# SumitTarafder/Figbird

Measured on AMD Instinct MI355X. Metric: gaps/sec (+ filled-bases/sec), synthetic 1e5-gap set recipe, jump-library fill pass, higher is better.
Workload: dtype f64

## Files before the change

figbird_amd/csrc/fig_abi.hip:

```cpp
#include <hip/hip_runtime.h>

#include <algorithm>
#include <cstdio>
#include <cstdlib>
#include <cstring>
#include <new>
#include <vector>
#include <chrono>
#include <thread>
#include <mutex>

#include "../../include/figbird_hip.h"
#include "fig_engine.h"
#include "fig_pack.h"
#include "fig_abi_host.h"
#include "fig_quality.h"
#include "fig_quality_host.h"
#include "fig_placement.h"
#include "fig_softqual.h"
#include "fig_indel.h"

#ifdef FIG_PROF
#define FIG_PROF_BEGIN() const unsigned long long _k0 = __builtin_readcyclecounter()
#define FIG_PROF_FLUSH() do { if (E.lane == 0) { atomicAdd(&B.counters[FIG_CNT_WAIT], E.wait_cycles); atomicAdd(&B.counters[FIG_CNT_WAVE], (unsigned long long)__builtin_readcyclecounter() - _k0); \
    for (int i = 0; i < FIG_PROF_SLOTS; i++) if (E.prof[i]) atomicAdd(&B.counters[i < FIG_PROF_SPLIT ? FIG_CNT_PROF_LO + i : FIG_CNT_PROF_HI + (i - FIG_PROF_SPLIT)], E.prof[i]); } } while (0)
#else
#define FIG_PROF_BEGIN() ((void)0)
#define FIG_PROF_FLUSH() ((void)0)
#endif

FIG_D void fig_eng_init(FigEng &E, const FigDevModel &M, const FigDevBatch &B, const FigKernArgs &A, bool lds_tab, FigScr &work) {
    fig_eng_ident(E, threadIdx.x, blockDim.x, 64);
    E.M = &M; E.B = &B;
    E.flops = 0; E.mle_alg = 0; E.mle_exec = 0; E.wait_cycles = 0;
    for (int i = 0; i < FIG_PROF_SLOTS; i++) E.prof[i] = 0;
    unsigned char *slab = B.scratch + (long long)blockIdx.x * B.scratch_stride;
    fig_scratch_layout(slab, B.capG, B.capR, B.capP, B.capC, B.capW, B.capE, &work);
    E.scr = work;
    fig_eng_carve(E, M, A, lds_tab);
}

FIG_D void fig_kernel_begin(FigEng &E, const FigDevModel &M, const FigDevBatch &B, const FigKernArgs &A, bool lds_tab, FigScr &work) {
    fig_eng_init(E, M, B, A, lds_tab, work);
    if (blockIdx.x == 0 && threadIdx.x == 0) B.queue_head[A.qsel ^ 1] = 0;
}

FIG_D int fig_queue_pop(FigEng &E, const FigDevBatch &B, const FigKernArgs &A) {
    if (E.tid == 0) E.S->bc_i = atomicAdd(B.queue_head + A.qsel, 1);
    __syncthreads();
    const int qi = E.S->bc_i;
    __syncthreads();
    return qi;
}

template <typename T> struct FigItemSrc { const T *v; int first, end; };
FIG_D FigItemSrc<int32_t> fig_src_order(const FigDevBatch &B, const FigKernArgs &A) { return {B.order, A.q_begin, A.q_end}; }

template <typename Src, typename Body>
FIG_D void fig_pop_loop(FigEng &E, const FigDevBatch &B, const FigKernArgs &A, Src src, Body body) {
    while (true) {
        const int qi = fig_queue_pop(E, B, A);
        const auto s = src();
        if (s.first + qi >= s.end) break;
        body(s.v[s.first + qi]);
    }
}

FIG_D void fig_kernel_flush(const FigEng &E, const FigDevBatch &B) {
    if (E.flops) atomicAdd(&B.counters[FIG_CNT_FLOPS], E.flops);
    if (E.mle_alg) atomicAdd(&B.counters[FIG_CNT_MLE_ALG], E.mle_alg);
    if (E.lane == 0 && E.mle_exec) atomicAdd(&B.counters[FIG_CNT_MLE_EXEC], E.mle_exec);
}

template <bool LDS_TAB, int NT>
__global__ void __launch_bounds__(NT, (NT <= 256 ? 2 : 1)) fig_fill_kernel(FigDevModel M, FigDevBatch B, FigKernArgs A) {
    FigEng E; FigScr work;
    fig_kernel_begin(E, M, B, A, LDS_TAB, work);
    FIG_PROF_BEGIN();
    fig_pop_loop(E, B, A, [&] { return fig_src_order(B, A); }, [&](int gi) { fig_item_fill<LDS_TAB>(E, work, gi); });
    FIG_PROF_FLUSH();
    fig_kernel_flush(E, B);
}

template <bool LDS_TAB, int NT>
__global__ void __launch_bounds__(NT, (NT <= 256 ? 2 : 1)) fig_begin_kernel(FigDevModel M, FigDevBatch B, FigKernArgs A) {
    FigEng E; FigScr work;
    fig_kernel_begin(E, M, B, A, LDS_TAB, work);
    fig_pop_loop(E, B, A, [&] { return fig_src_order(B, A); }, [&](int gi) { fig_item_begin<LDS_TAB>(E, work, gi); });
    fig_kernel_flush(E, B);
}

template <bool LDS_TAB, int NT>
__global__ void __launch_bounds__(NT, (NT <= 256 ? 2 : 1)) fig_probe_kernel(FigDevModel M, FigDevBatch B, FigKernArgs A) {
    FigEng E; FigScr work;
    fig_kernel_begin(E, M, B, A, LDS_TAB, work);
    fig_pop_loop(E, B, A, [&] { return fig_src_order(B, A); }, [&](int gi) { fig_item_probe<LDS_TAB>(E, work, gi); });
}

FIG_D int fig_ld_acquire(const int32_t *p) { return __hip_atomic_load(p, __ATOMIC_ACQUIRE, __HIP_MEMORY_SCOPE_AGENT); }
FIG_D int fig_ld_relaxed(const int32_t *p) { return __hip_atomic_load(p, __ATOMIC_RELAXED, __HIP_MEMORY_SCOPE_AGENT); }

FIG_D bool fig_chunk_finished(FigEng &E, const FigDevBatch &B, int gi, int n) {
    __threadfence();
    __syncthreads();
    if (E.tid == 0) {
        const int done = __hip_atomic_fetch_add(B.gap_pending + gi, 1, __ATOMIC_ACQ_REL, __HIP_MEMORY_SCOPE_AGENT) + 1;
        if (done == n) __hip_atomic_store(B.gap_pending + gi, 0, __ATOMIC_RELAXED, __HIP_MEMORY_SCOPE_AGENT);
        E.S->bc_i = done == n;
    }
    __syncthreads();
    const bool last = E.S->bc_i != 0;
    __syncthreads();
    if (last) __threadfence();
    return last;
}

FIG_D void fig_cont_publish(FigEng &E, const FigDevBatch &B, const FigKernArgs &A, const FigCont &c) {
    __threadfence();
    __syncthreads();
    if (E.tid == 0) {
        bool ok = true;
        if (c.kind == FIG_CONT_EVAL) {
            const long long live = (long long)gridDim.x - fig_ld_relaxed(&B.cont_hdr->exited);
            ok = live * 100 >= (long long)c.n * A.cont_live;
        }
        if (ok) {
            const int idx = atomicAdd(&B.cont_hdr->tail, 1);
            if (idx < B.cont_cap) {
                FigCont *e = B.cont + idx;
                e->gap = c.gap; e->j0 = c.j0; e->n = c.n; e->kind = c.kind; e->next = 0; e->rank = c.rank; e->pad = 0;
                __hip_atomic_store(&e->ready, 1, __ATOMIC_RELEASE, __HIP_MEMORY_SCOPE_AGENT);
                if (c.kind == FIG_CONT_EVAL) atomicAdd(&B.counters[FIG_CNT_CONT], 1ull);
            }
        }
    }
    __syncthreads();
}

FIG_D bool fig_cont_pop(FigEng &E, const FigDevBatch &B, const FigKernArgs &A, FigCont &out, int &k) {
    FigState &S = *E.S;
    if (E.tid == 0) { const int t = fig_ld_relaxed(&B.cont_hdr->tail); S.bc_j = t < B.cont_cap ? t : B.cont_cap; }
    __syncthreads();
    const int tail = S.bc_j;
    __syncthreads();
    for (int pass = 0; pass <= tail; pass++) {
        if (E.tid == 0) S.bc_i = -1;
        __syncthreads();
        int best = -1;
        for (int i = E.tid; i < tail; i += E.nt) {
            const FigCont *e = B.cont + i;
            if (!fig_ld_acquire(&e->ready)) continue;
            if (fig_ld_relaxed(&e->next) >= e->n) continue;
            const int rank = A.cont_prio ? (e->rank < 32767 ? e->rank : 32767) : 0;
            const int key = rank * 65536 + (FIG_CONT_CAP_MAX - i);
            best = key > best ? key : best;
        }
        if (best >= 0) atomicMax(&S.bc_i, best);
        __syncthreads();
        const int key = S.bc_i;
        if (key < 0) { __syncthreads(); return false; }
        const int idx = FIG_CONT_CAP_MAX - (key & 65535);
        if (E.tid == 0) S.bc_j = atomicAdd(&B.cont[idx].next, 1);
        __syncthreads();
        k = S.bc_j;
        __syncthreads();
        if (k < B.cont[idx].n) { __threadfence(); out = B.cont[idx]; return true; }
    }
    return false;
}

static_assert(sizeof(FigItem) == sizeof(int4) && sizeof(FigEntry) == sizeof(int4), "item records travel as int4");
template <bool LDS_TAB, int NT>
__global__ void __launch_bounds__(NT, (NT <= 256 ? 2 : 1)) fig_eval_kernel(FigDevModel M, FigDevBatch B, FigKernArgs A, const int4 *items, int n_items) {
    FigEng E; FigScr work;
    fig_kernel_begin(E, M, B, A, LDS_TAB, work);
    FIG_PROF_BEGIN();
    auto eval = [&](FigItem it) {
        fig_item_eval<LDS_TAB>(E, work, it);
        if (A.cont && it.chunk > 0 && fig_chunk_finished(E, B, it.gap, it.chunk)) {
            FigCont nx;
            fig_item_continue(E, work, it.gap, it.chunk, A.minc, nx);
            fig_cont_publish(E, B, A, nx);
        }
    };
    fig_pop_loop(E, B, A, [&] { return FigItemSrc<FigItem>{(const FigItem *)items, 0, n_items}; }, eval);
    if (A.cont) {
        FigCont c; int k;
        while (fig_cont_pop(E, B, A, c, k)) {
            if (c.kind == FIG_CONT_END) fig_item_end<LDS_TAB>(E, work, c.gap);
            else eval(FigItem{c.gap, c.j0 + k, k, c.n});
        }
        if (E.tid == 0) atomicAdd(&B.cont_hdr->exited, 1);
    }
    FIG_PROF_FLUSH();
    fig_kernel_flush(E, B);
}

__global__ void __launch_bounds__(64) fig_replay_kernel(FigDevModel M, FigDevBatch B, const int4 *entries, int n) {
    if ((int)blockIdx.x >= n) return;
    FigEng E{}; FigScr work{};
    fig_eng_ident(E, threadIdx.x, blockDim.x, 64);
    E.M = &M; E.B = &B; E.nteams = 1; E.S = (FigState *)fig_lds;
    const FigEntry en = ((const FigEntry *)entries)[blockIdx.x];
    if (en.stamped) {
        const FigGapCtl c = B.gapctl[en.gap];
        if (c.status != FIG_GAP_MORE || c.j != en.j_planned || en.n != 0) return;
    }
    fig_item_replay(E, work, en);
}

template <bool LDS_TAB, int NT>
__global__ void __launch_bounds__(NT, (NT <= 256 ? 2 : 1)) fig_end_kernel(FigDevModel M, FigDevBatch B, FigKernArgs A, const int *list, int n) {
    FigEng E; FigScr work;
    fig_kernel_begin(E, M, B, A, LDS_TAB, work);
    fig_pop_loop(E, B, A, [&] { return FigItemSrc<int>{list, 0, n}; }, [&](int gi) { fig_item_end<LDS_TAB>(E, work, gi); });
    fig_kernel_flush(E, B);
}

__global__ void __launch_bounds__(256) fig_stream_kernel(FigDevModel M, FigDevBatch B, uint32_t *out) {
    for (long long gi = blockIdx.x; gi < B.n_gaps; gi += gridDim.x) {
        const FigDevGap &g = B.gaps[gi];
        const int L = M.L;
        const long long n = (long long)((g.nU + FIG_SH_C - 1) / FIG_SH_C) * L * (FIG_SH_C / 2);
        for (long long i = threadIdx.x; i < n; i += blockDim.x) {
            const int sp = (int)(i % (FIG_SH_C / 2));
            const long long cj = i / (FIG_SH_C / 2);
            const int j = (int)(cj % L);
            uint32_t v = 0;
            for (int h = 0; h < 2; h++) {
                const long long r = (cj / L) * FIG_SH_C + 2 * sp + h;
                unsigned e = 0x1000u | FIG_SH_ONE;
                if (r < g.nU) {
                    const long long idx = g.uBase + r;
                    const int len = B.u.len[idx], aux = B.u.aux[idx];
                    if (len == L && !(aux & 2)) {
                        const uint32_t w = B.packed[B.u.woff[idx] + (j >> 4)];
                        e = 0x1000u | (2u * (4u * (unsigned)(aux & 1) + ((w >> ((j & 15) * 2)) & 3u)));
                    }
                }
                v |= e << (16 * h);
            }
            out[g.streamOff + i] = v;
        }
    }
}

#define FIG_HIP(call) do { hipError_t _e = (call); if (_e != hipSuccess) { ctx->last_hip = (int)_e; return FIG_EHIP; } } while (0)

struct DevBuf { void *p = nullptr; };

struct FigTmpBufs {
    std::vector<void *> bufs;
    ~FigTmpBufs() { for (void *p : bufs) hipFree(p); }
    void *alloc(size_t n) { void *p = nullptr; if (hipMalloc(&p, n ? n : 8) != hipSuccess) return nullptr; bufs.push_back(p); return p; }
};

struct FigLane { hipStream_t stream = nullptr; hipEvent_t done = nullptr; int32_t *queue_head = nullptr; uint8_t *scratch = nullptr; FigItem *d_items = nullptr; FigEntry *d_entries = nullptr; size_t cap = 0;
                 FigGapCtl *h_ctl = nullptr; FigItem *h_items = nullptr; FigEntry *h_entries = nullptr; int qsel = 0;
                 uint8_t *d_cont = nullptr; int cont_cap = 0; };

struct fig_ctx {
    int device = 0;
    hipStream_t stream = nullptr;
    hipEvent_t ev0 = nullptr, ev1 = nullptr;
    int n_cu = 0;
    int last_hip = 0;
    bool have_model = false;
    FigDevModel dm;
    DevBuf d_model_tabs;
    fig_model hm;
    std::vector<double> h_ins, h_del;
    bool have_batch = false;
    FigDevBatch db;
    std::vector<int32_t> h_order;
    struct Cls { FigLaunchClass c; int blocks; int capacity; };
    std::vector<Cls> classes;
    std::vector<DevBuf> bufs;
    int64_t n_gaps = 0, n_ureads = 0, n_preads = 0, str_total = 0;
    std::vector<int64_t> h_str_off;
    int nslots = 32;
    std::vector<FigLane> lanes;
    fig_stats stats;
    int sh_on = FIG_SH_SC;
    FigKnobs fill_knobs;
    std::vector<uint8_t> h_ot;
    uint8_t *d_ot = nullptr;
};

static int dev_alloc(fig_ctx *ctx, size_t bytes, void **out) {
    DevBuf b;
    if (bytes == 0) bytes = 8;
    hipError_t e = hipMalloc(&b.p, bytes);
    if (e != hipSuccess) { ctx->last_hip = (int)e; return FIG_ENOMEM; }
    ctx->bufs.push_back(b);
    *out = b.p;
    return FIG_OK;
}

template <typename T>
static int dev_upload(fig_ctx *ctx, const std::vector<T> &v, const T **out) {
    void *p = nullptr;
    int rc = dev_alloc(ctx, v.size() * sizeof(T), &p);
    if (rc) return rc;
    if (!v.empty()) {
        hipError_t e = hipMemcpyAsync(p, v.data(), v.size() * sizeof(T), hipMemcpyHostToDevice, ctx->stream);
        if (e != hipSuccess) { ctx->last_hip = (int)e; return FIG_EHIP; }
    }
    *out = (const T *)p;
    return FIG_OK;
}

extern "C" int fig_version(void) { return FIG_ABI_VERSION; }

extern "C" const char *fig_strerror(int code) { return fig_strerror_text(code); }

extern "C" int fig_ctx_create(int device_ordinal, fig_ctx **out) {
    if (!out) return FIG_EINVAL;
    *out = nullptr;
    static std::once_flag env_once;
    std::call_once(env_once, [] { setenv("GPU_MAX_HW_QUEUES", "8", 0); });
    int n = 0;
    if (hipGetDeviceCount(&n) != hipSuccess || n <= 0) return FIG_ENODEV;
    if (device_ordinal < 0 || device_ordinal >= n) return FIG_ENODEV;
    if (hipSetDevice(device_ordinal) != hipSuccess) return FIG_ENODEV;
    hipDeviceProp_t prop;
    if (hipGetDeviceProperties(&prop, device_ordinal) != hipSuccess) return FIG_ENODEV;
    fig_ctx *ctx = new (std::nothrow) fig_ctx();
    if (!ctx) return FIG_ENOMEM;
    ctx->device = device_ordinal;
    ctx->n_cu = prop.multiProcessorCount > 0 ? prop.multiProcessorCount : 256;
    if (hipStreamCreate(&ctx->stream) != hipSuccess || hipEventCreate(&ctx->ev0) != hipSuccess || hipEventCreate(&ctx->ev1) != hipSuccess) {
        delete ctx;
        return FIG_EHIP;
    }
    memset(&ctx->stats, 0, sizeof(ctx->stats));
    ctx->sh_on = fig_knobs_from_env(0).sh_on;
    *out = ctx;
    return FIG_OK;
}

static void free_batch(fig_ctx *ctx) {
    for (auto &b : ctx->bufs) if (b.p) hipFree(b.p);
    ctx->bufs.clear();
    ctx->d_ot = nullptr;
    ctx->have_batch = false;
    ctx->classes.clear();
    for (auto &l : ctx->lanes) { if (l.stream) hipStreamDestroy(l.stream); if (l.done) hipEventDestroy(l.done); if (l.h_ctl) hipHostFree(l.h_ctl); if (l.h_items) hipHostFree(l.h_items); if (l.h_entries) hipHostFree(l.h_entries); }
    ctx->lanes.clear();
}

extern "C" void fig_batch_free(fig_ctx *ctx) {
    if (!ctx) return;
    hipSetDevice(ctx->device);
    free_batch(ctx);
}

extern "C" void fig_ctx_destroy(fig_ctx *ctx) {
    if (!ctx) return;
    hipSetDevice(ctx->device);
    free_batch(ctx);
    if (ctx->d_model_tabs.p) hipFree(ctx->d_model_tabs.p);
    if (ctx->ev0) hipEventDestroy(ctx->ev0);
    if (ctx->ev1) hipEventDestroy(ctx->ev1);
    if (ctx->stream) hipStreamDestroy(ctx->stream);
    delete ctx;
}

extern "C" int fig_ctx_set_model(fig_ctx *ctx, const fig_model *m) {
    if (!ctx) return FIG_EINVAL;
    if (int rc = fig_model_check(m)) return rc;
    hipSetDevice(ctx->device);
    free_batch(ctx);
    ctx->hm = *m;
    ctx->h_ins.assign(m->in_pos_dist, m->in_pos_dist + m->max_read_length);
    ctx->h_del.assign(m->del_pos_dist, m->del_pos_dist + m->max_read_length);
    std::vector<double> all;
    FigModelOffsets o;
    fig_model_tables(m, all, o, ctx->dm);
    if (ctx->d_model_tabs.p) { hipFree(ctx->d_model_tabs.p); ctx->d_model_tabs.p = nullptr; }
    if (hipMalloc(&ctx->d_model_tabs.p, all.size() * sizeof(double)) != hipSuccess) return FIG_ENOMEM;
    if (hipMemcpy(ctx->d_model_tabs.p, all.data(), all.size() * sizeof(double), hipMemcpyHostToDevice) != hipSuccess) return FIG_EHIP;
    fig_model_point(ctx->dm, o, (const double *)ctx->d_model_tabs.p);
    ctx->have_model = true;
    return FIG_OK;
}

extern "C" int64_t fig_results_capacity(const fig_model *m, const fig_gap_batch *b) {
    if (!m || !b) return FIG_EINVAL;
    return fig_pack_results_capacity(m, b);
}

enum FigKind { FIG_K_FILL, FIG_K_BEGIN, FIG_K_EVAL, FIG_K_END, FIG_K_PROBE };

template <typename... P, typename... Args>
static hipError_t launch_one(void (*k)(P...), size_t lds, int nt, int blocks, hipStream_t stream, Args... args) {
    hipError_t e = hipFuncSetAttribute((const void *)k, hipFuncAttributeMaxDynamicSharedMemorySize, (int)lds);
    if (e != hipSuccess) return e;
    hipLaunchKernelGGL(k, dim3(blocks), dim3(nt), lds, stream, args...);
    return hipGetLastError();
}

template <bool LDS_TAB, int NT>
static hipError_t launch_kind(fig_ctx *ctx, const fig_ctx::Cls &c, const FigDevBatch &db, hipStream_t stream, FigKind kind, int blocks, const void *list, int n, int qsel) {
    FigKernArgs A = fig_kargs_of(c.c, qsel, ctx->sh_on);
    if (kind == FIG_K_EVAL) { const FigKnobs &kn = ctx->fill_knobs; A.cont = kn.cont && db.cont_cap > 0; A.minc = kn.minc; A.cont_live = kn.cont_live; A.cont_prio = kn.cont_prio; }
    switch (kind) {
        case FIG_K_FILL: return launch_one(fig_fill_kernel<LDS_TAB, NT>, c.c.lds, NT, blocks, stream, ctx->dm, db, A);
        case FIG_K_BEGIN: return launch_one(fig_begin_kernel<LDS_TAB, NT>, c.c.lds, NT, blocks, stream, ctx->dm, db, A);
        case FIG_K_PROBE: return launch_one(fig_probe_kernel<LDS_TAB, NT>, c.c.lds, NT, blocks, stream, ctx->dm, db, A);
        case FIG_K_EVAL: return launch_one(fig_eval_kernel<LDS_TAB, NT>, c.c.lds, NT, blocks, stream, ctx->dm, db, A, (const int4 *)list, n);
        case FIG_K_END: return launch_one(fig_end_kernel<LDS_TAB, NT>, c.c.lds, NT, blocks, stream, ctx->dm, db, A, (const int *)list, n);
    }
    return hipErrorInvalidValue;
}

static hipError_t launch_any(fig_ctx *ctx, const fig_ctx::Cls &c, const FigDevBatch &db, hipStream_t stream, FigKind kind, int blocks, const void *list, int n, int qsel = 0) {
    if (c.c.tiles > 0) return launch_kind<true, 512>(ctx, c, db, stream, kind, blocks, list, n, qsel);
    if (c.c.lds_tab) return c.c.nt == 256 ? launch_kind<true, 256>(ctx, c, db, stream, kind, blocks, list, n, qsel) : launch_kind<true, 512>(ctx, c, db, stream, kind, blocks, list, n, qsel);
    return launch_kind<false, 512>(ctx, c, db, stream, kind, blocks, list, n, qsel);
}

extern "C" int fig_batch_upload(fig_ctx *ctx, const fig_gap_batch *b) {
    if (!ctx || !b) return FIG_EINVAL;
    if (!ctx->have_model) return FIG_EINVAL;
    hipSetDevice(ctx->device);
    free_batch(ctx);
    const fig_model *m = &ctx->hm;
    hipEventRecord(ctx->ev0, ctx->stream);
    FigPacked K;
    int prc = fig_pack(m, b, sizeof(FigState), K);
    if (prc) return prc;
    int64_t ng = K.n_gaps;
    ctx->h_order = K.order; ctx->h_str_off = K.str_off;
    ctx->str_total = K.str_total; ctx->n_gaps = ng;
    ctx->n_ureads = (int64_t)K.u_pos.size(); ctx->n_preads = (int64_t)K.p_pos.size();
    ctx->classes.clear();
    const bool log = fig_knobs_from_env(0).log;
    for (const FigLaunchClass &lc : K.classes) {
        fig_ctx::Cls c;
        c.c = lc;
        int per_cu = (int)std::max<size_t>(1, std::min<size_t>((160 * 1024) / std::max<size_t>(lc.lds, 1), (size_t)(2048 / lc.nt)));
        per_cu = std::min(per_cu, 8);
        c.capacity = ctx->n_cu * per_cu;
        c.blocks = std::min<int>(lc.q_end - lc.q_begin, c.capacity);
        if (log) fprintf(stderr, "[figsched] class: capG=%d capGl=%d ncolE=%d Wcap=%d nt=%d nteams=%d lds_tab=%d tiles=%d tile_cols=%d lds=%zu gaps=%d per_cu=%d blocks=%d (FigState %zu B)\n",
                                             lc.capG, lc.capGl, lc.ncolE, lc.Wcap, lc.nt, lc.nteams, (int)lc.lds_tab, lc.tiles, lc.tile_cols, lc.lds, lc.q_end - lc.q_begin, per_cu, c.blocks, sizeof(FigState));
        ctx->classes.push_back(c);
    }
    int64_t stride = fig_scratch_layout(nullptr, K.capG, K.capR, K.capP, K.capC, K.capW, K.capE, nullptr);
    stride = (stride + 255) & ~255LL;

    FigDevBatch &db = ctx->db;
    memset(&db, 0, sizeof(db));
    db.n_gaps = ng;
    int rc;
#define UP(vec, field) do { rc = dev_upload(ctx, K.vec, &db.field); if (rc) return rc; } while (0)
    UP(gaps, gaps); UP(order, order); UP(packed, packed); UP(qual, qual); UP(flank, flank);
    UP(u_pos, u.pos); UP(u_aux, u.aux); UP(u_len, u.len); UP(u_woff, u.woff);
    UP(p_pos, p.pos); UP(p_aux, p.aux); UP(p_clip, p.clip); UP(p_ref, p.refpos); UP(p_len, p.len); UP(p_woff, p.woff); UP(p_qoff, p.qoff);
#undef UP
    db.u.clip = nullptr; db.u.refpos = nullptr; db.u.qoff = nullptr;
    void *p;
    if (m->unmapped_flag) {
        if ((rc = dev_alloc(ctx, (size_t)K.stream_total * 4, &p))) return rc;
        db.ustream = (const uint32_t *)p;
        FIG_HIP(hipMemsetD32Async((hipDeviceptr_t)p, (int)(((0x1000u | FIG_SH_ONE) << 16) | (0x1000u | FIG_SH_ONE)), (size_t)K.stream_total, ctx->stream));
        if (ng > 0) {
            hipLaunchKernelGGL(fig_stream_kernel, dim3((unsigned)std::min<int64_t>(ng, 4096)), dim3(256), 0, ctx->stream, ctx->dm, db, (uint32_t *)p);
            FIG_HIP(hipGetLastError());
        }
    }
    if ((rc = dev_alloc(ctx, (size_t)ng * 4, &p))) return rc; db.filled_len = (int32_t *)p;
    if ((rc = dev_alloc(ctx, (size_t)ng * 4, &p))) return rc; db.gaptofill = (int32_t *)p;
    if ((rc = dev_alloc(ctx, (size_t)K.str_total, &p))) return rc; db.str = (char *)p;
    if ((rc = dev_alloc(ctx, 64 * (ctx->classes.size() + 1), &p))) return rc; db.queue_head = (int32_t *)p;
    if ((rc = dev_alloc(ctx, FIG_CNT_N * sizeof(unsigned long long), &p))) return rc; db.counters = (unsigned long long *)p;
    size_t total_blocks = 0;
    for (const fig_ctx::Cls &c : ctx->classes) total_blocks += (size_t)c.capacity;
    if ((rc = dev_alloc(ctx, (size_t)stride * std::max<size_t>(total_blocks, 1), &p))) return rc; db.scratch = (uint8_t *)p;
    if ((rc = dev_alloc(ctx, (size_t)K.persist_total + 256, &p))) return rc; db.persist = (uint8_t *)p;
    if ((rc = dev_alloc(ctx, (size_t)std::max<int64_t>(ng, 1) * sizeof(FigGapCtl), &p))) return rc; db.gapctl = (FigGapCtl *)p;
    if ((rc = dev_alloc(ctx, (size_t)std::max<int64_t>(ng, 1) * 4, &p))) return rc; db.gap_pending = (int32_t *)p;
    if ((rc = dev_alloc(ctx, (size_t)std::max<int64_t>(ng, 1), &p))) return rc; ctx->d_ot = (uint8_t *)p; db.ot_preset = ctx->d_ot;
    ctx->h_ot = K.ot_preset;
    FIG_HIP(hipMemcpyAsync(ctx->d_ot, ctx->h_ot.data(), (size_t)std::max<int64_t>(ng, 1), hipMemcpyHostToDevice, ctx->stream));
    ctx->nslots = K.nslots;
    {   size_t blk = 0;
        for (size_t ci = 0; ci < ctx->classes.size(); ci++) {
            const fig_ctx::Cls &c = ctx->classes[ci];
            ctx->lanes.push_back(FigLane());
            FigLane &l = ctx->lanes.back();
            if (hipStreamCreate(&l.stream) != hipSuccess || hipEventCreateWithFlags(&l.done, hipEventDisableTiming) != hipSuccess) return FIG_EHIP;
            l.queue_head = db.queue_head + 16 * (ci + 1);
            l.scratch = db.scratch + (size_t)stride * blk; blk += (size_t)c.capacity;
            l.cap = (size_t)std::max(c.c.q_end - c.c.q_begin, 1) * (size_t)(K.nslots + 1);
            if ((rc = dev_alloc(ctx, l.cap * sizeof(FigItem), &p))) return rc; l.d_items = (FigItem *)p;
            if ((rc = dev_alloc(ctx, l.cap * sizeof(FigEntry), &p))) return rc; l.d_entries = (FigEntry *)p;
            l.cont_cap = fig_cont_capacity(std::vector<int>(K.order.begin() + c.c.q_begin, K.order.begin() + c.c.q_end), K.gaps, fig_knobs_from_env(0).minc);
            if ((rc = dev_alloc(ctx, sizeof(FigContHdr) + (size_t)l.cont_cap * sizeof(FigCont), &p))) return rc; l.d_cont = (uint8_t *)p;
            if (hipHostMalloc((void **)&l.h_ctl, (size_t)std::max<int64_t>(ng, 1) * sizeof(FigGapCtl), hipHostMallocDefault) != hipSuccess) return FIG_ENOMEM;
            if (hipHostMalloc((void **)&l.h_items, l.cap * sizeof(FigItem), hipHostMallocDefault) != hipSuccess) return FIG_ENOMEM;
            if (hipHostMalloc((void **)&l.h_entries, l.cap * sizeof(FigEntry), hipHostMallocDefault) != hipSuccess) return FIG_ENOMEM;
        }
    }
    db.scratch_stride = stride;
    db.capG = K.capG; db.capR = K.capR; db.capP = K.capP; db.capC = K.capC; db.capW = K.capW; db.capE = K.capE;
    db.n_ureads = ctx->n_ureads;
    FIG_HIP(hipMemsetAsync(db.counters, 0, FIG_CNT_N * sizeof(unsigned long long), ctx->stream));
    FIG_HIP(hipMemsetAsync(db.queue_head, 0, 64 * (ctx->classes.size() + 1), ctx->stream));
    hipEventRecord(ctx->ev1, ctx->stream);
    FIG_HIP(hipStreamSynchronize(ctx->stream));
    float ms = 0; hipEventElapsedTime(&ms, ctx->ev0, ctx->ev1);
    ctx->stats.h2d_ms = ms;
    ctx->stats.packed_bytes = K.packed_bytes();
    ctx->have_batch = true;
    if (!K.ot_given && m->partial_flag && ng > 0 && (rc = fig_ot_carry_measured(ctx, ng))) { free_batch(ctx); return rc; }
    return FIG_OK;
}

extern "C" int fig_batch_probe_reach(fig_ctx *ctx, uint8_t *reach) {
    if (!ctx || !reach || !ctx->have_batch) return FIG_EINVAL;
    hipSetDevice(ctx->device);
    const int64_t ng = ctx->n_gaps;
    memset(reach, 0, (size_t)ng);
    if (!ctx->hm.partial_flag || ng == 0) return FIG_OK;
    FigDevBatch db = ctx->db;
    fig_batch_clear_planes(db);
    FIG_HIP(hipMemsetAsync(db.gapctl, 0, (size_t)ng * sizeof(FigGapCtl), ctx->stream));
    for (const fig_ctx::Cls &c : ctx->classes) {
        FIG_HIP(hipMemsetAsync(db.queue_head, 0, 8, ctx->stream));
        FIG_HIP(launch_any(ctx, c, db, ctx->stream, FIG_K_PROBE, c.blocks, nullptr, 0));
    }
    std::vector<FigGapCtl> ctl((size_t)ng);
    FIG_HIP(hipMemcpyAsync(ctl.data(), db.gapctl, (size_t)ng * sizeof(FigGapCtl), hipMemcpyDeviceToHost, ctx->stream));
    FIG_HIP(hipStreamSynchronize(ctx->stream));
    for (int64_t g = 0; g < ng; g++) reach[g] = ctl[g].reach ? 1 : 0;
    return FIG_OK;
}

extern "C" int fig_batch_set_ot_preset(fig_ctx *ctx, const uint8_t *preset) {
    if (!ctx || !preset || !ctx->have_batch) return FIG_EINVAL;
    hipSetDevice(ctx->device);
    const int64_t ng = ctx->n_gaps;
    for (int64_t g = 0; g < ng; g++) ctx->h_ot[(size_t)g] = preset[g] ? 1 : 0;
    if (ng > 0) { FIG_HIP(hipMemcpy(ctx->d_ot, ctx->h_ot.data(), (size_t)ng, hipMemcpyHostToDevice)); }
    return FIG_OK;
}

static int run_class_parallel(fig_ctx *ctx, const fig_ctx::Cls &c, FigLane &ln, const FigKnobs &knobs) {
    FigDevBatch db = ctx->db;
    db.queue_head = ln.queue_head; db.scratch = ln.scratch;
    db.cont_hdr = (FigContHdr *)ln.d_cont; db.cont = (FigCont *)(ln.d_cont + sizeof(FigContHdr));
    db.cont_cap = knobs.cont ? std::min(ln.cont_cap, knobs.cont_cap) : 0;
    const size_t cont_bytes = sizeof(FigContHdr) + (size_t)db.cont_cap * sizeof(FigCont);
    hipStream_t stream = ln.stream;
    hipSetDevice(ctx->device);
    int nl = 0;
    hipError_t e;
    auto fail = [&](hipError_t er) { ctx->last_hip = (int)er; return -1; };
    const int capacity = std::max(1, c.capacity);
    auto launch = [&](FigKind kind, int n_work, const void *list) {
        hipError_t er = launch_any(ctx, c, db, stream, kind, std::min(capacity, n_work), list, n_work, ln.qsel);
        ln.qsel ^= 1; nl++;
        return er;
    };
    if ((e = launch(FIG_K_BEGIN, c.c.q_end - c.c.q_begin, nullptr)) != hipSuccess) return fail(e);
    FigGapCtl *ctl = ln.h_ctl;
    const size_t ctl_bytes = (size_t)ctx->n_gaps * sizeof(FigGapCtl);
    const std::vector<int> ids(ctx->h_order.begin() + c.c.q_begin, ctx->h_order.begin() + c.c.q_end);
    FigRound R;
    auto now = [] { return std::chrono::duration<double, std::milli>(std::chrono::steady_clock::now().time_since_epoch()).count(); };
    const double t_start = now();
    double t_prev = now(); int round = 0, last_items = 0, last_active = 0, last_chunk = 0, n_active_max = 0;
    while (true) {
        if ((e = hipMemcpyAsync(ctl, db.gapctl, ctl_bytes, hipMemcpyDeviceToHost, stream)) != hipSuccess) return fail(e);
        if ((e = hipStreamSynchronize(stream)) != hipSuccess) return fail(e);
        fig_plan_round(ids, ctl, capacity, c.c.nsplit, ctx->nslots, knobs.minc, knobs.ipw, n_active_max, R);
        if (knobs.log) { double t = now(); fprintf(stderr, "[figsched] capG=%d round %d: active=%d chunk=%d items=%d blocks=%d  %.1f ms\n", c.c.capG, round, last_active, last_chunk, last_items, capacity, t - t_prev); t_prev = t; }
        round++;
        if (R.n_active == 0) break;
        if (ln.cap < R.items.size() || ln.cap < R.entries.size()) return fail(hipErrorOutOfMemory);
        const int n_empty = knobs.cont ? fig_round_stamp(R, ctl) : 0;
        const int n_items = (int)R.items.size(), n_ent = (int)R.entries.size();
        const size_t items_bytes = R.items.size() * sizeof(FigItem), ent_bytes = R.entries.size() * sizeof(FigEntry);
        last_items = n_items; last_active = R.n_active; last_chunk = R.chunk;
        if (n_items > 0) {
            memcpy(ln.h_items, R.items.data(), items_bytes);
            if ((e = hipMemcpyAsync(ln.d_items, ln.h_items, items_bytes, hipMemcpyHostToDevice, stream)) != hipSuccess) return fail(e);
            if (knobs.cont && (e = hipMemsetAsync(ln.d_cont, 0, cont_bytes, stream)) != hipSuccess) return fail(e);
            if ((e = launch(FIG_K_EVAL, n_items, ln.d_items)) != hipSuccess) return fail(e);
        }
        if (knobs.cont && n_empty == 0) continue;
        memcpy(ln.h_entries, R.entries.data(), ent_bytes);
        if ((e = hipMemcpyAsync(ln.d_entries, ln.h_entries, ent_bytes, hipMemcpyHostToDevice, stream)) != hipSuccess) return fail(e);
        hipLaunchKernelGGL(fig_replay_kernel, dim3(n_ent), dim3(64), sizeof(FigState) + 64, stream, ctx->dm, db, (const int4 *)ln.d_entries, n_ent);
        if ((e = hipGetLastError()) != hipSuccess) return fail(e);
        nl++;
    }
    std::vector<int> endlist;
    for (int g : ids) if (ctl[g].status == FIG_GAP_LOOP_DONE) endlist.push_back(g);
    if (!endlist.empty()) {
        if ((e = hipStreamSynchronize(stream)) != hipSuccess) return fail(e);
        memcpy(ln.h_items, endlist.data(), endlist.size() * sizeof(int));
        if ((e = hipMemcpyAsync(ln.d_items, ln.h_items, endlist.size() * sizeof(int), hipMemcpyHostToDevice, stream)) != hipSuccess) return fail(e);
        if ((e = launch(FIG_K_END, (int)endlist.size(), ln.d_items)) != hipSuccess) return fail(e);
        if (knobs.log) { const double t0 = now(); hipStreamSynchronize(stream); fprintf(stderr, "[figsched] capG=%d end kernel: %d gaps, %.1f ms (lane done at %.1f ms since its first round)\n", c.c.capG, (int)endlist.size(), now() - t0, now() - t_start); }
    }
    return nl;
}

extern "C" int fig_fill_resident(fig_ctx *ctx, fig_gap_results *out) { return fig_fill_resident_ex(ctx, out, nullptr); }

extern "C" int fig_fill_resident_ex(fig_ctx *ctx, fig_gap_results *out, const fig_gap_support *sup) {
    if (!ctx || !out || !ctx->have_batch) return FIG_EINVAL;
    if (!out->filled_len || !out->gaptofill || !out->str_off || (!out->str && ctx->str_total > 0)) return FIG_EINVAL;
    if (sup && (!sup->counts || !sup->origin)) return FIG_EINVAL;
    hipSetDevice(ctx->device);
    int64_t ng = ctx->n_gaps;
    FigDevBatch &db = ctx->db;
    FigTmpBufs tmp;
    std::vector<int32_t> hsup(sup ? (size_t)ctx->str_total * 5 : 0);
    const std::vector<FigPlane> planes = fig_fill_planes(db, ctx->n_ureads + ctx->n_preads, ctx->str_total, out, sup, hsup.data());
    auto clear = [&](void *p, int v, size_t n) { return n ? hipMemsetAsync(p, v, n, ctx->stream) : hipSuccess; };
    auto fetch = [&](void *dst, const void *src, size_t n) { return n ? hipMemcpyAsync(dst, src, n, hipMemcpyDeviceToHost, ctx->stream) : hipSuccess; };
    for (const FigPlane &pl : planes) {
        if (!(*pl.dev = tmp.alloc(pl.bytes))) return FIG_ENOMEM;
        if (pl.fill >= 0) FIG_HIP(clear(*pl.dev, pl.fill, pl.bytes));
    }
    FIG_HIP(clear(db.counters, 0, FIG_CNT_N * sizeof(unsigned long long)));
    FIG_HIP(clear(db.queue_head, 0, 64 * (ctx->classes.size() + 1)));
    for (auto &l : ctx->lanes) l.qsel = 0;
    FIG_HIP(clear(db.filled_len, 0, (size_t)std::max<int64_t>(ng, 1) * 4));
    FIG_HIP(clear(db.gaptofill, 0, (size_t)std::max<int64_t>(ng, 1) * 4));
    FIG_HIP(clear(db.str, 'N', (size_t)ctx->str_total));
    FIG_HIP(clear(db.gapctl, 0, (size_t)std::max<int64_t>(ng, 1) * sizeof(FigGapCtl)));
    FIG_HIP(clear(db.gap_pending, 0, (size_t)std::max<int64_t>(ng, 1) * 4));
    FIG_HIP(hipEventRecord(ctx->ev0, ctx->stream));
    int nl = 0;
    const FigKnobs knobs = fig_knobs_from_env(ctx->dm.unmapped);
    ctx->fill_knobs = knobs;
    if (knobs.seq) {
        for (const fig_ctx::Cls &c : ctx->classes) {
            FIG_HIP(clear(db.queue_head, 0, 4));
            FIG_HIP(launch_any(ctx, c, db, ctx->stream, FIG_K_FILL, c.blocks, nullptr, 0));
            nl++;
        }
    } else {
        const size_t nc = ctx->classes.size();
        std::vector<int> rcs(nc, 0);
        for (size_t ci = 0; ci < nc; ci++) FIG_HIP(hipStreamWaitEvent(ctx->lanes[ci].stream, ctx->ev0, 0));
        if (nc <= 1 || knobs.lanes_serial) {
            for (size_t ci = 0; ci < nc; ci++) rcs[ci] = run_class_parallel(ctx, ctx->classes[ci], ctx->lanes[ci], knobs);
        } else {
            std::vector<std::thread> th;
            for (size_t ci = 0; ci < nc; ci++) th.emplace_back([&, ci] { rcs[ci] = run_class_parallel(ctx, ctx->classes[ci], ctx->lanes[ci], knobs); });
            for (auto &t : th) t.join();
        }
        for (size_t ci = 0; ci < nc; ci++) {
            if (rcs[ci] < 0) { hipDeviceSynchronize(); return FIG_EHIP; }
            nl += rcs[ci];
            FIG_HIP(hipEventRecord(ctx->lanes[ci].done, ctx->lanes[ci].stream));
            FIG_HIP(hipStreamWaitEvent(ctx->stream, ctx->lanes[ci].done, 0));
        }
    }
    FIG_HIP(hipEventRecord(ctx->ev1, ctx->stream)); FIG_HIP(hipStreamSynchronize(ctx->stream));
    float ms = 0; FIG_HIP(hipEventElapsedTime(&ms, ctx->ev0, ctx->ev1));
    ctx->stats.kernel_ms = ms; ctx->stats.n_launches = nl;
    FIG_HIP(hipEventRecord(ctx->ev0, ctx->stream));
    std::vector<char> hstr((size_t)ctx->str_total);
    unsigned long long cnt[FIG_CNT_N] = {0};
    FIG_HIP(fetch(out->filled_len, db.filled_len, (size_t)ng * 4)); FIG_HIP(fetch(out->gaptofill, db.gaptofill, (size_t)ng * 4));
    FIG_HIP(fetch(hstr.data(), db.str, (size_t)ctx->str_total));
    FIG_HIP(fetch(cnt, db.counters, sizeof(cnt)));
    for (const FigPlane &pl : planes) FIG_HIP(fetch(pl.host, *pl.dev, pl.bytes));
    FIG_HIP(hipEventRecord(ctx->ev1, ctx->stream)); FIG_HIP(hipStreamSynchronize(ctx->stream));
    FIG_HIP(hipEventElapsedTime(&ms, ctx->ev0, ctx->ev1));
    ctx->stats.d2h_ms = ms;
#ifdef FIG_PROF
    { auto prof = [&](int i) { return cnt[i < FIG_PROF_SPLIT ? FIG_CNT_PROF_LO + i : FIG_CNT_PROF_HI + (i - FIG_PROF_SPLIT)]; };
      const unsigned long long wave = cnt[FIG_CNT_WAVE];
      const char *nm[14] = {"A.wait", "B.wait", "-", "M.finish", "PR.pre", "PR.estep", "PR.mid", "PR.mle", "PR.post", "A.chain", "A.logexp", "A.work", "B.work", "M.chains"};
      for (int i = 0; i < 14; i++) fprintf(stderr, "[figprof] %-9s %8.1f Gcycles = %5.1f %% of wave-cycles\n", nm[i], prof(i) / 1e9, wave ? 100.0 * prof(i) / wave : 0.0);
      const char *mn[4] = {"M.setup", "M.hint", "M.rounds", "M.surv"};
      for (int i = 0; i < 4; i++) fprintf(stderr, "[figprof] %-9s %8.1f Gcycles = %5.1f %% of wave-cycles\n", mn[i], prof(14 + i) / 1e9, wave ? 100.0 * prof(14 + i) / wave : 0.0);
      fprintf(stderr, "[figprof] raw slots:"); for (int i = 0; i < FIG_PROF_SLOTS; i++) fprintf(stderr, " %d:%.1f", i, prof(i) / 1e9); fprintf(stderr, "\n");
      fprintf(stderr, "[figprof] barrier wait %.3f of %.3f wave-Gcycles = %.1f %%\n", cnt[FIG_CNT_WAIT] / 1e9, wave / 1e9, wave ? 100.0 * cnt[FIG_CNT_WAIT] / wave : 0.0); }
#endif
    if (knobs.log) fprintf(stderr, "[figsched] useful flops %.4g, speculative evaluations executed %.4g (%.1f %% discarded)\n", (double)cnt[FIG_CNT_FLOPS], (double)cnt[FIG_CNT_SPEC], cnt[FIG_CNT_SPEC] ? 100.0 * (1.0 - ((double)cnt[FIG_CNT_FLOPS] / (double)cnt[FIG_CNT_SPEC])) : 0.0);
    fig_stats_from_counters(cnt, ctx->stats);
    int rc = fig_compact_results(ng, hstr.data(), ctx->h_str_off.data(), out);
    if (!rc && sup) fig_compact_support(ng, hsup.data(), ctx->h_str_off.data(), out, sup->counts);
    return rc;
}

struct FigPostFill {
    fig_ctx *ctx = nullptr;
    const fig_gap_results *f = nullptr;
    int64_t total = 0;
    std::vector<FigDevGap> hg;
    std::vector<double> tabs;
    FigTmpBufs tmp;
    bool oom = false;
    float ms = 0;

    int open(fig_ctx *c, const fig_gap_results *filled, std::vector<double> *insd = nullptr) {
        ctx = c; f = filled;
        if (!ctx || !f || !ctx->have_batch || !ctx->have_model) return FIG_EINVAL;
        if (!f->filled_len || !f->str_off || !f->draw_pos || !f->draw_len) return FIG_EINVAL;
        hipSetDevice(ctx->device);
        const int64_t ng = ctx->n_gaps;
        if (f->str_off[0] < 0) return FIG_EINVAL;
        for (int64_t g = 0; g < ng; g++) if (f->str_off[g + 1] < f->str_off[g]) return FIG_EINVAL;
        total = f->str_off[ng];
        if (total > 0 && !f->str) return FIG_EINVAL;
        const int L = ctx->dm.L;
        hg.resize((size_t)ng);
        std::vector<double> he((size_t)L), home((size_t)L);
        tabs.resize((size_t)fig_quality_tab_doubles(L));
        if (ng > 0) FIG_HIP(fetch(hg.data(), ctx->db.gaps, (size_t)ng * sizeof(FigDevGap)));
        FIG_HIP(fetch(he.data(), ctx->dm.e, (size_t)L * sizeof(double)));
        FIG_HIP(fetch(home.data(), ctx->dm.ome1, (size_t)L * sizeof(double)));
        if (insd) { insd->resize((size_t)ctx->dm.max_insert); FIG_HIP(fetch(insd->data(), ctx->dm.insd, insd->size() * sizeof(double))); }
        FIG_HIP(hipStreamSynchronize(ctx->stream));
        fig_quality_tables(L, he.data(), home.data(), ctx->dm.T, tabs.data(), tabs.data() + L, tabs.data() + 2 * L);
        return FIG_OK;
    }
    int64_t drawn_reads(int64_t g, int32_t n, int64_t base, int64_t cnt, int64_t limit) const {
        if (n > (1 << 30) || f->str_off[g] + n > f->str_off[g + 1] || base < 0 || cnt < 0 || base + cnt > limit) return -1;
        return fig_quality_check_placements(f->draw_pos + base, cnt);
    }
    hipError_t fetch(void *dst, const void *src, size_t bytes) { return hipMemcpyAsync(dst, src, bytes, hipMemcpyDeviceToHost, ctx->stream); }
    void *alloc(size_t bytes) { void *p = tmp.alloc(bytes); oom = oom || !p; return p; }
    template <typename T> const T *up(const T *src, size_t count) {
        void *p = alloc(count * sizeof(T));
        if (p && count && hipMemcpyAsync(p, src, count * sizeof(T), hipMemcpyHostToDevice, ctx->stream) != hipSuccess) { oom = true; return nullptr; }
        return (const T *)p;
    }
    template <typename Launch, typename Back> int run(Launch launch, Back back) {
        if (oom) { hipStreamSynchronize(ctx->stream); return FIG_ENOMEM; }
        FIG_HIP(hipEventRecord(ctx->ev0, ctx->stream));
        launch();
        FIG_HIP(hipGetLastError());
        FIG_HIP(hipEventRecord(ctx->ev1, ctx->stream));
        FIG_HIP(back());
        FIG_HIP(hipStreamSynchronize(ctx->stream));
        FIG_HIP(hipEventElapsedTime(&ms, ctx->ev0, ctx->ev1));
        return FIG_OK;
    }
};
#define FIG_TRY(call) do { const int _rc = (call); if (_rc != FIG_OK) return _rc; } while (0)

extern "C" int fig_batch_quality(fig_ctx *ctx, const fig_gap_results *f, const int32_t *origin, fig_gap_quality *q) {
    if (!q || !q->loglik || !q->phred || !q->state || (f && !f->draw_isz)) return FIG_EINVAL;
    FigPostFill P;
    FIG_TRY(P.open(ctx, f));
    const int64_t ng = ctx->n_gaps, total = P.total, nr = ctx->n_ureads + ctx->n_preads;
    const FigDevBatch &db = ctx->db;
    std::vector<int32_t> list, ncol((size_t)std::max<int64_t>(ng, 1), 0);
    std::vector<uint8_t> part((size_t)std::max<int64_t>(ng, 1), 0);
    int64_t cols = 0, reads = 0;
    for (int64_t g = 0; g < ng; g++) {
        const int32_t n = f->filled_len[g], lu = f->draw_len[2 * g], lp = f->draw_len[2 * g + 1];
        q->state[g] = fig_quality_gap_on(n, lu, lp, origin != nullptr, origin ? origin[g] : 0);
        if (q->state[g] != FIG_QUAL_ON) continue;
        const bool p = lp >= 0;
        const int64_t base = p ? ctx->n_ureads + P.hg[(size_t)g].pBase : P.hg[(size_t)g].uBase, cnt = p ? P.hg[(size_t)g].nP : P.hg[(size_t)g].nU;
        const int64_t drawn = P.drawn_reads(g, n, base, cnt, nr);
        if (drawn < 0) return FIG_EINVAL;
        list.push_back((int32_t)g); ncol[(size_t)g] = n; part[(size_t)g] = p ? 1 : 0;
        cols += n; reads += drawn;
    }
    if (total > 0) memset(q->loglik, 0, (size_t)total * 4 * sizeof(double));
    if (total > 0) memset(q->phred, 0, (size_t)total);
    if (!list.empty()) {
        FigQualArgs A;
        A.gaps = db.gaps; A.u_len = db.u.len; A.u_aux = db.u.aux; A.p_len = db.p.len; A.u_woff = db.u.woff; A.p_woff = db.p.woff;
        A.packed = db.packed; A.n_ureads = ctx->n_ureads; A.L = ctx->dm.L;
        A.draw_pos = P.up(f->draw_pos, (size_t)nr);
        A.list = P.up(list.data(), list.size());
        A.ncol = P.up(ncol.data(), (size_t)ng);
        A.partial = P.up(part.data(), (size_t)ng);
        A.str_off = P.up(f->str_off, (size_t)(ng + 1));
        A.tabs = P.up(P.tabs.data(), P.tabs.size());
        A.loglik = (double *)P.alloc((size_t)total * 4 * sizeof(double));
        if (A.loglik) FIG_HIP(hipMemsetAsync(A.loglik, 0, (size_t)total * 4 * sizeof(double), ctx->stream));
        FIG_TRY(P.run([&] { hipLaunchKernelGGL(fig_quality_kernel, dim3((unsigned)list.size()), dim3(FIG_Q_NT), 0, ctx->stream, A); },
                      [&] { return P.fetch(q->loglik, A.loglik, (size_t)total * 4 * sizeof(double)); }));
    }
    for (int32_t g : list)
        for (int64_t i = f->str_off[g], e = f->str_off[g] + ncol[(size_t)g]; i < e; i++) q->phred[i] = fig_quality_phred(q->loglik + i * 4, f->str[i]);
    if (fig_knobs_from_env(ctx->dm.unmapped).log)
        fprintf(stderr, "[figqual] gaps on %zu of %lld, columns %lld, reads %lld, kernel %.3f ms\n", list.size(), (long long)ng, (long long)cols, (long long)reads, P.ms);
    return FIG_OK;
}

struct FigPlacePass {
    std::vector<int32_t> items, ncol;
    std::vector<uint8_t> scored, state;
    std::vector<double> li, hd;
    std::vector<int32_t> hi;
    int64_t gaps_on = 0, reads = 0, placements = 0, cols = 0, nu = 0;
    FigPlaceArgs A;
    double *dd = nullptr;
    int32_t *di = nullptr;

    int prepare(FigPostFill &P, const int32_t *origin, const std::vector<double> &insd) {
        fig_ctx *ctx = P.ctx;
        const fig_gap_results *f = P.f;
        const int64_t ng = ctx->n_gaps;
        const FigDevBatch &db = ctx->db;
        const int MI = ctx->dm.max_insert;
        nu = ctx->n_ureads;
        li.resize((size_t)MI);
        fig_placement_li(MI, insd.data(), li.data());
        ncol.assign((size_t)std::max<int64_t>(ng, 1), 0);
        state.assign((size_t)std::max<int64_t>(ng, 1), FIG_PLACE_OFF);
        scored.assign((size_t)std::max<int64_t>(nu, 1), 0);
        for (int64_t g = 0; g < ng; g++) {
            const int32_t n = f->filled_len[g];
            state[(size_t)g] = fig_placement_gap_on(ctx->dm.unmapped != 0, n, f->draw_len[2 * g], f->draw_len[2 * g + 1], origin != nullptr, origin ? origin[g] : 0);
            if (state[(size_t)g] != FIG_PLACE_ON) continue;
            const int64_t base = P.hg[(size_t)g].uBase, cnt = P.hg[(size_t)g].nU;
            const int64_t drawn = P.drawn_reads(g, n, base, cnt, nu);
            if (drawn < 0) return FIG_EINVAL;
            gaps_on++; ncol[(size_t)g] = n; reads += drawn; cols += n;
            for (int64_t r = 0; r < cnt; r++) scored[(size_t)(base + r)] = f->draw_pos[base + r] != INT32_MIN;
            for (int64_t c0 = 0; c0 < cnt; c0 += FIG_RS_CHUNK) {
                bool any = false;
                for (int64_t r = c0; r < std::min<int64_t>(c0 + FIG_RS_CHUNK, cnt); r++) any = any || scored[(size_t)(base + r)];
                if (any) { items.push_back((int32_t)g); items.push_back((int32_t)c0); }
            }
        }
        if (items.empty()) return FIG_OK;
        A.gaps = db.gaps; A.u_len = db.u.len; A.u_aux = db.u.aux; A.u_pos = db.u.pos; A.u_woff = db.u.woff; A.packed = db.packed; A.flank = db.flank;
        A.L = ctx->dm.L; A.Tmin = ctx->dm.Tmin; A.Tmax = ctx->dm.Tmax; A.max_insert = MI;
        A.draw_pos = P.up(f->draw_pos, (size_t)nu);
        A.items = P.up(items.data(), items.size());
        A.ncol = P.up(ncol.data(), (size_t)ng);
        A.str_off = P.up(f->str_off, (size_t)(ng + 1));
        A.str = P.up(f->str, (size_t)P.total);
        A.tabs = P.up(P.tabs.data(), P.tabs.size());
        A.li = P.up(li.data(), li.size());
        dd = (double *)P.alloc((size_t)nu * 3 * sizeof(double));
        di = (int32_t *)P.alloc((size_t)nu * 2 * sizeof(int32_t));
        A.ll_drawn = dd; A.ll_other = dd + nu; A.sum_other = dd + 2 * nu; A.off_other = di; A.n_valid = di + nu;
        hd.resize((size_t)nu * 3); hi.resize((size_t)nu * 2);
        return FIG_OK;
    }
    void launch(hipStream_t stream) { hipLaunchKernelGGL(fig_placement_kernel, dim3((unsigned)(items.size() / 2)), dim3(FIG_P_NT), 0, stream, A); }
    hipError_t fetch(FigPostFill &P) { const hipError_t e = P.fetch(hd.data(), dd, hd.size() * sizeof(double)); return e != hipSuccess ? e : P.fetch(hi.data(), di, hi.size() * sizeof(int32_t)); }
    void finish(fig_read_placement *p, int64_t ng, bool launched) {
        for (int64_t g = 0; g < ng; g++) p->state[g] = state[(size_t)g];
        for (int64_t r = 0; r < nu; r++) {
            p->ll_drawn[r] = 0.0; p->ll_other[r] = 0.0; p->sum_other[r] = 0.0; p->off_other[r] = INT32_MIN; p->n_valid[r] = 0; p->pq[r] = FIG_PLACE_NONE;
        }
        placements = 0;
        if (!launched) return;
        for (int64_t r = 0; r < nu; r++) {
            if (!scored[(size_t)r]) continue;
            p->ll_drawn[r] = hd[(size_t)r]; p->ll_other[r] = hd[(size_t)(nu + r)]; p->sum_other[r] = hd[(size_t)(2 * nu + r)];
            p->off_other[r] = hi[(size_t)r]; p->n_valid[r] = hi[(size_t)(nu + r)];
            p->pq[r] = fig_placement_phred(p->ll_drawn[r], p->ll_other[r], p->sum_other[r]);
            placements += p->n_valid[r];
        }
    }
};
static bool fig_placement_members(const fig_read_placement *p) { return p->ll_drawn && p->ll_other && p->sum_other && p->off_other && p->n_valid && p->pq && p->state; }

extern "C" int fig_batch_placement(fig_ctx *ctx, const fig_gap_results *f, const int32_t *origin, fig_read_placement *p) {
    if (!p || !fig_placement_members(p)) return FIG_EINVAL;
    FigPostFill P;
    std::vector<double> insd;
    FIG_TRY(P.open(ctx, f, &insd));
    FigPlacePass PP;
    FIG_TRY(PP.prepare(P, origin, insd));
    const bool work = !PP.items.empty();
    if (work) FIG_TRY(P.run([&] { PP.launch(ctx->stream); }, [&] { return PP.fetch(P); }));
    PP.finish(p, ctx->n_gaps, work);
    if (fig_knobs_from_env(ctx->dm.unmapped).log)
        fprintf(stderr, "[figplace] gaps on %lld of %lld, reads scored %lld, placements scored %lld, kernel %.3f ms\n", (long long)PP.gaps_on, (long long)ctx->n_gaps, (long long)PP.reads, (long long)PP.placements, P.ms);
    return FIG_OK;
}

extern "C" int fig_batch_softqual(fig_ctx *ctx, const fig_gap_results *f, const int32_t *origin, fig_read_placement *pl, fig_gap_softqual *out) {
    if (!out || !out->wcount || !out->eloglik || !out->phred || !out->state) return FIG_EINVAL;
    if (pl && !fig_placement_members(pl)) return FIG_EINVAL;
    FigPostFill P;
    std::vector<double> insd;
    FIG_TRY(P.open(ctx, f, &insd));
    FigPlacePass PP;
    FIG_TRY(PP.prepare(P, origin, insd));
    const int64_t ng = ctx->n_gaps, total = P.total;
    for (int64_t g = 0; g < ng; g++) out->state[g] = PP.state[(size_t)g] == FIG_PLACE_ON ? FIG_SOFTQ_ON : FIG_SOFTQ_OFF;
    if (total > 0) { memset(out->wcount, 0, (size_t)total * 4 * sizeof(double)); memset(out->eloglik, 0, (size_t)total * 4 * sizeof(double)); memset(out->phred, 0, (size_t)total); }
    const bool work = !PP.items.empty();
    float ms_place = 0, ms_soft = 0;
    int64_t active = 0;
    if (work) {
        std::vector<int32_t> blocks;
        for (int64_t g = 0; g < ng; g++)
            if (PP.state[(size_t)g] == FIG_PLACE_ON) for (int32_t xb = 0; xb < PP.ncol[(size_t)g]; xb += FIG_SQ_NT) { blocks.push_back((int32_t)g); blocks.push_back(xb); }
        const size_t nb = blocks.size() / 2, plane = (size_t)total * 4;
        FigSoftqArgs A;
        const FigPlaceArgs &Q = PP.A;
        A.gaps = Q.gaps; A.u_len = Q.u_len; A.u_aux = Q.u_aux; A.u_pos = Q.u_pos; A.u_woff = Q.u_woff; A.packed = Q.packed; A.flank = Q.flank;
        A.draw_pos = Q.draw_pos; A.ncol = Q.ncol; A.str_off = Q.str_off; A.str = Q.str; A.tabs = Q.tabs; A.li = Q.li;
        A.L = Q.L; A.Tmin = Q.Tmin; A.Tmax = Q.Tmax; A.max_insert = Q.max_insert;
        A.placed = PP.dd; A.n_ureads = PP.nu;
        A.items = P.up(blocks.data(), blocks.size());
        double *dp = (double *)P.alloc(plane * 2 * sizeof(double) + nb * sizeof(int32_t));
        A.out = dp; A.plane = (int64_t)plane;
        std::vector<int32_t> hact(nb, 0);
        struct Ev { hipEvent_t e = nullptr; ~Ev() { if (e) hipEventDestroy(e); } } mid;
        if (P.oom) { hipStreamSynchronize(ctx->stream); return FIG_ENOMEM; }
        FIG_HIP(hipEventCreate(&mid.e));
        FIG_HIP(hipMemsetAsync(dp, 0, plane * 2 * sizeof(double), ctx->stream));
        FIG_HIP(hipEventRecord(ctx->ev0, ctx->stream));
        PP.launch(ctx->stream);
        FIG_HIP(hipGetLastError());
        FIG_HIP(hipEventRecord(mid.e, ctx->stream));
        hipLaunchKernelGGL(fig_softqual_kernel, dim3((unsigned)nb), dim3(FIG_SQ_NT), 0, ctx->stream, A);
        FIG_HIP(hipGetLastError());
        FIG_HIP(hipEventRecord(ctx->ev1, ctx->stream));
        FIG_HIP(P.fetch(out->wcount, dp, plane * sizeof(double)));
        FIG_HIP(P.fetch(out->eloglik, dp + plane, plane * sizeof(double)));
        FIG_HIP(P.fetch(hact.data(), dp + 2 * plane, nb * sizeof(int32_t)));
        if (pl) FIG_HIP(PP.fetch(P));
        FIG_HIP(hipStreamSynchronize(ctx->stream));
        FIG_HIP(hipEventElapsedTime(&ms_place, ctx->ev0, mid.e));
        FIG_HIP(hipEventElapsedTime(&ms_soft, mid.e, ctx->ev1));
        for (int32_t a : hact) active += a;
    }
    if (pl) PP.finish(pl, ng, work);
    for (int64_t g = 0; g < ng; g++)
        if (out->state[g] == FIG_SOFTQ_ON)
            for (int64_t i = f->str_off[g], e = f->str_off[g] + PP.ncol[(size_t)g]; i < e; i++) out->phred[i] = fig_quality_phred(out->eloglik + i * 4, f->str[i]);
    if (fig_knobs_from_env(ctx->dm.unmapped).log)
        fprintf(stderr, "[figsoftq] gaps on %lld of %lld, columns %lld, reads %lld, active placements %lld, placement kernel %.3f ms, softqual kernel %.3f ms\n",
                (long long)PP.gaps_on, (long long)ng, (long long)PP.cols, (long long)PP.reads, (long long)active, ms_place, ms_soft);
    return FIG_OK;
}

extern "C" int fig_batch_indel(fig_ctx *ctx, const fig_gap_results *f, const int32_t *origin, fig_gap_indel *out) {
    if (!out || !out->ll_flat || !out->ll_gapped || !out->n_ins || !out->n_del || !out->d_end || !out->d_start || !out->del_reads || !out->ins_reads ||
        !out->cover || !out->ins_end || !out->call || !out->call_end || !out->state) return FIG_EINVAL;
    FigPostFill P;
    FIG_TRY(P.open(ctx, f));
    const int64_t ng = ctx->n_gaps, total = P.total, nu = ctx->n_ureads;
    const FigDevBatch &db = ctx->db;
    const int L = ctx->dm.L;
    std::vector<int32_t> hlen((size_t)std::max<int64_t>(nu, 1), 0);
    if (nu > 0) { FIG_HIP(P.fetch(hlen.data(), db.u.len, (size_t)nu * sizeof(int32_t))); FIG_HIP(hipStreamSynchronize(ctx->stream)); }
    std::vector<int32_t> items, ncol((size_t)std::max<int64_t>(ng, 1), 0);
    std::vector<uint8_t> aligned((size_t)std::max<int64_t>(nu, 1), 0);
    int64_t gaps_on = 0, reads = 0, events = 0, called = 0;
    for (int64_t g = 0; g < ng; g++) {
        const int32_t n = f->filled_len[g];
        out->state[g] = fig_indel_gap_on(ctx->dm.unmapped != 0, n, f->draw_len[2 * g], f->draw_len[2 * g + 1], origin != nullptr, origin ? origin[g] : 0);
        if (out->state[g] != FIG_INDEL_ON) continue;
        const int64_t base = P.hg[(size_t)g].uBase, cnt = P.hg[(size_t)g].nU;
        if (P.drawn_reads(g, n, base, cnt, nu) < 0) return FIG_EINVAL;
        gaps_on++; ncol[(size_t)g] = n;
        for (int64_t c0 = 0; c0 < cnt; c0 += FIG_RS_CHUNK) {
            bool any = false;
            for (int64_t r = c0; r < std::min<int64_t>(c0 + FIG_RS_CHUNK, cnt); r++) {
                const bool a = fig_indel_aligned(f->draw_pos[base + r], std::min(std::max(hlen[(size_t)(base + r)], 0), L), n);
                aligned[(size_t)(base + r)] = a; any = any || a; reads += a;
            }
            if (any) { items.push_back((int32_t)g); items.push_back((int32_t)c0); }
        }
    }
    for (int64_t r = 0; r < nu; r++) { out->ll_flat[r] = 0.0; out->ll_gapped[r] = 0.0; out->n_ins[r] = 0; out->n_del[r] = 0; out->d_end[r] = 0; out->d_start[r] = INT32_MIN; }
    for (int64_t i = 0; i < total; i++) { out->del_reads[i] = 0; out->ins_reads[i] = 0; out->cover[i] = 0; out->call[i] = '.'; }
    for (int64_t g = 0; g < ng; g++) { out->ins_end[g] = 0; out->call_end[g] = '.'; }
    if (!items.empty()) {
        std::vector<double> tid((size_t)(2 * L));
        fig_indel_tables(L, ctx->h_ins.data(), ctx->h_del.data(), tid.data(), tid.data() + L);
        FigIndelArgs A;
        A.gaps = db.gaps; A.u_len = db.u.len; A.u_aux = db.u.aux; A.u_woff = db.u.woff; A.packed = db.packed; A.flank = db.flank; A.L = L;
        A.draw_pos = P.up(f->draw_pos, (size_t)nu);
        A.items = P.up(items.data(), items.size());
        A.ncol = P.up(ncol.data(), (size_t)ng);
        A.str_off = P.up(f->str_off, (size_t)(ng + 1));
        A.str = P.up(f->str, (size_t)total);
        A.tabs = P.up(P.tabs.data(), P.tabs.size());
        A.tabs_id = P.up(tid.data(), tid.size());
        double *dd = (double *)P.alloc((size_t)nu * 2 * sizeof(double));
        int32_t *di = (int32_t *)P.alloc((size_t)nu * 4 * sizeof(int32_t));
        const size_t ncnt = (size_t)total * 3 + (size_t)ng;
        int32_t *dc = (int32_t *)P.alloc(ncnt * sizeof(int32_t));
        A.ll_flat = dd; A.ll_gapped = dd + nu; A.n_ins = di; A.n_del = di + nu; A.d_end = di + 2 * nu; A.d_start = di + 3 * nu;
        A.del_reads = dc; A.ins_reads = dc + total; A.cover = dc + 2 * total; A.ins_end = dc + 3 * total;
        if (dc) FIG_HIP(hipMemsetAsync(dc, 0, ncnt * sizeof(int32_t), ctx->stream));
        std::vector<double> hd((size_t)nu * 2);
        std::vector<int32_t> hi((size_t)nu * 4);
        FIG_TRY(P.run([&] { fig_indel_launch(A, (unsigned)(items.size() / 2), ctx->stream); },
                      [&] {
                          hipError_t e = P.fetch(hd.data(), dd, hd.size() * sizeof(double));
                          if (e == hipSuccess) e = P.fetch(hi.data(), di, hi.size() * sizeof(int32_t));
                          if (e == hipSuccess && total > 0) e = P.fetch(out->del_reads, A.del_reads, (size_t)total * sizeof(int32_t));
                          if (e == hipSuccess && total > 0) e = P.fetch(out->ins_reads, A.ins_reads, (size_t)total * sizeof(int32_t));
                          if (e == hipSuccess && total > 0) e = P.fetch(out->cover, A.cover, (size_t)total * sizeof(int32_t));
                          return e != hipSuccess ? e : P.fetch(out->ins_end, A.ins_end, (size_t)ng * sizeof(int32_t));
                      }));
        for (int64_t r = 0; r < nu; r++) {
            if (!aligned[(size_t)r]) continue;
            out->ll_flat[r] = hd[(size_t)r]; out->ll_gapped[r] = hd[(size_t)(nu + r)];
            out->n_ins[r] = hi[(size_t)r]; out->n_del[r] = hi[(size_t)(nu + r)]; out->d_end[r] = hi[(size_t)(2 * nu + r)]; out->d_start[r] = hi[(size_t)(3 * nu + r)];
            events += out->n_ins[r] + out->n_del[r] > 0;
        }
        for (int64_t g = 0; g < ng; g++) {
            if (out->state[g] != FIG_INDEL_ON) continue;
            const int64_t s0 = f->str_off[g], n = ncol[(size_t)g];
            for (int64_t i = s0; i < s0 + n; i++) { out->call[i] = fig_indel_call(out->del_reads[i], out->ins_reads[i], out->cover[i]); called += out->call[i] != '.'; }
            out->call_end[g] = fig_indel_majority(out->ins_end[g], out->cover[s0 + n - 1]) ? 'I' : '.';
            called += out->call_end[g] != '.';
        }
    }
    if (fig_knobs_from_env(ctx->dm.unmapped).log)
        fprintf(stderr, "[figindel] gaps on %lld of %lld, reads aligned %lld, reads with an event %lld, columns called %lld, kernel %.3f ms\n",
                (long long)gaps_on, (long long)ng, (long long)reads, (long long)events, (long long)called, P.ms);
    return FIG_OK;
}

extern "C" int fig_fill_gaps(fig_ctx *ctx, const fig_gap_batch *batch, fig_gap_results *out) { return fig_fill_gaps_once(ctx, batch, out); }

extern "C" int fig_get_stats(const fig_ctx *ctx, fig_stats *out) {
    if (!ctx || !out) return FIG_EINVAL;
    *out = ctx->stats;
    return FIG_OK;
}
```

figbird_amd/csrc/fig_abi_host.h:

```cpp
#ifndef FIG_ABI_HOST_H
#define FIG_ABI_HOST_H
#include <algorithm>
#include <cmath>
#include <cstdlib>
#include <cstring>
#include <vector>
#include "../../include/figbird_hip.h"
#include "fig_types.h"
#include "fig_gaprules.h"

static_assert(FIG_ORG_NONE == FIG_SUP_NONE && FIG_ORG_FINAL == FIG_SUP_FINAL && FIG_ORG_ORIGINAL == FIG_SUP_ORIGINAL && FIG_ORG_TIEBREAK == FIG_SUP_TIEBREAK,
              "the engine's path mask (fig_types.h) is fig_gap_support::origin");

static inline const char *fig_strerror_text(int code) {
    switch (code) {
        case FIG_OK: return "ok";
        case FIG_EINVAL: return "invalid argument";
        case FIG_ENODEV: return "no usable HIP device (libfighip has no CPU path)";
        case FIG_ENOMEM: return "out of memory";
        case FIG_EHIP: return "HIP runtime error";
        case FIG_ENOSPC: return "result string buffer too small";
        case FIG_EUNSUP: return "input outside the supported envelope";
        default: return "unknown error";
    }
}

static inline int fig_model_check(const fig_model *m) {
    if (!m || !m->error_pos_dist || !m->in_pos_dist || !m->del_pos_dist || !m->insert_len_dist_smoothed) return FIG_EINVAL;
    if (m->max_read_length <= 0 || m->max_read_length > FIG_MAX_READLEN) return FIG_EUNSUP;
    if (m->max_insert_size <= 0) return FIG_EINVAL;
    if (m->partial_flag && m->unmapped_flag) return FIG_EUNSUP;
    if (m->insert_threshold_min < 0 || m->insert_threshold_max >= m->max_insert_size + 1) return FIG_EINVAL;
    return FIG_OK;
}

struct FigModelOffsets { size_t e, pairs, m3, insd, qtab, ome; };

static void fig_model_tables(const fig_model *m, std::vector<double> &all, FigModelOffsets &o, FigDevModel &dm) {
    const int L = m->max_read_length;
    std::vector<double> h_e(m->error_pos_dist, m->error_pos_dist + L), h_ome(L), h_m3(L);
    for (int k = 0; k < L; k++) {
        volatile double a = 1 - m->error_pos_dist[k];
        h_ome[k] = a;
        volatile double b = 1 - m->error_pos_dist[k] - m->in_pos_dist[k] - m->del_pos_dist[k];
        h_m3[k] = b;
    }
    std::vector<double> h_insd(m->insert_len_dist_smoothed, m->insert_len_dist_smoothed + m->max_insert_size);
    h_insd.push_back(0.0);
    std::vector<double> h_qtab(256);
    for (int c = 0; c < 256; c++) { int Q = c - 33; h_qtab[c] = pow(10, -Q / 10.0); }
    std::vector<double> pairs((size_t)8 * L);
    for (int k = 0; k < L; k++) {
        pairs[2 * k] = h_ome[k]; pairs[2 * k + 1] = h_e[k];
        pairs[2 * L + 2 * k] = h_ome[L - 1 - k]; pairs[2 * L + 2 * k + 1] = h_e[L - 1 - k];
        pairs[4 * L + 2 * k] = h_m3[k]; pairs[4 * L + 2 * k + 1] = h_e[k];
        pairs[6 * L + 2 * k] = h_m3[L - 1 - k]; pairs[6 * L + 2 * k + 1] = h_e[L - 1 - k];
    }
    all.clear();
    o.e = 0; all.insert(all.end(), h_e.begin(), h_e.end()); while (all.size() % 8) all.push_back(0);
    o.pairs = all.size(); all.insert(all.end(), pairs.begin(), pairs.end()); while (all.size() % 8) all.push_back(0);
    o.m3 = all.size(); all.insert(all.end(), h_m3.begin(), h_m3.end()); while (all.size() % 8) all.push_back(0);
    o.insd = all.size(); all.insert(all.end(), h_insd.begin(), h_insd.end()); while (all.size() % 8) all.push_back(0);
    o.qtab = all.size(); all.insert(all.end(), h_qtab.begin(), h_qtab.end());
    o.ome = all.size(); all.insert(all.end(), h_ome.begin(), h_ome.end());
    dm.L = L; dm.Tmin = m->insert_threshold_min; dm.Tmax = m->insert_threshold_max; dm.cutoff = m->gap_prob_cutoff;
    dm.partial_flag = m->partial_flag; dm.unmapped = m->unmapped_flag; dm.script_itr = m->script_itr; dm.D = m->max_distance;
    dm.read_length = m->read_length; dm.neg_overlap = m->neg_overlap; dm.partial_len = m->partial_len; dm.unm_limit = m->unm_limit;
    dm.max_insert = m->max_insert_size;
    for (int i = 0; i < 25; i++) dm.T[i] = m->error_type_probs[i];
    dm.fmm_up = fig_model_fmm(m);
}

static inline void fig_model_point(FigDevModel &dm, const FigModelOffsets &o, const double *d) {
    dm.e = d + o.e; dm.ome = d + o.pairs; dm.m3 = d + o.m3; dm.insd = d + o.insd; dm.qtab = d + o.qtab;
    dm.ome1 = d + o.ome;
}

static inline void fig_batch_clear_planes(FigDevBatch &db) {
    db.dbg_n_cand = nullptr; db.dbg_cand_i = nullptr; db.dbg_cand_lik = nullptr; db.dbg_max_cand = 0; db.dbg_n_place = nullptr;
    db.draw_pos = db.draw_isz = db.draw_len = nullptr;
    db.dbg_counts = db.dbg_read_maxlv = nullptr; db.dbg_plane_cols = db.dbg_plane_reads = 0;
    db.sup_counts = db.sup_origin = nullptr;
}

struct FigPlane { void **dev; void *host; size_t bytes; int fill; };

static std::vector<FigPlane> fig_fill_planes(FigDevBatch &db, int64_t n_reads, int64_t str_total, const fig_gap_results *out, const fig_gap_support *sup, int32_t *sup_host) {
    std::vector<FigPlane> pl;
    auto add = [&](auto *&dev, void *host, size_t bytes, int fill) { pl.push_back(FigPlane{(void **)&dev, host, bytes, fill}); };
    const size_t ng = (size_t)db.n_gaps, nr = (size_t)n_reads;
    fig_batch_clear_planes(db);
    if (out->dbg_n_cand && out->dbg_cand_i && out->dbg_cand_lik && out->dbg_max_cand > 0) {
        const size_t nc = ng * out->dbg_max_cand;
        db.dbg_max_cand = out->dbg_max_cand;
        add(db.dbg_n_cand, out->dbg_n_cand, ng * 4, 0);
        add(db.dbg_cand_i, out->dbg_cand_i, nc * 12, -1);
        add(db.dbg_cand_lik, out->dbg_cand_lik, nc * 8, -1);
        if (out->dbg_n_place) add(db.dbg_n_place, out->dbg_n_place, ng * 4, 0);
        if (out->dbg_counts && out->dbg_plane_cols > 0) { db.dbg_plane_cols = out->dbg_plane_cols; add(db.dbg_counts, out->dbg_counts, nc * out->dbg_plane_cols * 5 * 8, 0); }
        if (out->dbg_read_maxlv && out->dbg_plane_reads > 0) { db.dbg_plane_reads = out->dbg_plane_reads; add(db.dbg_read_maxlv, out->dbg_read_maxlv, nc * out->dbg_plane_reads * 8, 0); }
    }
    if (out->draw_pos && out->draw_isz && out->draw_len) {
        add(db.draw_pos, out->draw_pos, nr * 4, -1);
        add(db.draw_isz, out->draw_isz, nr * 4, 0);
        add(db.draw_len, out->draw_len, ng * 8, -1);
    }
    if (sup) {
        add(db.sup_counts, sup_host, (size_t)str_total * 5 * 4, 0);
        add(db.sup_origin, sup->origin, ng * 4, 0);
    }
    return pl;
}

static inline void fig_stats_from_counters(const unsigned long long *cnt, fig_stats &st) {
    st.place_calls = (int64_t)cnt[FIG_CNT_PLACE];
    st.alg_flops = (double)cnt[FIG_CNT_FLOPS]; st.spec_flops = (double)cnt[FIG_CNT_SPEC];
    st.mle_alg_flops = (double)cnt[FIG_CNT_MLE_ALG]; st.mle_exec_flops = (double)cnt[FIG_CNT_MLE_EXEC];
    st.cont_chunks = (int32_t)cnt[FIG_CNT_CONT];
}

static FigKernArgs fig_kargs_of(const FigLaunchClass &c, int qsel, int sh_on) {
    FigKernArgs A;
    A.capG = c.capG; A.capGl = c.capGl; A.ncolE = c.ncolE; A.Wcap = c.Wcap; A.nteams = c.nteams;
    A.q_begin = c.q_begin; A.q_end = c.q_end; A.qsel = qsel;
    A.tiles = c.tiles; A.tile_step = c.tile_step; A.tile_cols = c.tile_cols; A.tiled_max = c.tiled_max;
    A.sh_on = sh_on;
    return A;
}

static int fig_ot_carry_measured(fig_ctx *ctx, int64_t ng) {
    std::vector<uint8_t> reach((size_t)ng, 0), preset((size_t)ng, 0);
    int rc;
    if ((rc = fig_batch_probe_reach(ctx, reach.data()))) return rc;
    std::vector<int64_t> ids((size_t)ng);
    for (int64_t g = 0; g < ng; g++) ids[(size_t)g] = g;
    fig_ot_carry(ids, reach.data(), preset.data());
    return fig_batch_set_ot_preset(ctx, preset.data());
}

static int fig_compact_results(int64_t ng, const char *src, const int64_t *src_off, fig_gap_results *out) {
    int64_t need = 0;
    for (int64_t g = 0; g < ng; g++) need += out->filled_len[g] > 0 ? out->filled_len[g] : 0;
    if (need > out->str_capacity) return FIG_ENOSPC;
    int64_t o = 0;
    for (int64_t g = 0; g < ng; g++) {
        out->str_off[g] = o;
        int n = out->filled_len[g];
        if (n > 0) { memcpy(out->str + o, src + src_off[g], (size_t)n); o += n; }
    }
    out->str_off[ng] = o;
    return FIG_OK;
}

static void fig_compact_support(int64_t ng, const int32_t *src, const int64_t *src_off, const fig_gap_results *out, int32_t *dst) {
    for (int64_t g = 0; g < ng; g++) {
        int n = out->filled_len[g];
        if (n > 0) memcpy(dst + out->str_off[g] * 5, src + src_off[g] * 5, (size_t)n * 5 * sizeof(int32_t));
    }
}

static int fig_fill_gaps_once(fig_ctx *ctx, const fig_gap_batch *batch, fig_gap_results *out) {
    int rc = fig_batch_upload(ctx, batch);
    if (rc) return rc;
    rc = fig_fill_resident(ctx, out);
    fig_batch_free(ctx);
    return rc;
}

struct FigKnobs {
    bool seq;
    bool cont; int cont_cap, cont_live, cont_prio;
    bool lanes_serial;
    bool log;
    int minc;
    double ipw;
    int sh_on;
};

static FigKnobs fig_knobs_from_env(int unmapped) {
    FigKnobs k;
    const char *sched = getenv("FIG_SCHED"), *ser = getenv("FIG_LANES"), *mc = getenv("FIG_MIN_CHUNK"), *ipw = getenv("FIG_ITEMS_PER_WG");
    const char *ev = getenv("FIG_ESTEP"), *sc = getenv("FIG_SH_CHUNKS");
    k.seq = sched && strcmp(sched, "seq") == 0;
    const char *cc = getenv("FIG_CONT_CAP"), *cl = getenv("FIG_CONT_LIVE"), *cp = getenv("FIG_CONT_PRIO");
    k.cont = sched ? strcmp(sched, "continuous") == 0 : unmapped != 0;
    k.cont_cap = cc ? std::max(1, atoi(cc)) : FIG_CONT_CAP_MAX;
    k.cont_live = cl ? std::max(0, atoi(cl)) : 100;
    k.cont_prio = cp ? (atoi(cp) != 0) : 1;
    k.lanes_serial = ser && strcmp(ser, "serial") == 0;
    k.log = getenv("FIG_SCHED_LOG") != nullptr;
    k.minc = mc ? std::max(1, atoi(mc)) : 16;
    k.ipw = ipw ? std::max(1.0, atof(ipw)) : (unmapped ? 12.0 : 6.0);
    k.sh_on = (ev && !strcmp(ev, "pair")) ? 0 : (sc ? std::max(1, std::min(FIG_SH_SC, atoi(sc))) : FIG_SH_SC);
    return k;
}

struct FigRound { std::vector<FigItem> items; std::vector<FigEntry> entries; int chunk = 0, n_active = 0; };

static void fig_plan_round(const std::vector<int> &ids, const FigGapCtl *ctl, int capacity, int nsplit, int slots_cap, int minc, double ipw_base,
                           int &n_active_max, FigRound &R) {
    R.items.clear(); R.entries.clear();
    R.chunk = 0; R.n_active = 0;
    for (int g : ids) if (ctl[g].status == FIG_GAP_MORE) R.n_active++;
    if (R.n_active == 0) return;
    long long rem_total = 0;
    for (int g : ids) if (ctl[g].status == FIG_GAP_MORE) rem_total += std::max(0, ctl[g].range - ctl[g].j);
    n_active_max = std::max(n_active_max, R.n_active);
    const double ipw = ipw_base * std::min(8.0, std::max(1.0, n_active_max / 96.0));
    const double share = rem_total > 0 ? (ipw * capacity / (double)std::max(1, nsplit)) / (double)rem_total : 1.0;
    const double target = ipw * capacity / (double)std::max(1, nsplit);
    long long total = 0;
    for (int g : ids) {
        if (ctl[g].status != FIG_GAP_MORE) continue;
        if ((double)total >= 1.25 * target) break;
        int j = ctl[g].j, range = ctl[g].range;
        int want = (int)std::ceil((range - j) * share);
        want = std::min(std::max(want, minc), slots_cap);
        int n = std::max(0, std::min(want, range - j));
        R.chunk = std::max(R.chunk, n);
        total += n;
        R.entries.push_back(FigEntry{g, n, 0, 0});
    }
    for (const FigEntry &en : R.entries)
        for (int k = en.n - 1; k >= 0; k--) R.items.push_back(FigItem{en.gap, ctl[en.gap].j + k, k, 0});
}

static int fig_round_stamp(FigRound &R, const FigGapCtl *ctl) {
    size_t pos = 0; int n_empty = 0;
    for (FigEntry &en : R.entries) {
        en.j_planned = ctl[en.gap].j; en.stamped = 1;
        if (en.n == 0) n_empty++;
        for (int k = 0; k < en.n; k++) R.items[pos++].chunk = en.n;
    }
    return n_empty;
}

static int fig_cont_capacity(const std::vector<int> &ids, const std::vector<FigDevGap> &gaps, int minc) {
    long long n = 0;
    for (int g : ids) n += gaps[(size_t)g].rangeCap / std::max(1, minc) + 3;
    return (int)std::min<long long>(std::max<long long>(n, 1), FIG_CONT_CAP_MAX);
}

#endif
```

figbird_amd/csrc/fig_engine.h:

```cpp
#ifndef FIG_ENGINE_H
#define FIG_ENGINE_H

#include "fig_types.h"

#ifdef FIG_EMU
#include <cmath>
#include <cstring>
#define FIG_D static inline
#define FIG_NOINLINE
#define FIG_HD static inline
#define FIG_SYNC() ((void)0)
FIG_D double fig_log10(double x) { return log10(x); }
FIG_D double fig_log(double x) { return log(x); }
FIG_D double fig_exp(double x) { return exp(x); }
FIG_D double fig_pow10(double x) { return pow(10, x); }
FIG_D int fig_atomic_add_i32(int *p, int v) { int o = *p; *p += v; return o; }
FIG_D void fig_atomic_max_i32(int *p, int v) { if (v > *p) *p = v; }
FIG_D int fig_atomic_fetch_add_i32(int *p, int v) { int o = *p; *p += v; return o; }
FIG_D void fig_atomic_min_i32(int *p, int v) { if (v < *p) *p = v; }
FIG_D void fig_atomic_or_i32(int *p, int v) { *p |= v; }
FIG_D void fig_atomic_add_u64(unsigned long long *p, unsigned long long v) { *p += v; }
FIG_D unsigned long long fig_shfl_down_u64(unsigned long long v, int off) { (void)v; (void)off; return 0; }
#else
#include <hip/hip_runtime.h>
#define FIG_D __device__ static
#define FIG_NOINLINE __attribute__((noinline))
#define FIG_HD __host__ __device__ static
#ifdef FIG_PROF
#define FIG_SYNC() do { unsigned long long _bt = __builtin_readcyclecounter(); __syncthreads(); E.wait_cycles += __builtin_readcyclecounter() - _bt; } while (0)
#else
#define FIG_SYNC() __syncthreads()
#endif
FIG_D double fig_log10(double x) { return log10(x); }
FIG_D double fig_log(double x) { return log(x); }
FIG_D double fig_exp(double x) { return exp(x); }
FIG_D double fig_pow10(double x) { return pow(10.0, x); }
FIG_D int fig_atomic_add_i32(int *p, int v) { return atomicAdd(p, v); }
FIG_D void fig_atomic_max_i32(int *p, int v) { atomicMax(p, v); }
FIG_D int fig_atomic_fetch_add_i32(int *p, int v) { return atomicAdd(p, v); }
FIG_D void fig_atomic_min_i32(int *p, int v) { atomicMin(p, v); }
FIG_D void fig_atomic_or_i32(int *p, int v) { atomicOr(p, v); }
FIG_D void fig_atomic_add_u64(unsigned long long *p, unsigned long long v) { atomicAdd(p, v); }
FIG_D unsigned long long fig_shfl_down_u64(unsigned long long v, int off) { return __shfl_down(v, off, 64); }
#endif

#define FIG_NOPOS 0x7fffffff
#define FIG_PLB_TEAMS 8
#define FIG_PLB_BYTES (FIG_PLB_TEAMS * 64 * 4)

#if defined(FIG_PROF) && !defined(FIG_EMU)
#define FIG_T0(E) unsigned long long _fig_t = __builtin_readcyclecounter()
#define FIG_TICK(E, slot) do { unsigned long long _n = __builtin_readcyclecounter(); (E).prof[slot] += _n - _fig_t; _fig_t = _n; } while (0)
#define FIG_COUNT(E, slot, n) do { (E).prof[slot] += (n); } while (0)
#else
#define FIG_COUNT(E, slot, n) do { } while (0)
#define FIG_T0(E) do { } while (0)
#define FIG_TICK(E, slot) do { } while (0)
#endif

#ifdef FIG_EMU
static double *fig_lds = nullptr;
#define FIG_RFL(x) (x)
typedef const uint32_t *fig_cu32p;
typedef const double *fig_cdp;
typedef double *fig_gdp;
typedef const double *fig_gcdp;
typedef const uint32_t *fig_gcu32p;
typedef const unsigned char *fig_gcu8p;
typedef const unsigned char *fig_lcu8p;
#else
extern __shared__ __attribute__((aligned(16))) double fig_lds[];
#define FIG_RFL(x) __builtin_amdgcn_readfirstlane(x)
typedef const uint32_t __attribute__((address_space(4))) *fig_cu32p;
typedef const double __attribute__((address_space(4))) *fig_cdp;
typedef double __attribute__((address_space(1))) *fig_gdp;
typedef const double __attribute__((address_space(1))) *fig_gcdp;
typedef const uint32_t __attribute__((address_space(1))) *fig_gcu32p;
typedef const unsigned char __attribute__((address_space(1))) *fig_gcu8p;
typedef const unsigned char __attribute__((address_space(3))) *fig_lcu8p;
#endif

struct alignas(16) FigPQ { double p, q; };

struct FigLoop {
    int inr, range, gapMin, j, gapEstimate, maxGapEstimate, finalize_flag;
    int fill_or_not, same_count, same_thresh, stuckCount, side_flag, less_read_flag;
    int prev_best, curr_best, prev_u, curr_u, sec_same, sec_same2;
    int done, need_orig;
    int ev_iters, ev_side_break, ev_fill;
    double maxLikelihood, secondMaxLikelihood, prevlikelihood, likelihood;
};

struct FigState {
    int G, ncols;
    int left, right;
    int side_limit; long long end_pos_max;
    int valid_count, invalid_count, partial_read_count;
    double region_perct, region_perct_max;
    int partial_read_len, rep_flag, one_side_repeat_flag, large_gap_flag, comp_count;
    int left_max, right_min, discont_or_not;
    int psr_temp[2], psr_final[2];
    int umaxleftf, umaxrightf, ucoverf;
    int num_itr, overlap_threshold, gaptofill;
    int gl_len, gr_len, pl_len, pr_len;
    int cons_len, best_len, cur_len, prev_len, orig_len;
    unsigned char gap_left[32], gap_right[32];
    unsigned char partial_left[100], partial_right[100];
    double FP[6][5], FQ[6][5];
    double red_v[16]; int red_i[16];
    double bc_d; int bc_i, bc_j;
    int ibuf[8];
    double lik;
    int ctl[8];
    int tm_lo[16], tm_hi[16], tm_len[16], tm_tis0[16], tm_dir[16];
    int tm_aux[16]; long long tm_woff[16];
    double wv_v[32]; int wv_o[32];
    short sh_lo[FIG_SH_SC * FIG_SH_C], sh_hi[FIG_SH_SC * FIG_SH_C];
    int sh_tis0[FIG_SH_SC * FIG_SH_C];
    unsigned sh_woff[FIG_SH_SC * FIG_SH_C];
    unsigned char sh_len[FIG_SH_SC * FIG_SH_C], sh_aux[FIG_SH_SC * FIG_SH_C];
    unsigned sh_irr[16], sh_pad;
    int mle_next, pad_mn;
    int fin_i[8];
    FigLoop L;
    unsigned long long flops_useful; int n_place, sup_any;
    int dbg_j, sup_origin;
};

struct FigTrip { int v[3]; };



struct FigScr {
    double *cnt;
    double *ncnt;
    double *tmp;
    int *pc;
    int *nci;
    unsigned char *accf;
    unsigned char *mdone;
    int *cov;
    int *region;
    unsigned char *cons, *best, *cur, *prev, *orig;
    unsigned char *colchar;
    unsigned char *mark, *saved;
    double *maxlv;
    int *frp;
    int *org;
    int *fin;
    FigTrip *sortbuf;
    int *hint;
    int *hint_e;
    double *hval;
    int *repeatflag;
    int *ppos_org;
    int *pflag;
    int *prf;
    int *lcross, *rcross; unsigned char *smflag;
    int *used_read_arr; int *lrmd;
    FigPQ *pqg; double *q4g;
    double *wg;
};

FIG_HD long long fig_align8(long long x) { return (x + 15) & ~15LL; }

FIG_HD long long fig_scratch_layout(unsigned char *base, int capG, int capR, int capP, int capC, int capW, int capE, FigScr *s) {
    long long o = 0;
#define FIG_CARVE(field, type, count) do { if (s) s->field = (type *)(base + o); o = fig_align8(o + (long long)sizeof(type) * (count)); } while (0)
    FIG_CARVE(cnt, double, 5LL * capG);
    FIG_CARVE(ncnt, double, 5LL * capG);
    FIG_CARVE(tmp, double, 5LL * capG);
    FIG_CARVE(pqg, FigPQ, 4LL * capE);
    FIG_CARVE(q4g, double, capE);
    FIG_CARVE(wg, double, capW);
    FIG_CARVE(maxlv, double, capR > capP ? capR : capP);
    FIG_CARVE(hval, double, capR);
    FIG_CARVE(pc, int, 4LL * capG);
    FIG_CARVE(nci, int, 5LL * capG);
    FIG_CARVE(cov, int, capG);
    FIG_CARVE(region, int, 2LL * capG + 16);
    FIG_CARVE(frp, int, 2LL * capR);
    FIG_CARVE(org, int, 2LL * capR);
    FIG_CARVE(fin, int, 2LL * capR);
    FIG_CARVE(sortbuf, FigTrip, capR);
    FIG_CARVE(hint, int, capR);
    FIG_CARVE(hint_e, int, capR);
    FIG_CARVE(repeatflag, int, 3LL * capP);
    FIG_CARVE(ppos_org, int, 3LL * capP);
    FIG_CARVE(pflag, int, 2LL * capP);
    FIG_CARVE(prf, int, 3LL * capP);
    FIG_CARVE(lcross, int, capP);
    FIG_CARVE(rcross, int, capP);
    FIG_CARVE(used_read_arr, int, capC);
    FIG_CARVE(lrmd, int, 2LL * capC);
    FIG_CARVE(cons, unsigned char, capG + 8);
    FIG_CARVE(best, unsigned char, capG + 8);
    FIG_CARVE(cur, unsigned char, capG + 8);
    FIG_CARVE(prev, unsigned char, capG + 8);
    FIG_CARVE(orig, unsigned char, capG + 8);
    FIG_CARVE(colchar, unsigned char, capG + 8);
    FIG_CARVE(mark, unsigned char, capR + 8);
    FIG_CARVE(saved, unsigned char, capR + 8);
    FIG_CARVE(accf, unsigned char, capR + 8);
    FIG_CARVE(mdone, unsigned char, capR + 8);
    FIG_CARVE(smflag, unsigned char, capP + 8);
#undef FIG_CARVE
    return o;
}

struct FigEng {
    int tid, nt;
    const FigDevModel *M;
    const FigDevBatch *B;
    const FigDevGap *g;
    FigState *S;
    FigScr scr;
    FigPQ *pq; double *q4;
    int ncolE, xoff;
    int off_pq, off_q4, off_w;
    int off_plb;
    int pq_lds, w_lds;
    int lds_tw;
    int tiles, tile_step, tile_cols;
    double *wbuf;
    int Wcap, nteams;
    int sh_on;
    int lane, wave, nw, wsz;
    const double *kt_fwd, *kt_rev;
    const double *mt_fwd, *mt_rev;
    unsigned char *rb;
    uint32_t *plb;
    unsigned char *gs;
    int capG;
    unsigned long long flops;
    unsigned long long mle_alg;
    unsigned long long mle_exec;
    unsigned long long wait_cycles;
    unsigned long long prof[FIG_PROF_SLOTS];
};

FIG_D void fig_eng_ident(FigEng &E, unsigned tid, unsigned nt, unsigned wsz) {
    E.tid = (int)tid; E.nt = (int)nt;
    E.lane = (int)(tid % wsz); E.wave = (int)(tid / wsz); E.nw = (int)((nt + wsz - 1) / wsz); E.wsz = (int)wsz;
}

struct FigKernArgs { int capG, capGl, ncolE, Wcap, nteams, q_begin, q_end, qsel, tiles, tile_step, tile_cols, tiled_max, sh_on;
                     int cont = 0, minc = 16, cont_live = 100, cont_prio = 1; };

FIG_D long long fig_eng_carve(FigEng &E, const FigDevModel &M, const FigKernArgs &A, bool lds_tab) {
    E.capG = A.capG;
    E.ncolE = A.ncolE; E.xoff = M.L - 1; E.Wcap = A.Wcap; E.nteams = A.nteams; E.sh_on = A.sh_on;
    long long off = 0;
    E.pq_lds = lds_tab; E.w_lds = lds_tab;
    E.tiles = A.tiles; E.tile_step = A.tile_step; E.tile_cols = A.tile_cols;
    if (lds_tab && A.tiles > 0) {
        E.pq_lds = 0;
        E.off_pq = 0; E.off_q4 = 8 * A.tile_cols; E.off_w = 9 * A.tile_cols;
        off = 9LL * A.tile_cols + (long long)A.nteams * A.Wcap;
        { const long long mle = FIG_TILED_MLE_DOUBLES(A.ncolE, (int)E.nw); if (mle > off && mle <= A.tiled_max) off = mle; }
        E.pq = E.scr.pqg; E.q4 = E.scr.q4g; E.wbuf = E.scr.wg;
    } else if (lds_tab) {
        E.off_pq = 0; E.off_q4 = 8 * A.ncolE; E.off_w = 9 * A.ncolE;
        off = 9LL * A.ncolE + (long long)A.nteams * A.Wcap;
        E.pq = (FigPQ *)(fig_lds + E.off_pq); E.q4 = fig_lds + E.off_q4; E.wbuf = fig_lds + E.off_w;
    } else {
        E.off_pq = E.off_q4 = E.off_w = 0;
        E.pq = E.scr.pqg; E.q4 = E.scr.q4g; E.wbuf = E.scr.wg;
    }
    E.S = (FigState *)(fig_lds + off); E.lds_tw = (int)off;
    unsigned char *bp = (unsigned char *)(E.S + 1);
    E.gs = bp; bp += ((A.capGl + 7) & ~7);
    E.rb = bp; bp += ((FIG_MAX_READLEN + 8 + 15) & ~15);
    E.plb = (uint32_t *)bp; E.off_plb = (int)((double *)bp - fig_lds);
    E.kt_fwd = M.ome; E.kt_rev = M.ome + 2 * M.L; E.mt_fwd = M.ome + 4 * M.L; E.mt_rev = M.ome + 6 * M.L;
    return off * 8 + (long long)sizeof(FigState) + ((A.capGl + 7) & ~7) + ((FIG_MAX_READLEN + 8 + 15) & ~15) + FIG_PLB_BYTES;
}

FIG_D int fig_read_code(const uint32_t *packed, long long woff, int len, int j) {
    int nw2 = (len + 15) >> 4;
    uint32_t w = packed[woff + (j >> 4)];
    uint32_t m = packed[woff + nw2 + (j >> 5)];
    int c = (w >> ((j & 15) * 2)) & 3;
    return ((m >> (j & 31)) & 1) ? 4 : c;
}

FIG_D int fig_flank_l(const FigEng &E, int k) {
    if (k > FIG_FLANK) return 4;
    return ((fig_gcu8p)E.B->flank)[E.g->flankOff + (k - 1)];
}
FIG_D int fig_flank_r(const FigEng &E, int k) {
    if (k >= FIG_FLANK) return 4;
    return ((fig_gcu8p)E.B->flank)[E.g->flankOff + FIG_FLANK + k];
}

FIG_D void fig_stage_read(FigEng &E, const FigDevReads &R, long long idx) {
    int len = R.len[idx];
    long long woff = R.woff[idx];
    for (int j = E.tid; j < len; j += E.nt) E.rb[j] = (unsigned char)fig_read_code(E.B->packed, woff, len, j);
}

FIG_D int fig_load_read(const FigEng &E, const FigDevReads &R, long long idx, unsigned char *dst) {
    int len = R.len[idx];
    long long woff = R.woff[idx];
    for (int j = 0; j < len; j++) dst[j] = (unsigned char)fig_read_code(E.B->packed, woff, len, j);
    return len;
}

struct FigBest { double v; int o; };

FIG_D int fig_ovl(int o, int len, int G) { int a = o > 0 ? o : 0, b = o + len < G ? o + len : G; return b > a ? b - a : 0; }

FIG_D FigBest fig_best_merge(FigBest a, FigBest b) {
    if (b.o == FIG_NOPOS) return a;
    if (a.o == FIG_NOPOS) return b;
    if (b.v > a.v || (b.v == a.v && b.o < a.o)) return b;
    return a;
}

FIG_D FigBest fig_block_best(FigEng &E, FigBest x) {
#ifdef FIG_EMU
    return x;
#else
    for (int off = 32; off > 0; off >>= 1) {
        FigBest y;
        y.v = __shfl_down(x.v, off, 64);
        y.o = __shfl_down(x.o, off, 64);
        x = fig_best_merge(x, y);
    }
    int wave = E.tid >> 6, nw = (E.nt + 63) >> 6;
    if (nw == 1) {
        x.v = __shfl(x.v, 0, 64);
        x.o = __shfl(x.o, 0, 64);
        return x;
    }
    FIG_SYNC();
    if ((E.tid & 63) == 0) { E.S->red_v[wave] = x.v; E.S->red_i[wave] = x.o; }
    FIG_SYNC();
    FigBest r; r.v = E.S->red_v[0]; r.o = E.S->red_i[0];
    for (int w = 1; w < nw; w++) { FigBest y; y.v = E.S->red_v[w]; y.o = E.S->red_i[w]; r = fig_best_merge(r, y); }
    return r;
#endif
}

FIG_D void fig_ise(FigEng &E) {
    FigState &S = *E.S;
    long long gs = E.g->gapStart, cl = E.g->contigLen;
    if (gs - S.left < 0) { S.left = (int)gs; if (S.side_limit > S.left) S.side_limit = S.left; }
    if (gs + S.G + S.right > cl) { S.right = (int)(cl - (gs + S.G)); if (S.side_limit > S.right) S.side_limit = S.right; }
    long long endPos = gs + S.G + S.right;
    if (endPos > S.end_pos_max) S.end_pos_max = endPos;
    S.ncols = S.G;
}

FIG_D void fig_flank_tables(FigEng &E) {
    FigState &S = *E.S;
    for (int c = 0; c < 6; c++) {
        double cnt[5] = {0, 0, 0, 0, 0};
        if (c < 5) cnt[c] = 1;
        double total = 0;
        for (int j = 0; j < 5; j++) total = total + cnt[j];
        double Ncount = cnt[4];
        double pr[5];
        for (int j = 0; j < 4; j++) pr[j] = (c < 5) ? ((cnt[j] + (Ncount / 4)) / total) : 0.0;
        pr[4] = 0;
        for (int j = 0; j < 5; j++) {
            double sum = 0;
            for (int k = 0; k < 4; k++) { if (j == k) continue; sum += pr[k] * E.M->T[k * 5 + j]; }
            S.FQ[c][j] = (c < 5) ? sum : 0.0;
            S.FP[c][j] = pr[j];
        }
    }
}

FIG_D int fig_col_kind(const FigEng &E, int x, int G, int left, int right) {
    if (x < 0) { if (x < -left) return -1; return fig_flank_l(E, -x); }
    if (x < G) return 6;
    if (x < G + right) return fig_flank_r(E, x - G);
    return 5;
}
FIG_D int fig_from_code(const FigEng &E, int x, int G, int left, int right) {
    if (x < 0) { if (x < -left) return 4; return fig_flank_l(E, -x); }
    if (x < G) return ((fig_lcu8p)E.gs)[x];
    if (x < G + right) return fig_flank_r(E, x - G);
    return 4;
}

FIG_D int fig_from_code_u(fig_gcu8p fl, fig_lcu8p gs, int x, int G, int left, int right) {
    if (x < 0) { if (x < -left) return 4; const int k = -x; return k > FIG_FLANK ? 4 : fl[k - 1]; }
    if (x < G) return gs[x];
    if (x < G + right) { const int k = x - G; return k >= FIG_FLANK ? 4 : fl[FIG_FLANK + k]; }
    return 4;
}

#define FIG_PQ(E, b, x) ((E).pq[(long long)(b) * (E).ncolE + (x) + (E).xoff])
#define FIG_Q4(E, x) ((E).q4[(x) + (E).xoff])
#ifdef FIG_EMU
FIG_D void fig_pq_set(const FigEng &E, int b, int x, FigPQ v) { FIG_PQ(E, b, x) = v; }
FIG_D FigPQ fig_pq_get(const FigEng &E, int b, int x) { return FIG_PQ(E, b, x); }
FIG_D void fig_pq_set_p(const FigEng &E, int b, int x, double v) { FIG_PQ(E, b, x).p = v; }
FIG_D void fig_pq_set_q(const FigEng &E, int b, int x, double v) { FIG_PQ(E, b, x).q = v; }
FIG_D double fig_pq_get_p(const FigEng &E, int b, int x) { return FIG_PQ(E, b, x).p; }
FIG_D void fig_q4_set(const FigEng &E, int x, double v) { FIG_Q4(E, x) = v; }
FIG_D double fig_q4_get(const FigEng &E, int x) { return FIG_Q4(E, x); }
#else
typedef double fig_d2v __attribute__((ext_vector_type(2)));
typedef fig_d2v __attribute__((address_space(3))) *fig_ld2p;
typedef fig_d2v __attribute__((address_space(1))) *fig_gd2p;
typedef double __attribute__((address_space(3))) *fig_ldp;
FIG_D void fig_pq_set(const FigEng &E, int b, int x, FigPQ v) {
    const long long i = (long long)b * E.ncolE + x + E.xoff;
    fig_d2v t; t.x = v.p; t.y = v.q;
    if (E.pq_lds) ((fig_ld2p)(fig_lds + E.off_pq))[i] = t; else ((fig_gd2p)E.pq)[i] = t;
}
FIG_D FigPQ fig_pq_get(const FigEng &E, int b, int x) {
    const long long i = (long long)b * E.ncolE + x + E.xoff;
    fig_d2v t;
    if (E.pq_lds) t = ((fig_ld2p)(fig_lds + E.off_pq))[i]; else t = ((fig_gd2p)E.pq)[i];
    FigPQ v; v.p = t.x; v.q = t.y;
    return v;
}
FIG_D void fig_pq_set_p(const FigEng &E, int b, int x, double v) {
    const long long i = (long long)b * E.ncolE + x + E.xoff;
    if (E.pq_lds) ((fig_ldp)(fig_lds + E.off_pq))[2 * i] = v; else ((fig_gdp)(double *)E.pq)[2 * i] = v;
}
FIG_D void fig_pq_set_q(const FigEng &E, int b, int x, double v) {
    const long long i = (long long)b * E.ncolE + x + E.xoff;
    if (E.pq_lds) ((fig_ldp)(fig_lds + E.off_pq))[2 * i + 1] = v; else ((fig_gdp)(double *)E.pq)[2 * i + 1] = v;
}
FIG_D double fig_pq_get_p(const FigEng &E, int b, int x) {
    const long long i = (long long)b * E.ncolE + x + E.xoff;
    if (E.pq_lds) return ((fig_ldp)(fig_lds + E.off_pq))[2 * i];
    return ((fig_gdp)(double *)E.pq)[2 * i];
}
FIG_D void fig_q4_set(const FigEng &E, int x, double v) {
    if (E.pq_lds) ((fig_ldp)(fig_lds + E.off_q4))[x + E.xoff] = v; else ((fig_gdp)E.q4)[x + E.xoff] = v;
}
FIG_D double fig_q4_get(const FigEng &E, int x) {
    if (E.pq_lds) return ((fig_ldp)(fig_lds + E.off_q4))[x + E.xoff];
    return ((fig_gdp)E.q4)[x + E.xoff];
}
#endif

FIG_D void fig_build_flank_pq(FigEng &E) {
    const FigState &S = *E.S;
    int G = S.G, left = S.left, right = S.right, L1 = E.xoff;
    int n = 2 * L1;
    for (int i = E.tid; i < n; i += E.nt) {
        int x = i < L1 ? i - L1 : G + (i - L1);
        if (x + E.xoff >= E.ncolE) continue;
        int c;
        if (x < 0) c = (-x <= left) ? fig_flank_l(E, -x) : 5;
        else c = (x - G < right) ? fig_flank_r(E, x - G) : 5;
        for (int b = 0; b < 4; b++) { FigPQ v; v.p = S.FP[c][b]; v.q = S.FQ[c][b]; fig_pq_set(E, b, x, v); }
        fig_q4_set(E, x, S.FQ[c][4]);
    }
}

FIG_D void fig_compute_probs(FigEng &E) {
    int n = E.S->ncols, cg = E.capG;
    const double *T = E.M->T;
    for (int x = E.tid; x < n; x += E.nt) {
        double c0 = E.scr.cnt[x], c1 = E.scr.cnt[cg + x], c2 = E.scr.cnt[2 * cg + x], c3 = E.scr.cnt[3 * cg + x], c4 = E.scr.cnt[4 * cg + x];
        double total = 0;
        total = total + c0; total = total + c1; total = total + c2; total = total + c3; total = total + c4;
        double pr[4];
        if (total) {
            double nq = c4 / 4;
            pr[0] = (c0 + nq) / total; pr[1] = (c1 + nq) / total; pr[2] = (c2 + nq) / total; pr[3] = (c3 + nq) / total;
        } else { pr[0] = pr[1] = pr[2] = pr[3] = .25; }
        for (int j = 0; j < 5; j++) {
            double sum = 0;
            for (int k = 0; k < 4; k++) { if (j == k) continue; sum += pr[k] * T[k * 5 + j]; }
            if (j < 4) { FigPQ v; v.p = pr[j]; v.q = sum; fig_pq_set(E, j, x, v); }
            else fig_q4_set(E, x, sum);
        }
    }
    fig_build_flank_pq(E);
}
FIG_D void fig_compute_errprobs_only(FigEng &E) {
    int n = E.S->ncols;
    const double *T = E.M->T;
    for (int x = E.tid; x < n; x += E.nt) {
        double pr[4];
        for (int j = 0; j < 4; j++) pr[j] = fig_pq_get_p(E, j, x);
        for (int j = 0; j < 5; j++) {
            double sum = 0;
            for (int k = 0; k < 4; k++) { if (j == k) continue; sum += pr[k] * T[k * 5 + j]; }
            if (j < 4) fig_pq_set_q(E, j, x, sum); else fig_q4_set(E, x, sum);
        }
    }
    fig_build_flank_pq(E);
}

FIG_D void fig_compute_sequence(FigEng &E, int check, int choice) {
    int n = E.S->ncols, cg = E.capG;
    const double *A = choice == 0 ? E.scr.cnt : E.scr.ncnt;
    for (int x = E.tid; x < n; x += E.nt) {
        double mx = 0; int mi = -1;
        for (int j = 0; j <= 4; j++) { double v = A[j * cg + x]; if (v > mx) { mx = v; mi = j; } }
        int coverage_flag = 1;
        if (check == 1) { int cv = (int)mx; E.scr.cov[x] = cv; if (cv <= 0) coverage_flag = 0; }
        unsigned char c = 4;
        if (((mi != -1) || (!check)) && coverage_flag) c = (mi >= 0 && mi <= 3) ? (unsigned char)mi : 4;
        E.scr.cons[x] = c;
    }
    if (E.tid == 0) E.S->cons_len = n < 0 ? 0 : n;
    FIG_SYNC();
}

FIG_D void fig_copy_str(FigEng &E, unsigned char *dst, int *dlen, const unsigned char *src, int slen) {
    for (int x = E.tid; x < slen; x += E.nt) dst[x] = src[x];
    if (E.tid == 0) *dlen = slen;
    FIG_SYNC();
}

FIG_D bool fig_tlt(const FigTrip &a, const FigTrip &b) { return a.v[0] < b.v[0]; }
FIG_D void fig_tswap(FigTrip &a, FigTrip &b) { FigTrip t = a; a = b; b = t; }

FIG_D void fig_adjust_heap(FigTrip *first, int holeIndex, int len, FigTrip value) {
    int topIndex = holeIndex, secondChild = holeIndex;
    while (secondChild < (len - 1) / 2) {
        secondChild = 2 * (secondChild + 1);
        if (fig_tlt(first[secondChild], first[secondChild - 1])) secondChild--;
        first[holeIndex] = first[secondChild];
        holeIndex = secondChild;
    }
    if ((len & 1) == 0 && secondChild == (len - 2) / 2) {
        secondChild = 2 * (secondChild + 1);
        first[holeIndex] = first[secondChild - 1];
        holeIndex = secondChild - 1;
    }
    int parent = (holeIndex - 1) / 2;
    while (holeIndex > topIndex && fig_tlt(first[parent], value)) {
        first[holeIndex] = first[parent];
        holeIndex = parent;
        parent = (holeIndex - 1) / 2;
    }
    first[holeIndex] = value;
}
FIG_D void fig_heapsort(FigTrip *first, int n) {
    if (n < 2) return;
    for (int parent = (n - 2) / 2;; parent--) { FigTrip v = first[parent]; fig_adjust_heap(first, parent, n, v); if (parent == 0) break; }
    for (int last = n; last > 1; last--) { FigTrip v = first[last - 1]; first[last - 1] = first[0]; fig_adjust_heap(first, 0, last - 1, v); }
}
FIG_D void fig_unguarded_linear_insert(FigTrip *a, int last) {
    FigTrip val = a[last];
    int next = last - 1;
    while (fig_tlt(val, a[next])) { a[last] = a[next]; last = next; next--; }
    a[last] = val;
}
FIG_D void fig_insertion_sort(FigTrip *a, int first, int last) {
    if (first == last) return;
    for (int i = first + 1; i != last; ++i) {
        if (fig_tlt(a[i], a[first])) { FigTrip val = a[i]; for (int k = i; k > first; k--) a[k] = a[k - 1]; a[first] = val; }
        else fig_unguarded_linear_insert(a, i);
    }
}
FIG_D void fig_std_sort(FigTrip *a, int n) {
    if (n <= 0) return;
    int lg = 0; { int t = n; while (t > 1) { t >>= 1; lg++; } }
    int stack_f[64], stack_l[64], stack_d[64], sp = 0;
    stack_f[0] = 0; stack_l[0] = n; stack_d[0] = lg * 2; sp = 1;
    while (sp > 0) {
        sp--;
        int first = stack_f[sp], last = stack_l[sp], depth = stack_d[sp];
        while (last - first > 16) {
            if (depth == 0) { fig_heapsort(a + first, last - first); break; }
            --depth;
            int mid = first + (last - first) / 2;
            {
                int A = first + 1, Bm = mid, C = last - 1;
                if (fig_tlt(a[A], a[Bm])) {
                    if (fig_tlt(a[Bm], a[C])) fig_tswap(a[first], a[Bm]);
                    else if (fig_tlt(a[A], a[C])) fig_tswap(a[first], a[C]);
                    else fig_tswap(a[first], a[A]);
                } else if (fig_tlt(a[A], a[C])) fig_tswap(a[first], a[A]);
                else if (fig_tlt(a[Bm], a[C])) fig_tswap(a[first], a[C]);
                else fig_tswap(a[first], a[Bm]);
            }
            int lo = first + 1, hi = last;
            while (true) {
                while (fig_tlt(a[lo], a[first])) ++lo;
                --hi;
                while (fig_tlt(a[first], a[hi])) --hi;
                if (!(lo < hi)) break;
                fig_tswap(a[lo], a[hi]);
                ++lo;
            }
            int cut = lo;
            if (sp < 63) { stack_f[sp] = first; stack_l[sp] = cut; stack_d[sp] = depth; sp++; }
            first = cut;
        }
    }
    if (n > 16) { fig_insertion_sort(a, 0, 16); for (int i = 16; i != n; ++i) fig_unguarded_linear_insert(a, i); }
    else fig_insertion_sort(a, 0, n);
}

#include "fig_engine_core.h"

#endif
```

figbird_amd/csrc/fig_engine_sched.h:

```cpp
#ifndef FIG_ENGINE_SCHED_H
#define FIG_ENGINE_SCHED_H

template <bool LDS>
FIG_D void fig_gap_begin(FigEng &E) {
    FigState &S = *E.S;
    const FigDevModel &M = *E.M;
    const FigDevGap &g = *E.g;
    int G0 = g.G0, nU = g.nU;
    if (E.tid == 0) {
        S.left = M.D; S.right = M.D; S.side_limit = 30; S.end_pos_max = 0;
        S.valid_count = S.invalid_count = 0;
        S.partial_read_count = M.partial_flag == 1 ? g.nP : 0;
        S.region_perct = 0; S.region_perct_max = 0;
        S.partial_read_len = M.partial_len;
        S.rep_flag = 0; S.one_side_repeat_flag = 0; S.large_gap_flag = g.lgf; S.comp_count = 0;
        S.left_max = 0; S.right_min = 0; S.discont_or_not = 0;
        S.psr_temp[0] = S.psr_temp[1] = S.psr_final[0] = S.psr_final[1] = -1;
        S.umaxleftf = S.umaxrightf = S.ucoverf = 0;
        S.num_itr = 0; S.overlap_threshold = (E.B->ot_preset && E.B->ot_preset[g.gapNo]) ? 5 : 0; S.gaptofill = 0;
        S.gl_len = S.gr_len = S.pl_len = S.pr_len = 0;
        S.cons_len = 1; E.scr.cons[0] = 4;
        E.scr.used_read_arr[0] = 0;
        S.best_len = S.cur_len = S.prev_len = S.orig_len = 0;
        S.flops_useful = 0; S.n_place = 0; S.dbg_j = -1; S.sup_origin = FIG_ORG_NONE;
        fig_flank_tables(E);
        if (E.B->dbg_n_cand) E.B->dbg_n_cand[g.gapNo] = 0;
        if (E.B->draw_len) { E.B->draw_len[(long long)g.gapNo * 2] = -1; E.B->draw_len[(long long)g.gapNo * 2 + 1] = -1; }
    }
    for (int r = E.tid; r < nU; r += E.nt) {
        E.scr.saved[r] = 0; E.scr.mark[r] = 0; E.scr.org[r * 2] = -200; E.scr.org[r * 2 + 1] = 0;
        E.scr.frp[r * 2] = -200; E.scr.frp[r * 2 + 1] = 0;
        if (E.B->draw_pos) E.B->draw_pos[g.uBase + r] = (int)0x80000000;
    }
    for (int p = E.tid; p < g.nP; p += E.nt) {
        E.scr.ppos_org[p * 3] = 0; E.scr.ppos_org[p * 3 + 1] = -200; E.scr.ppos_org[p * 3 + 2] = 0;
        if (E.B->draw_pos) E.B->draw_pos[E.B->n_ureads + g.pBase + p] = (int)0x80000000;
    }
    FIG_SYNC();
    if (E.tid == 0) {
        S.G = G0; fig_ise(E);
        int n = 0;
        for (int k = S.side_limit; k >= 1; k--) S.gap_left[n++] = (unsigned char)fig_flank_l(E, k);
        S.gl_len = n;
        n = 0;
        for (int k = 0; k < S.right && n < S.side_limit; k++) {
            long long abs = g.gapStart + G0 + k;
            S.gap_right[n++] = (unsigned char)(abs < g.contigLen ? fig_flank_r(E, k) : 255);
        }
        S.gr_len = n;
    }
    FIG_SYNC();
    fig_find_repeat(E);
    if (E.tid == 0) {
        FigLoop &L = S.L;
        float gp_frac1 = g.gpf1, gp_frac2 = g.gpf2;
        int skip = 0;
        if (S.rep_flag == 1 && M.partial_flag) skip = 1;
        else if (S.one_side_repeat_flag == 1 && M.partial_flag && G0 > 3 * (2 * M.partial_len)) skip = 1;
        else if (g.fillflag == -1) skip = 1;
        else if (S.partial_read_count == 0 && nU == 0) skip = 1;
        int inr = !skip;
        if (inr && g.gapNo > (M.script_itr == 1 ? 765466 : 965757)) inr = 0;
        S.num_itr = inr ? 200 : 0;
        if (!inr) { gp_frac1 = 1; gp_frac2 = 1; }
        int gapMin = (int)(G0 * gp_frac1), gapMax = (int)(G0 * gp_frac2);
        L.inr = inr; L.gapMin = gapMin; L.gapEstimate = gapMin; L.maxGapEstimate = gapMin; L.j = 0;
        L.maxLikelihood = -FIG_DBL_MAX; L.secondMaxLikelihood = -FIG_DBL_MAX; L.likelihood = 0; L.prevlikelihood = 0;
        L.fill_or_not = 0; L.same_count = 0; L.same_thresh = M.unmapped ? 50 : 4; L.stuckCount = 0;
        int range = gapMax - gapMin + 1;
        if (range > E.B->capC) range = E.B->capC;
        L.range = range; L.side_flag = 0; L.less_read_flag = 0;
        L.prev_best = -1; L.curr_best = 0; L.prev_u = -1; L.curr_u = 0; L.sec_same = 0; L.sec_same2 = 0;
        L.done = 0; L.need_orig = 0; L.ev_iters = 0; L.ev_side_break = 0; L.ev_fill = 0;
        L.finalize_flag = 1;
        if (M.unmapped && S.large_gap_flag == 0) L.finalize_flag = 0;
    }
    FIG_SYNC();
    if (M.unmapped && G0 <= M.unm_limit && S.L.inr) {
        int lrf = fig_check_gap_reads<LDS>(E, G0);
        if (E.tid == 0) {
            S.L.less_read_flag = lrf;
            if (lrf == 1) S.L.range = 0;
            if (lrf == -2) { S.L.side_flag = 1; S.L.range = 0; }
        }
    }
    if (E.tid == 0 && S.L.range <= 0) S.L.done = 1;
    FIG_SYNC();
}

template <bool LDS>
FIG_D int fig_gap_probe(FigEng &E) {
    fig_gap_begin<LDS>(E);
    FigState &S = *E.S;
    if (S.L.range <= 0) return 0;
    int fill = fig_initialize(E, S.L.gapEstimate, 0);
    if (S.side_limit < 10) return 0;
    if (S.one_side_repeat_flag == 1) fill = 0;
    return !(fill != 0 && S.L.inr);
}

template <bool LDS>
FIG_D void fig_eval_candidate(FigEng &E) {
    FigState &S = *E.S;
    const FigDevModel &M = *E.M;
    const int G0 = E.g->G0;
    const int gapEstimate = S.L.gapEstimate, j = S.L.j, inr = S.L.inr, finalize_flag = S.L.finalize_flag;
    FIG_SYNC();
    FIG_T0(E);
    if (E.tid == 0) { S.umaxleftf = S.umaxrightf = S.ucoverf = 0; S.L.ev_side_break = 0; S.L.ev_iters = 0; S.dbg_j = j; }
    int fill = fig_initialize(E, gapEstimate, j);
    FIG_TICK(E, 35);
    if (S.side_limit < 10) { if (E.tid == 0) { S.L.ev_side_break = 1; S.L.ev_fill = fill; S.dbg_j = -1; } FIG_SYNC(); return; }
    if (S.one_side_repeat_flag == 1) fill = 0;
    if (E.tid == 0) S.L.ev_fill = fill;
    if (fill != 0 && inr) { if (E.tid == 0) S.dbg_j = -1; FIG_SYNC(); return; }
    int i = 0;
    if (E.tid == 0) { S.discont_or_not = 0; S.comp_count = 0; S.overlap_threshold = 5; S.lik = S.L.likelihood; }
    FIG_SYNC();
    int preset_unfilled_len = 2 * M.read_length;
    for (i = 0; i < S.num_itr; i++) {
        if (E.tid == 0) { S.valid_count = 0; S.invalid_count = 0; }
        FIG_SYNC();
        fig_place_reads<LDS>(E, i, finalize_flag, gapEstimate - G0, S.large_gap_flag);
        FIG_TICK(E, 38);
        fig_compute_probs(E);
        FIG_SYNC();
        FIG_TICK(E, 36);
        if (M.unmapped) {
            if (S.comp_count >= 5) break;
            if (S.large_gap_flag == 1 && S.region_perct * gapEstimate < preset_unfilled_len) break;
        } else { if (i == 2) break; }
    }
    if (M.unmapped && !finalize_flag && inr) {
        if (E.tid == 0) S.valid_count = 0;
        FIG_SYNC();
        fig_place_reads<LDS>(E, i, 1, gapEstimate - G0, 0);
    }
    fig_compute_sequence(E, 0, 0);
    if (E.tid == 0) { S.L.likelihood = S.lik; S.L.ev_iters = i; S.dbg_j = -1; }
    FIG_SYNC();
    FIG_TICK(E, 37);
}

FIG_D void fig_loop_step(FigEng &E) {
    FigState &S = *E.S;
    const FigDevModel &M = *E.M;
    const int G0 = E.g->G0, nU = E.g->nU;
    FIG_SYNC();
    if (S.L.ev_side_break) { if (E.tid == 0) { S.L.side_flag = 1; S.L.fill_or_not = S.L.ev_fill; S.L.done = 1; } FIG_SYNC(); return; }
    if (S.L.ev_fill != 0 && S.L.inr) { if (E.tid == 0) { S.L.fill_or_not = S.L.ev_fill; S.L.done = 1; } FIG_SYNC(); return; }
    const int j = S.L.j, gapEstimate = S.L.gapEstimate;
    const double likelihood = S.L.likelihood;
    const int valid_count = S.valid_count;
    const bool newbest = likelihood > S.L.maxLikelihood;
    if (E.tid == 0) fig_dbg_cand(E, gapEstimate, S.L.ev_iters, valid_count, likelihood);
    if (newbest) {
        fig_copy_str(E, E.scr.best, &S.best_len, E.scr.cons, S.cons_len);
        for (int k = E.tid; k < nU; k += E.nt) E.scr.saved[k] = E.scr.mark[k];
    }
    if (gapEstimate == G0) fig_copy_str(E, E.scr.orig, &S.orig_len, E.scr.cons, S.cons_len);
    FIG_SYNC();
    if (E.tid == 0) {
        FigLoop &L = S.L;
        L.fill_or_not = L.ev_fill;
        if (newbest) {
            L.secondMaxLikelihood = L.maxLikelihood;
            L.maxLikelihood = likelihood;
            L.maxGapEstimate = gapEstimate;
            S.region_perct_max = S.region_perct; S.psr_final[0] = S.psr_temp[0]; S.psr_final[1] = S.psr_temp[1];
            L.curr_best = j;
            L.prev_u = valid_count;
        } else if (likelihood > L.secondMaxLikelihood) L.secondMaxLikelihood = likelihood;
        if (j < E.B->capC) { E.scr.used_read_arr[j] = valid_count; E.scr.lrmd[j * 2] = S.left; E.scr.lrmd[j * 2 + 1] = S.right; }
        int brk = 0, need = 0;
        if (M.partial_flag || M.unmapped) {
            double diff1 = L.prevlikelihood - likelihood; if (diff1 < 0) diff1 = -diff1;
            if (diff1 <= 0.9) L.same_count++; else L.same_count = 0;
            L.prevlikelihood = likelihood;
            const int st = L.same_thresh;
            if (L.same_count == st) { brk = 1; need = S.G < G0; }
            if (!brk && M.unmapped) {
                L.curr_u = valid_count;
                int du = L.curr_u - L.prev_u; if (du < 0) du = -du;
                if (L.curr_best == L.prev_best && du <= 2) L.sec_same++;
                else { L.prev_best = L.curr_best; L.sec_same = 0; }
                if (L.sec_same >= 2 * st) { brk = 1; need = S.G < G0; }
                if (!brk && G0 <= 30) {
                    if (!(S.umaxleftf == 1 || S.umaxrightf == 1 || S.ucoverf == 1)) L.sec_same2++; else L.sec_same2 = 0;
                    if (L.sec_same2 >= 1.5 * st) { brk = 1; need = S.G < G0; }
                }
                if (!brk) {
                    if (S.discont_or_not == 1 && valid_count < 5) L.stuckCount++; else L.stuckCount = 0;
                    if (L.stuckCount > 3 * st) { brk = 1; need = S.G < G0; }
                }
            }
        }
        if (brk) { L.done = 1; L.need_orig = need; }
        else { L.gapEstimate++; L.j++; if (L.j >= L.range) L.done = 1; }
    }
    FIG_SYNC();
}

template <bool LDS>
FIG_D void fig_gap_end(FigEng &E) {
    FigState &S = *E.S;
    const FigDevModel &M = *E.M;
    const FigDevGap &g = *E.g;
    const int G0 = g.G0;
    FIG_SYNC();
    if (S.L.need_orig) fig_run_original<LDS>(E, E.scr.orig, &S.orig_len);
    const FigLoop L = S.L;
    FIG_SYNC();
    if (L.fill_or_not != 0 && L.inr) {
        if (E.tid == 0) { S.G = 0; S.gaptofill = L.fill_or_not; }
    } else if (L.inr) {
        if (M.unmapped) {
            if (L.less_read_flag == 1) {
                fig_run_original<LDS>(E, E.scr.orig, &S.orig_len);
                fig_finalize<LDS>(E, G0);
            } else if (L.side_flag) {
                fig_run_original<LDS>(E, E.scr.best, &S.best_len);
                fig_finalize<LDS>(E, G0);
            } else {
                int changed = 0;
                if (L.j != 1) for (int i = 1; i < L.j && i < E.B->capC; i++) if (E.scr.used_read_arr[0] != E.scr.used_read_arr[i]) { changed = 1; break; }
                if (changed) fig_finalize<LDS>(E, L.maxGapEstimate);
                else { fig_copy_str(E, E.scr.best, &S.best_len, E.scr.orig, S.orig_len); fig_finalize<LDS>(E, G0); }
            }
        } else {
            if (L.maxGapEstimate == 0) {
                if (E.scr.used_read_arr[0] != 0) fig_finalize<LDS>(E, L.maxGapEstimate);
                else {
                    if (L.maxGapEstimate < G0) fig_run_original<LDS>(E, E.scr.orig, &S.orig_len);
                    fig_finalize<LDS>(E, G0);
                }
            } else {
                if (L.side_flag) {
                    int idx = L.maxGapEstimate - L.gapMin;
                    if (E.tid == 0 && idx >= 0 && idx < E.B->capC) { S.left = E.scr.lrmd[idx * 2]; S.right = E.scr.lrmd[idx * 2 + 1]; }
                    FIG_SYNC();
                }
                fig_finalize<LDS>(E, L.maxGapEstimate);
            }
        }
    }
    FIG_SYNC();
    int len = S.G;
    const char A[5] = {'A', 'C', 'G', 'T', 'N'};
    char *dst = E.B->str + g.strOff;
    for (int x = E.tid; x < len && x < g.alloc_arg; x += E.nt) {
        int c = x < S.cons_len ? E.scr.cons[x] : 4;
        dst[x] = A[c > 4 ? 4 : c];
    }
    if (E.B->sup_counts) {
        const int org = S.sup_origin, cg = E.capG;
        int32_t *sup = E.B->sup_counts + g.strOff * 5;
        if (E.tid == 0) S.sup_any = 0;
        FIG_SYNC();
        int any = 0;
        for (int i = E.tid; i < 5 * len && i < 5 * g.alloc_arg; i += E.nt) {
            const int x = i / 5, b = i - 5 * x;
            const int32_t v = (org != FIG_ORG_NONE && x < S.cons_len && x < cg) ? (int32_t)E.scr.cnt[b * cg + x] : 0;
            sup[i] = v; any |= v;
        }
        if (any) S.sup_any = 1;
        FIG_SYNC();
        if (E.tid == 0) E.B->sup_origin[g.gapNo] = S.sup_any ? org : FIG_ORG_NONE;
    }
    if (E.tid == 0) {
        E.B->filled_len[g.gapNo] = len; E.B->gaptofill[g.gapNo] = S.gaptofill;
        fig_atomic_add_u64(&E.B->counters[FIG_CNT_PLACE], (unsigned long long)S.n_place);
        if (E.B->dbg_n_place) E.B->dbg_n_place[g.gapNo] = S.n_place;
        if (S.flops_useful) fig_atomic_add_u64(&E.B->counters[FIG_CNT_FLOPS], S.flops_useful);
    }
    FIG_SYNC();
}

template <bool LDS>
FIG_D void fig_fill_gap(FigEng &E) {
    fig_gap_begin<LDS>(E);
    while (!E.S->L.done) {
        fig_eval_candidate<LDS>(E);
        fig_loop_step(E);
    }
    fig_gap_end<LDS>(E);
}


struct FigSlot {
    double lik, region_perct;
    long long end_pos_max;
    unsigned long long flops;
    int G, iters, valid, side_break, fill, flags, psr0, psr1, left, right, side_limit, cons_len, partial_read_len, partial_read_count, n_place, prev_len;
};

struct FigPersist {
    unsigned char *state;
    unsigned char *best, *orig, *prev, *saved;
    int *org, *ppos_org, *repeatflag, *used_read_arr, *lrmd, *org_spec, *ppos_spec;
    unsigned char *slots; long long slot_stride;
};

FIG_HD long long fig_persist_layout(unsigned char *base, int capGg, int nU, int nP, int range, int nslots, size_t state_bytes, FigPersist *p) {
    long long o = 0;
#define FIG_PC(field, type, count) do { if (p) p->field = (type *)(base + o); o = fig_align8(o + (long long)sizeof(type) * (count)); } while (0)
    FIG_PC(state, unsigned char, (long long)state_bytes);
    FIG_PC(best, unsigned char, capGg + 8);
    FIG_PC(orig, unsigned char, capGg + 8);
    FIG_PC(prev, unsigned char, capGg + 8);
    FIG_PC(saved, unsigned char, nU + 8);
    FIG_PC(org, int, 2LL * nU + 2);
    FIG_PC(ppos_org, int, 3LL * nP + 3);
    FIG_PC(repeatflag, int, 3LL * nP + 3);
    FIG_PC(used_read_arr, int, range + 2);
    FIG_PC(lrmd, int, 2LL * range + 4);
    FIG_PC(org_spec, int, 2LL * nU + 2);
    FIG_PC(ppos_spec, int, 3LL * nP + 3);
    long long stride = fig_align8((long long)sizeof(FigSlot)) + 2 * fig_align8(capGg + 8) + fig_align8(nU + 8);
    if (p) { p->slots = base + o; p->slot_stride = stride; }
    o += stride * nslots;
#undef FIG_PC
    return o;
}

FIG_D FigSlot *fig_slot_hdr(const FigPersist &P, int s) { return (FigSlot *)(P.slots + P.slot_stride * s); }
FIG_D unsigned char *fig_slot_cons(const FigPersist &P, int s) { return P.slots + P.slot_stride * s + fig_align8((long long)sizeof(FigSlot)); }
FIG_D unsigned char *fig_slot_prev(const FigPersist &P, int s, int capGg) { return fig_slot_cons(P, s) + fig_align8(capGg + 8); }
FIG_D unsigned char *fig_slot_mark(const FigPersist &P, int s, int capGg) { return fig_slot_cons(P, s) + 2 * fig_align8(capGg + 8); }

FIG_D void fig_state_save(FigEng &E, const FigPersist &P) {
    FIG_SYNC();
    const int n = (int)(sizeof(FigState) / 4);
    const int *src = (const int *)E.S; int *dst = (int *)P.state;
    for (int i = E.tid; i < n; i += E.nt) dst[i] = src[i];
    FIG_SYNC();
}
FIG_D void fig_state_load(FigEng &E, const FigPersist &P) {
    FIG_SYNC();
    const int n = (int)(sizeof(FigState) / 4);
    int *dst = (int *)E.S; const int *src = (const int *)P.state;
    for (int i = E.tid; i < n; i += E.nt) dst[i] = src[i];
    FIG_SYNC();
}

enum { FIG_BIND_SEQ = 0, FIG_BIND_EVAL = 1, FIG_BIND_REPLAY = 2 };
FIG_D void fig_bind(FigEng &E, const FigScr &work, const FigPersist &P, int mode, int slot, int capGg) {
    E.scr = work;
    E.scr.best = P.best; E.scr.orig = P.orig; E.scr.saved = P.saved;
    E.scr.repeatflag = P.repeatflag; E.scr.used_read_arr = P.used_read_arr; E.scr.lrmd = P.lrmd;
    E.scr.org = P.org; E.scr.ppos_org = P.ppos_org;
    if (mode == FIG_BIND_SEQ) { E.scr.prev = P.prev; }
    else {
        E.scr.cons = fig_slot_cons(P, slot); E.scr.mark = fig_slot_mark(P, slot, capGg);
        if (mode == FIG_BIND_EVAL) { E.scr.org = P.org_spec; E.scr.ppos_org = P.ppos_spec; }
    }
}

#define FIG_PSR_UNSET (-2)

template <bool LDS>
FIG_D void fig_spec_eval(FigEng &E, const FigScr &work, const FigPersist &P, int j, int slot, int capGg) {
    FIG_T0(E);
    fig_bind(E, work, P, FIG_BIND_EVAL, slot, capGg);
    fig_state_load(E, P);
    FIG_TICK(E, 34);
    FigState &S = *E.S;
    const unsigned long long flops0 = E.flops;
    if (E.tid == 0) {
        fig_slot_hdr(P, slot)->flops = 0; S.n_place = 0;
        S.L.j = j; S.L.gapEstimate = S.L.gapMin + j;
        S.psr_temp[0] = S.psr_temp[1] = FIG_PSR_UNSET;
        if (j != 0) S.prev_len = 0;
    }
    FIG_SYNC();
    if (j == 0) for (int x = E.tid; x < S.prev_len; x += E.nt) E.scr.prev[x] = P.prev[x];
    FIG_SYNC();
    fig_eval_candidate<LDS>(E);
    FIG_TICK(E, 26);
    if (E.tid == 0) {
        FigSlot *h = fig_slot_hdr(P, slot);
        h->lik = S.L.likelihood; h->region_perct = S.region_perct; h->end_pos_max = S.end_pos_max;
        h->G = S.L.gapEstimate; h->iters = S.L.ev_iters; h->valid = S.valid_count; h->side_break = S.L.ev_side_break; h->fill = S.L.ev_fill;
        h->flags = (S.umaxleftf ? 1 : 0) | (S.umaxrightf ? 2 : 0) | (S.ucoverf ? 4 : 0) | (S.discont_or_not ? 8 : 0);
        h->psr0 = S.psr_temp[0]; h->psr1 = S.psr_temp[1];
        h->left = S.left; h->right = S.right; h->side_limit = S.side_limit; h->cons_len = S.cons_len;
        h->partial_read_len = S.partial_read_len; h->partial_read_count = S.partial_read_count; h->n_place = S.n_place; h->prev_len = S.prev_len;
    }
    FIG_SYNC();
    {
        unsigned char *pv = fig_slot_prev(P, slot, capGg);
        for (int x = E.tid; x < S.prev_len; x += E.nt) pv[x] = E.scr.prev[x];
    }
    {
        unsigned long long d = E.flops - flops0;
#ifndef FIG_EMU
        for (int off = 32; off > 0; off >>= 1) d += fig_shfl_down_u64(d, off);
        if (E.lane != 0) d = 0;
#endif
        if (d) { fig_atomic_add_u64(&fig_slot_hdr(P, slot)->flops, d); fig_atomic_add_u64(&E.B->counters[FIG_CNT_SPEC], d); }
    }
    E.flops = flops0;
    FIG_SYNC();
    FIG_TICK(E, 39);
}

FIG_D void fig_spec_replay(FigEng &E, const FigScr &work, const FigPersist &P, int n, int capGg) {
    fig_bind(E, work, P, FIG_BIND_REPLAY, 0, capGg);
    fig_state_load(E, P);
    FigState &S = *E.S;
    const int G0 = E.g->G0, nU = E.g->nU, nP = E.g->nP;
    for (int s = 0; s < n && !S.L.done; s++) {
        fig_bind(E, work, P, FIG_BIND_REPLAY, s, capGg);
        const FigSlot *h = fig_slot_hdr(P, s);
        if (E.tid == 0) {
            S.L.likelihood = h->lik; S.region_perct = h->region_perct; S.end_pos_max = h->end_pos_max;
            S.G = h->G; S.ncols = h->G; S.L.ev_iters = h->iters; S.valid_count = h->valid; S.L.ev_side_break = h->side_break; S.L.ev_fill = h->fill;
            S.umaxleftf = h->flags & 1; S.umaxrightf = (h->flags >> 1) & 1; S.ucoverf = (h->flags >> 2) & 1; S.discont_or_not = (h->flags >> 3) & 1;
            if (h->psr0 != FIG_PSR_UNSET || h->psr1 != FIG_PSR_UNSET) { S.psr_temp[0] = h->psr0; S.psr_temp[1] = h->psr1; }
            S.left = h->left; S.right = h->right; S.side_limit = h->side_limit; S.cons_len = h->cons_len;
            S.partial_read_len = h->partial_read_len; S.partial_read_count = h->partial_read_count;
            S.n_place += h->n_place; S.flops_useful += h->flops;
            if (!h->side_break && !(h->fill != 0 && S.L.inr)) S.overlap_threshold = 5;
        }
        FIG_SYNC();
        if (h->G == G0 && !h->side_break && !(h->fill != 0 && S.L.inr)) {
            for (int i = E.tid; i < 2 * nU; i += E.nt) P.org[i] = P.org_spec[i];
            for (int i = E.tid; i < 3 * nP; i += E.nt) P.ppos_org[i] = P.ppos_spec[i];
        }
        if (!h->side_break && !(h->fill != 0 && S.L.inr) && S.num_itr > 0) {
            const unsigned char *pv = fig_slot_prev(P, s, capGg);
            for (int x = E.tid; x < h->prev_len; x += E.nt) P.prev[x] = pv[x];
            if (E.tid == 0) S.prev_len = h->prev_len;
        }
        fig_loop_step(E);
    }
    fig_state_save(E, P);
}

FIG_D void fig_persist_of(const FigDevBatch &B, const FigDevGap &g, FigPersist &P) {
    fig_persist_layout(B.persist + g.persistOff, g.capGg, g.nU, g.nP, g.rangeCap, g.nslots, sizeof(FigState), &P);
}

FIG_D void fig_item_gap(FigEng &E, const FigScr &work, int gi, FigPersist &P) {
    E.g = &E.B->gaps[gi];
    fig_persist_of(*E.B, *E.g, P);
    fig_bind(E, work, P, FIG_BIND_SEQ, 0, E.g->capGg);
}

FIG_D FigGapCtl &fig_ctl_of(const FigEng &E, int gi) { return *(E.B->gapctl + gi); }
FIG_D void fig_ctl_publish(const FigEng &E, int gi) {
    if (E.tid != 0) return;
    FigGapCtl &c = fig_ctl_of(E, gi);
    c.status = E.S->L.done ? FIG_GAP_LOOP_DONE : FIG_GAP_MORE; c.j = E.S->L.j; c.range = E.S->L.range;
}

template <bool LDS>
FIG_D void fig_item_fill(FigEng &E, const FigScr &work, int gi) {
    FigPersist P; fig_item_gap(E, work, gi, P);
    fig_fill_gap<LDS>(E);
}

template <bool LDS>
FIG_D void fig_item_begin(FigEng &E, const FigScr &work, int gi) {
    FigPersist P; fig_item_gap(E, work, gi, P);
    fig_gap_begin<LDS>(E);
    if (!E.S->L.inr) {
        while (!E.S->L.done) { fig_eval_candidate<LDS>(E); fig_loop_step(E); }
        fig_gap_end<LDS>(E);
        if (E.tid == 0) fig_ctl_of(E, gi).status = FIG_GAP_FINISHED;
    } else {
        fig_state_save(E, P);
        fig_ctl_publish(E, gi);
    }
    FIG_SYNC();
}

template <bool LDS>
FIG_D void fig_item_probe(FigEng &E, const FigScr &work, int gi) {
    FigPersist P; fig_item_gap(E, work, gi, P);
    const int reach = fig_gap_probe<LDS>(E);
    if (E.tid == 0) fig_ctl_of(E, gi).reach = reach;
    FIG_SYNC();
}

template <bool LDS>
FIG_D void fig_item_eval(FigEng &E, const FigScr &work, const FigItem &it) {
    E.g = &E.B->gaps[it.gap];
    FigPersist P; fig_persist_of(*E.B, *E.g, P);
    fig_spec_eval<LDS>(E, work, P, it.j, it.slot, E.g->capGg);
    FIG_SYNC();
}

FIG_D void fig_item_replay(FigEng &E, const FigScr &work, const FigEntry &en) {
    E.g = &E.B->gaps[en.gap];
    FigPersist P; fig_persist_of(*E.B, *E.g, P);
    fig_spec_replay(E, work, P, en.n, E.g->capGg);
    fig_ctl_publish(E, en.gap);
}

template <bool LDS>
FIG_D void fig_item_end(FigEng &E, const FigScr &work, int gi) {
    FigPersist P; fig_item_gap(E, work, gi, P);
    fig_state_load(E, P);
    fig_gap_end<LDS>(E);
    if (E.tid == 0) fig_ctl_of(E, gi).status = FIG_GAP_FINISHED;
    FIG_SYNC();
}


FIG_HD int fig_cont_chunk(int minc, int last, int slots, int left) {
    int n = last > minc ? last : minc;
    if (n > slots) n = slots;
    if (n > left) n = left;
    return n;
}

FIG_D void fig_item_continue(FigEng &E, const FigScr &work, int gi, int n, int minc, FigCont &next) {
    fig_item_replay(E, work, FigEntry{gi, n, 0, 0});
    FIG_SYNC();
    const FigLoop &L = E.S->L;
    next.gap = gi; next.next = 0; next.ready = 0; next.pad = 0;
    if (L.done) { next.kind = FIG_CONT_END; next.j0 = 0; next.n = 1; next.rank = 1; }
    else {
        const int left = L.range - L.j;
        next.kind = FIG_CONT_EVAL; next.j0 = L.j; next.n = fig_cont_chunk(minc, n, E.g->nslots, left);
        next.rank = (left + next.n - 1) / (next.n > 0 ? next.n : 1);
    }
    FIG_SYNC();
}
#endif
```

figbird_amd/csrc/fig_pack.h:

```cpp
#ifndef FIG_PACK_H
#define FIG_PACK_H
#include <algorithm>
#include <cstdlib>
#include <cstring>
#include <vector>
#include "../../include/figbird_hip.h"
#include "fig_types.h"
#include "fig_gaprules.h"

static inline int code_of(char c) {
    switch (c) { case 'A': return 0; case 'C': return 1; case 'G': return 2; case 'T': return 3; default: return 4; }
}

static void pack_read(const char *s, int len, std::vector<uint32_t> &out) {
    int nw2 = (len + 15) >> 4, nwm = (len + 31) >> 5, nwp = ((len + 3) >> 2) + 4;
    size_t base = out.size();
    out.resize(base + nw2 + nwm + 2 + nwp, 0u);
    int cnt[5] = {0, 0, 0, 0, 0};
    for (int j = 0; j < len; j++) {
        int c = code_of(s[j]);
        if (c < 4) out[base + (j >> 4)] |= (uint32_t)c << ((j & 15) * 2);
        else out[base + nw2 + (j >> 5)] |= 1u << (j & 31);
        cnt[c]++;
    }
    uint8_t *cb = (uint8_t *)&out[base + nw2 + nwm];
    for (int c = 0; c < 5; c++) cb[c] = (uint8_t)cnt[c];
    uint8_t *pl = (uint8_t *)&out[base + nw2 + nwm + 2];
    int k = 0;
    for (int c = 0; c < 5; c++) {
        for (int j = len - 1; j >= 0; j--) if (code_of(s[j]) == c) pl[k++] = (uint8_t)j;
        k = (k + 3) & ~3;
    }
}

static inline double fig_model_fmm(const fig_model *m) {
    double emax = 0, tmax = 0;
    for (int k = 0; k < m->max_read_length; k++) emax = std::max(emax, m->error_pos_dist[k]);
    for (int from = 0; from < 5; from++) for (int to = 0; to < 4; to++) if (from != to) tmax = std::max(tmax, m->error_type_probs[from * 5 + to]);
    for (int k = 0; k < m->max_read_length; k++) {
        const double e = m->error_pos_dist[k], m3 = 1 - e - m->in_pos_dist[k] - m->del_pos_dist[k];
        if (!(e >= 0 && e <= 1 && m3 >= 0 && m3 <= 1)) return 2.0;
    }
    for (int i = 0; i < 25; i++) if (!(m->error_type_probs[i] >= 0 && m->error_type_probs[i] <= 1)) return 2.0;
    double f = emax * tmax * (1.0 + 1e-9);
    if (!(f > 0)) f = 1.0;
    return f < 1.0 ? f : 1.0;
}

#define FIG_SPLIT_MIN_GAPS 96
struct FigLaunchClass { int capG, capGl, ncolE, Wcap, nteams, nt; bool lds_tab; size_t lds; int q_begin, q_end;
                        int tiles, tile_step, tile_cols, tiled_max;
                        int nsplit; };

struct FigPacked {
    std::vector<FigDevGap> gaps;
    std::vector<int32_t> order;
    std::vector<uint8_t> flank, qual;
    std::vector<uint32_t> packed;
    std::vector<int32_t> u_pos, u_aux, u_len, p_pos, p_aux, p_clip, p_ref, p_len;
    std::vector<int64_t> u_woff, p_woff, p_qoff, str_off;
    std::vector<FigLaunchClass> classes;
    std::vector<uint8_t> ot_preset;
    bool ot_given = false;
    int capR = 1, capP = 1, capC = 1, capG = 8, capW = 0, capE = 0;
    int64_t str_total = 0, n_gaps = 0, persist_total = 0, stream_total = 0;
    int nslots = 64;
    int64_t packed_bytes() const {
        return (int64_t)(packed.size() * 4 + flank.size() + gaps.size() * sizeof(FigDevGap) + qual.size() +
                         (u_pos.size() * 3 + p_pos.size() * 5) * 4 + (u_woff.size() + p_woff.size() + p_qoff.size()) * 8);
    }
};

static int fig_pack(const fig_model *m, const fig_gap_batch *b, size_t state_bytes, FigPacked &K) {
    int64_t ng = b->n_gaps;
    if (ng < 0) return FIG_EINVAL;
    if (ng > 0 && (!b->gap_contig || !b->gap_start || !b->gap_len || !b->contig_off || !b->contig_seq || !b->p_read_off)) return FIG_EINVAL;
    if (m->unmapped_flag && ng > 0 && !b->u_read_off) return FIG_EINVAL;
    if (ng > 0) {
        if (b->p_read_off[0] < 0 || (m->unmapped_flag && b->u_read_off[0] < 0)) return FIG_EINVAL;
        for (int64_t g = 0; g < ng; g++) {
            if (b->p_read_off[g + 1] < b->p_read_off[g]) return FIG_EINVAL;
            if (m->unmapped_flag && b->u_read_off[g + 1] < b->u_read_off[g]) return FIG_EINVAL;
        }
        if (b->p_read_off[ng] > 0 && (!b->p_seq_off || !b->p_seq || !b->p_pos || !b->p_match || !b->p_clipped_index || !b->p_ref_pos)) return FIG_EINVAL;
        if (m->unmapped_flag && b->u_read_off[ng] > 0 && (!b->u_seq_off || !b->u_seq || !b->u_anchor_pos || !b->u_is_reverse)) return FIG_EINVAL;
    }
    if (m->max_distance < m->max_read_length) return FIG_EUNSUP;
    K.n_gaps = ng;
    K.gaps.assign(ng, FigDevGap());
    K.flank.assign((size_t)ng * 2 * FIG_FLANK, 4);
    K.str_off.assign(ng + 1, 0);
    std::vector<double> cost(ng, 0.0);
    int64_t str_total = 0;
    for (int64_t g = 0; g < ng; g++) {
        FigDevGap &d = K.gaps[g];
        int ci = b->gap_contig[g];
        if (ci < 0 || ci >= b->n_contigs) return FIG_EINVAL;
        int64_t c0 = b->contig_off[ci], c1 = b->contig_off[ci + 1];
        d.contigLen = c1 - c0; d.gapStart = b->gap_start[g]; d.G0 = b->gap_len[g];
        if (d.G0 < 1 || d.gapStart < 0 || d.gapStart + d.G0 > d.contigLen) return FIG_EINVAL;
        d.stat2 = b->gap_stat2 ? b->gap_stat2[g * 3 + 1] : 0;
        d.stat3 = b->gap_stat2 ? b->gap_stat2[g * 3 + 2] : 0;
        d.fillflag = b->gap_fillflag ? b->gap_fillflag[g] : 1;
        gap_alloc(m, d.G0, &d.alloc_arg, &d.gpf1, &d.gpf2, &d.lgf);
        if (d.alloc_arg < d.G0) d.alloc_arg = d.G0;
        d.gapNo = (int32_t)g;
        d.flankOff = g * 2 * FIG_FLANK;
        uint8_t *fl = &K.flank[(size_t)d.flankOff];
        const char *cs = b->contig_seq + c0;
        for (int k = 1; k <= FIG_FLANK; k++) { int64_t a = d.gapStart - k; fl[k - 1] = a >= 0 ? (uint8_t)code_of(cs[a]) : 4; }
        for (int k = 0; k < FIG_FLANK; k++) { int64_t a = d.gapStart + d.G0 + k; fl[FIG_FLANK + k] = a < d.contigLen ? (uint8_t)code_of(cs[a]) : 4; }
        d.strOff = str_total; K.str_off[g] = str_total; str_total += d.alloc_arg + 1;
        d.uBase = (int64_t)K.u_pos.size(); d.nU = 0;
        if (m->unmapped_flag) {
            int64_t r0 = b->u_read_off[g], r1 = b->u_read_off[g + 1];
            int64_t n = r1 - r0;
            if (n > FIG_READ_CAP) n = FIG_READ_CAP;
            for (int64_t r = r0; r < r0 + n; r++) {
                int len = (int)(b->u_seq_off[r + 1] - b->u_seq_off[r]);
                if (len > FIG_MAX_READLEN || len > m->max_read_length || len < 1) return FIG_EUNSUP;
                K.u_pos.push_back(b->u_anchor_pos[r]);
                {
                    int hasN = 0;
                    const char *rs_ = b->u_seq + b->u_seq_off[r];
                    for (int q = 0; q < len; q++) if (code_of(rs_[q]) > 3) { hasN = 1; break; }
                    K.u_aux.push_back((b->u_is_reverse[r] ? 1 : 0) | (hasN << 1));
                }
                K.u_len.push_back(len);
                K.u_woff.push_back((int64_t)K.packed.size());
                pack_read(b->u_seq + b->u_seq_off[r], len, K.packed);
            }
            d.nU = (int32_t)n;
        }
        d.pBase = (int64_t)K.p_pos.size(); d.nP = 0;
        {
            int64_t r0 = b->p_read_off[g], r1 = b->p_read_off[g + 1];
            int64_t n = r1 - r0;
            if (n > FIG_READ_CAP + 1) n = FIG_READ_CAP + 1;
            for (int64_t r = r0; r < r0 + n; r++) {
                int len = (int)(b->p_seq_off[r + 1] - b->p_seq_off[r]);
                if (len > FIG_MAX_READLEN || len > m->max_read_length || len < 1) return FIG_EUNSUP;
                { const char *rs_ = b->p_seq + b->p_seq_off[r]; for (int q = 0; q < len; q++) if (code_of(rs_[q]) > 3) { d.pad |= 1; break; } }
                K.p_pos.push_back(b->p_pos[r]); K.p_aux.push_back(b->p_match[r]); K.p_clip.push_back(b->p_clipped_index[r]);
                K.p_ref.push_back(b->p_ref_pos[r]); K.p_len.push_back(len);
                K.p_woff.push_back((int64_t)K.packed.size());
                pack_read(b->p_seq + b->p_seq_off[r], len, K.packed);
                K.p_qoff.push_back((int64_t)K.qual.size());
                if (b->p_qual) K.qual.insert(K.qual.end(), b->p_qual + b->p_seq_off[r], b->p_qual + b->p_seq_off[r] + len);
                else K.qual.insert(K.qual.end(), (size_t)len, (uint8_t)'I');
            }
            d.nP = (int32_t)n;
        }
        K.capR = std::max(K.capR, d.nU); K.capP = std::max(K.capP, d.nP);
        int range = gap_range(d.G0, d.gpf1, d.gpf2);
        K.capC = std::max(K.capC, range);
        K.capG = std::max(K.capG, d.alloc_arg);
        double L = m->max_read_length;
        if (m->unmapped_flag) cost[g] = (double)d.nU * std::min<double>(d.alloc_arg + L, 2200.0) * L * (d.lgf ? 2.0 : range * (d.G0 <= m->unm_limit / 3 ? 10.5 : 11.5));
        else cost[g] = (double)d.nP * L * L * range * 3.0;
        if (d.fillflag == -1) cost[g] = 1;
    }
    K.str_total = str_total; K.str_off[ng] = str_total;
    {
        int64_t so = 0;
        for (int64_t g = 0; g < ng; g++) {
            K.gaps[g].streamOff = so;
            so += (int64_t)((K.gaps[g].nU + FIG_SH_C - 1) / FIG_SH_C) * m->max_read_length * (FIG_SH_C / 2);
        }
        K.stream_total = so + FIG_SH_C;
    }
    K.capG = (K.capG + 7) & ~7;
    {
        K.ot_given = b->gap_ot_preset != nullptr;
        K.ot_preset.assign((size_t)std::max<int64_t>(ng, 1), 0);
        for (int64_t g = 0; g < ng; g++) if (b->gap_ot_preset) K.ot_preset[(size_t)g] = b->gap_ot_preset[g] ? 1 : 0;
    }
    std::vector<int> gmax(ng, 8);
    for (int64_t g = 0; g < ng; g++) {
        const FigDevGap &d = K.gaps[g];
        int gm = std::max(d.G0, (int)(d.G0 * d.gpf2));
        if (m->unmapped_flag && d.G0 <= m->unm_limit) gm = std::max(gm, d.G0 < 30 ? 70 : 3 * d.G0);
        gmax[g] = std::min(gm, d.alloc_arg);
    }
    {
        long long off = 0;
        for (int64_t g = 0; g < ng; g++) {
            FigDevGap &d = K.gaps[g];
            d.capGg = (gmax[g] + 7) & ~7; d.rangeCap = gap_range(d.G0, d.gpf1, d.gpf2); d.nslots = K.nslots;
            d.persistOff = off;
            off += (fig_persist_layout(nullptr, d.capGg, d.nU, d.nP, d.rangeCap, d.nslots, state_bytes, nullptr) + 255) & ~255LL;
        }
        K.persist_total = off;
    }
    struct ClsDef { int capGl, nt; };
    const ClsDef defs[] = {{448, 256}, {1216, 512}, {1600, 512}, {1 << 30, 512}};
    K.order.clear(); K.classes.clear();
    const int L1 = m->max_read_length - 1;
    int prevcap = 0;
    for (const ClsDef &cd : defs) {
        std::vector<int32_t> ids;
        int mx = 8, mxa = 8;
        for (int64_t g = 0; g < ng; g++)
            if (gmax[g] > prevcap && gmax[g] <= cd.capGl) { ids.push_back((int32_t)g); mx = std::max(mx, gmax[g]); mxa = std::max(mxa, K.gaps[g].alloc_arg); }
        prevcap = cd.capGl;
        if (ids.empty()) continue;
        std::stable_sort(ids.begin(), ids.end(), [&](int32_t a, int32_t c) { return cost[a] > cost[c]; });
        FigLaunchClass c;
        c.capG = (mxa + 7) & ~7;
        c.capGl = (mx + 7) & ~7;
        c.ncolE = (c.capGl + 2 * L1 + 7) & ~7;
        c.Wcap = (c.capGl + m->max_read_length + 7) & ~7;
        c.nt = cd.nt;
        const size_t LDS_MAX = 160 * 1024 - 1024;
        size_t fixed = state_bytes + (size_t)c.capGl + FIG_MAX_READLEN + 64 + FIG_PLB_BYTES;
        int nw = c.nt / 64;
        c.lds_tab = false; c.nteams = nw;
        for (int nt_ = nw; nt_ >= 1; nt_ >>= 1) {
            size_t need = fixed + sizeof(double) * ((size_t)9 * c.ncolE + (size_t)nt_ * c.Wcap);
            if (need <= LDS_MAX) { c.lds_tab = true; c.nteams = nt_; c.lds = need; break; }
        }
        c.tiles = 0; c.tile_step = 0; c.tile_cols = 0; c.tiled_max = 0;
        if (!c.lds_tab) {
            c.lds = fixed + 64; c.nt = 512; c.nteams = 8;
            bool found = false;
            for (int nt_ = 4; nt_ >= 1 && !found; nt_ >>= 1)
                for (int ntl = 2; ntl <= 8 && !found; ntl++) {
                    int step = ((c.ncolE + ntl - 1) / ntl + 7) & ~7;
                    int tcols = (step + m->max_read_length + 8 + 7) & ~7;
                    size_t need = fixed + sizeof(double) * ((size_t)9 * tcols + (size_t)nt_ * c.Wcap);
                    if (need <= LDS_MAX) { found = true; c.tiles = ntl; c.tile_step = step; c.tile_cols = tcols; c.nteams = nt_; c.lds = need; }
                }
            if (found) {
                c.tiled_max = (int)((LDS_MAX - fixed) / sizeof(double));
                const long long mle = FIG_TILED_MLE_DOUBLES(c.ncolE, c.nt / 64);
                if (mle <= c.tiled_max && fixed + sizeof(double) * (size_t)mle > c.lds) c.lds = fixed + sizeof(double) * (size_t)mle;
            }
        }
        { const char *ev = getenv("FIG_CLASS_LANES");
          const int want = ev ? std::max(1, std::min(8, atoi(ev))) : 2;
          c.nsplit = (int)ids.size() >= (FIG_SPLIT_MIN_GAPS / 2) * want ? want : 1; }
        for (int part = 0; part < c.nsplit; part++) {
            c.q_begin = (int)K.order.size();
            for (size_t k = (size_t)part; k < ids.size(); k += (size_t)c.nsplit) { const int32_t id = ids[k]; K.gaps[id].cls = (int)K.classes.size(); K.order.push_back(id); }
            c.q_end = (int)K.order.size();
            K.classes.push_back(c);
        }
        K.capE = std::max(K.capE, c.ncolE);
        K.capW = std::max(K.capW, (c.tiles ? 8 : c.nteams) * c.Wcap + 1024);
        if (m->unmapped_flag && c.lds_tab && !c.tiles && c.nteams >= 4) K.capW = std::max(K.capW, FIG_SH_SC * FIG_SH_C * c.Wcap + 1024);
    }
    return FIG_OK;
}

static int64_t fig_pack_results_capacity(const fig_model *m, const fig_gap_batch *b) {
    int64_t tot = 0;
    for (int64_t g = 0; g < b->n_gaps; g++) {
        int a, lgf; float f1, f2;
        gap_alloc(m, b->gap_len[g], &a, &f1, &f2, &lgf);
        tot += std::max(a, b->gap_len[g]) + 1;
    }
    return tot;
}
#endif
```

figbird_amd/csrc/fig_types.h:

```cpp
#ifndef FIG_TYPES_H
#define FIG_TYPES_H
#include <stdint.h>

#define FIG_MAX_READLEN 200
#define FIG_READ_CAP 3000
#define FIG_MAX_GAP 100000
#define FIG_FLANK 208
#define FIG_DBL_MAX 1.7976931348623157e308
#define FIG_SH_C 32
#define FIG_SH_SC 4
#define FIG_SH_ONE 16
#define FIG_MLE_FB 208
#define FIG_TILED_MLE_DOUBLES(ncolE, nw) (7LL * (ncolE) + (long long)(nw) * FIG_MLE_FB + ((ncolE) + 15) / 16 + 16 + 8)

enum { FIG_ORG_NONE = 0, FIG_ORG_FINAL = 1, FIG_ORG_ORIGINAL = 2, FIG_ORG_TIEBREAK = 4 };

enum { FIG_GAP_FINISHED = 0, FIG_GAP_MORE = 1, FIG_GAP_LOOP_DONE = 2 };
struct FigGapCtl { int32_t status, j, range, reach; };

struct alignas(16) FigItem { int32_t gap, j, slot, chunk; };
struct alignas(16) FigEntry { int32_t gap, n, j_planned, stamped; };
static_assert(sizeof(FigGapCtl) == 16 && sizeof(FigItem) == 16 && sizeof(FigEntry) == 16, "control words are four int32: buffers and copies are sized by sizeof");
enum { FIG_CONT_EVAL = 0, FIG_CONT_END = 1 };
#define FIG_CONT_CAP_MAX 65535
struct alignas(16) FigCont { int32_t gap, j0, n, kind; int32_t next, ready, rank, pad; };
struct alignas(16) FigContHdr { int32_t tail, exited, pad[2]; };
static_assert(sizeof(FigCont) == 32 && sizeof(FigContHdr) == 16, "continuation records: buffers are sized by sizeof");

enum FigCounter {
    FIG_CNT_PLACE = 0,
    FIG_CNT_FLOPS = 1, FIG_CNT_SPEC = 2,
    FIG_CNT_MLE_ALG = 3, FIG_CNT_MLE_EXEC = 4,
    FIG_CNT_CONT = 5,
    FIG_CNT_PROF_LO = 8, FIG_CNT_WAIT = 30, FIG_CNT_WAVE = 31, FIG_CNT_PROF_HI = 32,
    FIG_CNT_N = 64
};
#define FIG_PROF_SLOTS 40
#define FIG_PROF_SPLIT 22

struct FigDevModel {
    int32_t L;
    int32_t Tmin, Tmax, cutoff;
    int32_t partial_flag, unmapped, script_itr, D, read_length, neg_overlap, partial_len, unm_limit;
    int32_t max_insert;
    double T[25];
    const double *e;
    const double *ome;
    const double *ome1;
    const double *m3;
    const double *insd;
    const double *qtab;
    double fmm_up;
};

struct FigDevGap {
    int64_t gapStart, contigLen;
    int32_t G0, stat2, stat3, fillflag;
    int32_t nU; int32_t nP;
    int64_t uBase, pBase;
    int32_t alloc_arg; float gpf1, gpf2; int32_t lgf;
    int64_t flankOff;
    int64_t strOff;
    int32_t gapNo; int32_t cls;
    int64_t persistOff;
    int32_t capGg, rangeCap, nslots, pad;
    int64_t streamOff;
};

struct FigDevReads {
    const int32_t *pos;
    const int32_t *aux;
    const int32_t *clip;
    const int32_t *refpos;
    const int32_t *len;
    const int64_t *woff;
    const int64_t *qoff;
};

struct FigDevBatch {
    int64_t n_gaps;
    const FigDevGap *gaps;
    const int32_t *order;
    FigDevReads u, p;
    const uint32_t *packed;
    const uint32_t *ustream;
    const uint8_t *qual;
    const uint8_t *flank;
    int32_t *filled_len, *gaptofill; char *str;
    int32_t dbg_max_cand; int32_t *dbg_n_cand; int32_t *dbg_cand_i; double *dbg_cand_lik; int32_t *dbg_n_place;
    int32_t *draw_pos, *draw_isz, *draw_len; int64_t n_ureads;
    int32_t dbg_plane_cols, dbg_plane_reads; double *dbg_counts, *dbg_read_maxlv;
    int32_t *queue_head;
    unsigned long long *counters;
    uint8_t *scratch; int64_t scratch_stride;
    int32_t capG, capR, capP, capC;
    int32_t capW, capE;
    uint8_t *persist;
    FigGapCtl *gapctl;
    int32_t *gap_pending; FigContHdr *cont_hdr; FigCont *cont; int32_t cont_cap;
    const uint8_t *ot_preset;
    int32_t *sup_counts, *sup_origin;
};

#endif
```

Baseline: 24.64.

## Widen continuation chunks per gap by growth or idle workgroups, with wider slot slabs

Adds a 'wide' scheduling mode in which each gap's speculative chunk can grow, either doubling per round or expanding to fill idle live workgroups. The per-gap slot count is raised up to FIG_SLOTS_WIDE, with the persistent slab sized to fit device memory. Chunks are narrowed to the number of live workgroups when they would otherwise be rejected, and an open-item counter tracks waiting work. The aim is to cut the number of serial rounds for long gaps, at the cost of more discarded speculative work and more persistent memory.

```diff
diff --git a/figbird_amd/csrc/fig_abi.hip b/figbird_amd/csrc/fig_abi.hip
--- a/figbird_amd/csrc/fig_abi.hip
+++ b/figbird_amd/csrc/fig_abi.hip
@@ -120,21 +120,40 @@
     __syncthreads();
     if (E.tid == 0) {
         bool ok = true;
+        int n = c.n, rank = c.rank;
         if (c.kind == FIG_CONT_EVAL) {
             const long long live = (long long)gridDim.x - fig_ld_relaxed(&B.cont_hdr->exited);
-            ok = live * 100 >= (long long)c.n * A.cont_live;
+            ok = live * 100 >= (long long)n * A.cont_live;
+            if (!ok && n > c.pad && A.cont_live > 0) {
+                const long long fit = live * 100 / A.cont_live;
+                if (fit >= c.pad && fit >= 1) { n = (int)(fit < n ? fit : n); rank = rank + 1; ok = true; atomicAdd(&B.counters[FIG_CNT_NARROW], 1ull); }
+            }
         }
         if (ok) {
             const int idx = atomicAdd(&B.cont_hdr->tail, 1);
             if (idx < B.cont_cap) {
                 FigCont *e = B.cont + idx;
-                e->gap = c.gap; e->j0 = c.j0; e->n = c.n; e->kind = c.kind; e->next = 0; e->rank = c.rank; e->pad = 0;
+                e->gap = c.gap; e->j0 = c.j0; e->n = n; e->kind = c.kind; e->next = 0; e->rank = rank; e->pad = 0;
+                atomicAdd(&B.cont_hdr->open, n);
                 __hip_atomic_store(&e->ready, 1, __ATOMIC_RELEASE, __HIP_MEMORY_SCOPE_AGENT);
                 if (c.kind == FIG_CONT_EVAL) atomicAdd(&B.counters[FIG_CNT_CONT], 1ull);
             }
         }
     }
     __syncthreads();
+}
+
+FIG_D int fig_cont_spare(FigEng &E, const FigDevBatch &B, const FigKernArgs &A, int n_items) {
+    if (E.tid == 0) {
+        const long long live = (long long)gridDim.x - fig_ld_relaxed(&B.cont_hdr->exited);
+        const long long popped = fig_ld_relaxed(B.queue_head + A.qsel), open = fig_ld_relaxed(&B.cont_hdr->open);
+        const long long waiting = (popped < n_items ? n_items - popped : 0) + (open > 0 ? open : 0);
+        E.S->bc_i = live > waiting ? (int)(live - waiting) : 0;
+    }
+    __syncthreads();
+    const int spare = E.S->bc_i;
+    __syncthreads();
+    return spare;
 }
 
 FIG_D bool fig_cont_pop(FigEng &E, const FigDevBatch &B, const FigKernArgs &A, FigCont &out, int &k) {
@@ -164,7 +183,7 @@
         __syncthreads();
         k = S.bc_j;
         __syncthreads();
-        if (k < B.cont[idx].n) { __threadfence(); out = B.cont[idx]; return true; }
+        if (k < B.cont[idx].n) { if (E.tid == 0) atomicSub(&B.cont_hdr->open, 1); __threadfence(); out = B.cont[idx]; return true; }
     }
     return false;
 }
@@ -179,7 +198,8 @@
         fig_item_eval<LDS_TAB>(E, work, it);
         if (A.cont && it.chunk > 0 && fig_chunk_finished(E, B, it.gap, it.chunk)) {
             FigCont nx;
-            fig_item_continue(E, work, it.gap, it.chunk, A.minc, nx);
+            const int spare = (A.wide & FIG_WIDE_IDLE) ? fig_cont_spare(E, B, A, n_items) : 0;
+            fig_item_continue(E, work, it.gap, it.chunk, A.minc, FigWide{A.wide, A.wide_base, A.wide_cap}, spare, nx);
             fig_cont_publish(E, B, A, nx);
         }
     };
@@ -257,7 +277,7 @@
 
 struct FigLane { hipStream_t stream = nullptr; hipEvent_t done = nullptr; int32_t *queue_head = nullptr; uint8_t *scratch = nullptr; FigItem *d_items = nullptr; FigEntry *d_entries = nullptr; size_t cap = 0;
                  FigGapCtl *h_ctl = nullptr; FigItem *h_items = nullptr; FigEntry *h_entries = nullptr; int qsel = 0;
-                 uint8_t *d_cont = nullptr; int cont_cap = 0; };
+                 uint8_t *d_cont = nullptr; int cont_cap = 0; int wide = 0; };
 
 struct fig_ctx {
     int device = 0;
@@ -278,7 +298,7 @@
     std::vector<DevBuf> bufs;
     int64_t n_gaps = 0, n_ureads = 0, n_preads = 0, str_total = 0;
     std::vector<int64_t> h_str_off;
-    int nslots = 32;
+    int nslots = 32, nslots_wide = 32;
     std::vector<FigLane> lanes;
     fig_stats stats;
     int sh_on = FIG_SH_SC;
@@ -401,9 +421,10 @@
 }
 
 template <bool LDS_TAB, int NT>
-static hipError_t launch_kind(fig_ctx *ctx, const fig_ctx::Cls &c, const FigDevBatch &db, hipStream_t stream, FigKind kind, int blocks, const void *list, int n, int qsel) {
+static hipError_t launch_kind(fig_ctx *ctx, const fig_ctx::Cls &c, const FigDevBatch &db, hipStream_t stream, FigKind kind, int blocks, const void *list, int n, int qsel, int wide) {
     FigKernArgs A = fig_kargs_of(c.c, qsel, ctx->sh_on);
-    if (kind == FIG_K_EVAL) { const FigKnobs &kn = ctx->fill_knobs; A.cont = kn.cont && db.cont_cap > 0; A.minc = kn.minc; A.cont_live = kn.cont_live; A.cont_prio = kn.cont_prio; }
+    if (kind == FIG_K_EVAL) { const FigKnobs &kn = ctx->fill_knobs; A.cont = kn.cont && db.cont_cap > 0; A.minc = kn.minc; A.cont_live = kn.cont_live; A.cont_prio = kn.cont_prio;
+                              A.wide = A.cont ? wide : 0; A.wide_base = ctx->nslots; A.wide_cap = ctx->nslots_wide; }
     switch (kind) {
         case FIG_K_FILL: return launch_one(fig_fill_kernel<LDS_TAB, NT>, c.c.lds, NT, blocks, stream, ctx->dm, db, A);
         case FIG_K_BEGIN: return launch_one(fig_begin_kernel<LDS_TAB, NT>, c.c.lds, NT, blocks, stream, ctx->dm, db, A);
@@ -414,28 +435,45 @@
     return hipErrorInvalidValue;
 }
 
-static hipError_t launch_any(fig_ctx *ctx, const fig_ctx::Cls &c, const FigDevBatch &db, hipStream_t stream, FigKind kind, int blocks, const void *list, int n, int qsel = 0) {
-    if (c.c.tiles > 0) return launch_kind<true, 512>(ctx, c, db, stream, kind, blocks, list, n, qsel);
-    if (c.c.lds_tab) return c.c.nt == 256 ? launch_kind<true, 256>(ctx, c, db, stream, kind, blocks, list, n, qsel) : launch_kind<true, 512>(ctx, c, db, stream, kind, blocks, list, n, qsel);
-    return launch_kind<false, 512>(ctx, c, db, stream, kind, blocks, list, n, qsel);
-}
-
-extern "C" int fig_batch_upload(fig_ctx *ctx, const fig_gap_batch *b) {
-    if (!ctx || !b) return FIG_EINVAL;
-    if (!ctx->have_model) return FIG_EINVAL;
-    hipSetDevice(ctx->device);
+static hipError_t launch_any(fig_ctx *ctx, const fig_ctx::Cls &c, const FigDevBatch &db, hipStream_t stream, FigKind kind, int blocks, const void *list, int n, int qsel = 0, int wide = 0) {
+    if (c.c.tiles > 0) return launch_kind<true, 512>(ctx, c, db, stream, kind, blocks, list, n, qsel, wide);
+    if (c.c.lds_tab) return c.c.nt == 256 ? launch_kind<true, 256>(ctx, c, db, stream, kind, blocks, list, n, qsel, wide) : launch_kind<true, 512>(ctx, c, db, stream, kind, blocks, list, n, qsel, wide);
+    return launch_kind<false, 512>(ctx, c, db, stream, kind, blocks, list, n, qsel, wide);
+}
+
+static int fig_upload_once(fig_ctx *ctx, const fig_gap_batch *b, int wide_cap, int wide_asked) {
     free_batch(ctx);
     const fig_model *m = &ctx->hm;
     hipEventRecord(ctx->ev0, ctx->stream);
     FigPacked K;
+    const FigKnobs up_knobs = fig_knobs_from_env(0);
+    K.nslots_wide = std::max(K.nslots, wide_cap);
     int prc = fig_pack(m, b, sizeof(FigState), K);
     if (prc) return prc;
+    void *persist_mem = nullptr;
+    const int wide_first = K.nslots_wide;
+    K.nslots_wide = K.nslots; fig_pack_persist(K, sizeof(FigState));
+    const int64_t persist_base = K.persist_total;
+    K.nslots_wide = wide_first; fig_pack_persist(K, sizeof(FigState));
+    size_t mem_free = 0, mem_total = 0;
+    if (hipMemGetInfo(&mem_free, &mem_total) != hipSuccess) mem_free = 0;
+    while (true) {
+        const bool fits = (size_t)K.persist_total + 256 <= mem_free / 4 || K.nslots_wide <= K.nslots;
+        if (fits && hipMalloc(&persist_mem, (size_t)K.persist_total + 256) == hipSuccess) break;
+        persist_mem = nullptr; (void)hipGetLastError();
+        if (K.nslots_wide <= K.nslots) return FIG_ENOMEM;
+        K.nslots_wide = std::max(K.nslots, K.nslots_wide / 2);
+        fig_pack_persist(K, sizeof(FigState));
+    }
+    { DevBuf pb; pb.p = persist_mem; ctx->bufs.push_back(pb); }
     int64_t ng = K.n_gaps;
     ctx->h_order = K.order; ctx->h_str_off = K.str_off;
     ctx->str_total = K.str_total; ctx->n_gaps = ng;
     ctx->n_ureads = (int64_t)K.u_pos.size(); ctx->n_preads = (int64_t)K.p_pos.size();
     ctx->classes.clear();
-    const bool log = fig_knobs_from_env(0).log;
+    const bool log = up_knobs.log;
+    if (log) fprintf(stderr, "[figsched] persistent slab: %lld B with %d base slots per gap, %lld B with min(candidates, %d) slots per gap%s\n", (long long)persist_base, K.nslots,
+                     (long long)K.persist_total, K.nslots_wide, K.nslots_wide < wide_asked ? " (FIG_SLOTS_WIDE halved: what was asked for does not fit, the slab in a quarter of the free device memory or a later allocation)" : "");
     for (const FigLaunchClass &lc : K.classes) {
         fig_ctx::Cls c;
         c.c = lc;
@@ -478,13 +516,13 @@
     size_t total_blocks = 0;
     for (const fig_ctx::Cls &c : ctx->classes) total_blocks += (size_t)c.capacity;
     if ((rc = dev_alloc(ctx, (size_t)stride * std::max<size_t>(total_blocks, 1), &p))) return rc; db.scratch = (uint8_t *)p;
-    if ((rc = dev_alloc(ctx, (size_t)K.persist_total + 256, &p))) return rc; db.persist = (uint8_t *)p;
+    db.persist = (uint8_t *)persist_mem;
     if ((rc = dev_alloc(ctx, (size_t)std::max<int64_t>(ng, 1) * sizeof(FigGapCtl), &p))) return rc; db.gapctl = (FigGapCtl *)p;
     if ((rc = dev_alloc(ctx, (size_t)std::max<int64_t>(ng, 1) * 4, &p))) return rc; db.gap_pending = (int32_t *)p;
     if ((rc = dev_alloc(ctx, (size_t)std::max<int64_t>(ng, 1), &p))) return rc; ctx->d_ot = (uint8_t *)p; db.ot_preset = ctx->d_ot;
     ctx->h_ot = K.ot_preset;
     FIG_HIP(hipMemcpyAsync(ctx->d_ot, ctx->h_ot.data(), (size_t)std::max<int64_t>(ng, 1), hipMemcpyHostToDevice, ctx->stream));
-    ctx->nslots = K.nslots;
+    ctx->nslots = K.nslots; ctx->nslots_wide = K.nslots_wide;
     {   size_t blk = 0;
         for (size_t ci = 0; ci < ctx->classes.size(); ci++) {
             const fig_ctx::Cls &c = ctx->classes[ci];
@@ -493,10 +531,11 @@
             if (hipStreamCreate(&l.stream) != hipSuccess || hipEventCreateWithFlags(&l.done, hipEventDisableTiming) != hipSuccess) return FIG_EHIP;
             l.queue_head = db.queue_head + 16 * (ci + 1);
             l.scratch = db.scratch + (size_t)stride * blk; blk += (size_t)c.capacity;
-            l.cap = (size_t)std::max(c.c.q_end - c.c.q_begin, 1) * (size_t)(K.nslots + 1);
+            const std::vector<int> lane_ids(K.order.begin() + c.c.q_begin, K.order.begin() + c.c.q_end);
+            l.cap = fig_lane_items(lane_ids, K.gaps);
             if ((rc = dev_alloc(ctx, l.cap * sizeof(FigItem), &p))) return rc; l.d_items = (FigItem *)p;
             if ((rc = dev_alloc(ctx, l.cap * sizeof(FigEntry), &p))) return rc; l.d_entries = (FigEntry *)p;
-            l.cont_cap = fig_cont_capacity(std::vector<int>(K.order.begin() + c.c.q_begin, K.order.begin() + c.c.q_end), K.gaps, fig_knobs_from_env(0).minc);
+            l.cont_cap = fig_cont_capacity(lane_ids, K.gaps, up_knobs.minc);
             if ((rc = dev_alloc(ctx, sizeof(FigContHdr) + (size_t)l.cont_cap * sizeof(FigCont), &p))) return rc; l.d_cont = (uint8_t *)p;
             if (hipHostMalloc((void **)&l.h_ctl, (size_t)std::max<int64_t>(ng, 1) * sizeof(FigGapCtl), hipHostMallocDefault) != hipSuccess) return FIG_ENOMEM;
             if (hipHostMalloc((void **)&l.h_items, l.cap * sizeof(FigItem), hipHostMallocDefault) != hipSuccess) return FIG_ENOMEM;
@@ -516,6 +555,20 @@
     ctx->have_batch = true;
     if (!K.ot_given && m->partial_flag && ng > 0 && (rc = fig_ot_carry_measured(ctx, ng))) { free_batch(ctx); return rc; }
     return FIG_OK;
+}
+
+extern "C" int fig_batch_upload(fig_ctx *ctx, const fig_gap_batch *b) {
+    if (!ctx || !b) return FIG_EINVAL;
+    if (!ctx->have_model) return FIG_EINVAL;
+    hipSetDevice(ctx->device);
+    const FigKnobs kn = fig_knobs_from_env(ctx->hm.unmapped_flag);
+    const int base = FigPacked().nslots;
+    const int asked = kn.wide ? std::max(base, std::min(kn.slots_wide, FIG_SLOTS_WIDE_MAX)) : base;
+    for (int w = asked;; w = std::max(base, w / 2)) {
+        const int rc = fig_upload_once(ctx, b, w, asked);
+        if (rc != FIG_ENOMEM || w <= base) return rc;
+        (void)hipGetLastError();
+    }
 }
 
 extern "C" int fig_batch_probe_reach(fig_ctx *ctx, uint8_t *reach) {
@@ -560,7 +613,7 @@
     auto fail = [&](hipError_t er) { ctx->last_hip = (int)er; return -1; };
     const int capacity = std::max(1, c.capacity);
     auto launch = [&](FigKind kind, int n_work, const void *list) {
-        hipError_t er = launch_any(ctx, c, db, stream, kind, std::min(capacity, n_work), list, n_work, ln.qsel);
+        hipError_t er = launch_any(ctx, c, db, stream, kind, std::min(capacity, n_work), list, n_work, ln.qsel, ln.wide);
         ln.qsel ^= 1; nl++;
         return er;
     };
@@ -575,7 +628,8 @@
     while (true) {
         if ((e = hipMemcpyAsync(ctl, db.gapctl, ctl_bytes, hipMemcpyDeviceToHost, stream)) != hipSuccess) return fail(e);
         if ((e = hipStreamSynchronize(stream)) != hipSuccess) return fail(e);
-        fig_plan_round(ids, ctl, capacity, c.c.nsplit, ctx->nslots, knobs.minc, knobs.ipw, n_active_max, R);
+        fig_plan_round(ids, ctl, capacity, c.c.nsplit, ctx->nslots, knobs.wide, ctx->nslots_wide, knobs.wide_max_active, knobs.minc, knobs.ipw, n_active_max, R);
+        ln.wide = fig_wide_for_lane(knobs.wide, n_active_max, knobs.wide_max_active);
         if (knobs.log) { double t = now(); fprintf(stderr, "[figsched] capG=%d round %d: active=%d chunk=%d items=%d blocks=%d  %.1f ms\n", c.c.capG, round, last_active, last_chunk, last_items, capacity, t - t_prev); t_prev = t; }
         round++;
         if (R.n_active == 0) break;
@@ -687,6 +741,7 @@
       fprintf(stderr, "[figprof] barrier wait %.3f of %.3f wave-Gcycles = %.1f %%\n", cnt[FIG_CNT_WAIT] / 1e9, wave / 1e9, wave ? 100.0 * cnt[FIG_CNT_WAIT] / wave : 0.0); }
 #endif
     if (knobs.log) fprintf(stderr, "[figsched] useful flops %.4g, speculative evaluations executed %.4g (%.1f %% discarded)\n", (double)cnt[FIG_CNT_FLOPS], (double)cnt[FIG_CNT_SPEC], cnt[FIG_CNT_SPEC] ? 100.0 * (1.0 - ((double)cnt[FIG_CNT_FLOPS] / (double)cnt[FIG_CNT_SPEC])) : 0.0);
+    if (knobs.log && knobs.wide) fprintf(stderr, "[figsched] widened chunks narrowed to the live workgroups: %llu\n", cnt[FIG_CNT_NARROW]);
     fig_stats_from_counters(cnt, ctx->stats);
     int rc = fig_compact_results(ng, hstr.data(), ctx->h_str_off.data(), out);
     if (!rc && sup) fig_compact_support(ng, hsup.data(), ctx->h_str_off.data(), out, sup->counts);
diff --git a/figbird_amd/csrc/fig_abi_host.h b/figbird_amd/csrc/fig_abi_host.h
--- a/figbird_amd/csrc/fig_abi_host.h
+++ b/figbird_amd/csrc/fig_abi_host.h
@@ -170,6 +170,7 @@
 struct FigKnobs {
     bool seq;
     bool cont; int cont_cap, cont_live, cont_prio;
+    int wide, slots_wide, wide_max_active;
     bool lanes_serial;
     bool log;
     int minc;
@@ -177,6 +178,8 @@
     int sh_on;
 };
 
+#define FIG_WIDE_DEFAULT_UNMAPPED FIG_WIDE_GROW
+#define FIG_SLOTS_WIDE_MAX 4096
 static FigKnobs fig_knobs_from_env(int unmapped) {
     FigKnobs k;
     const char *sched = getenv("FIG_SCHED"), *ser = getenv("FIG_LANES"), *mc = getenv("FIG_MIN_CHUNK"), *ipw = getenv("FIG_ITEMS_PER_WG");
@@ -187,6 +190,12 @@
     k.cont_cap = cc ? std::max(1, atoi(cc)) : FIG_CONT_CAP_MAX;
     k.cont_live = cl ? std::max(0, atoi(cl)) : 100;
     k.cont_prio = cp ? (atoi(cp) != 0) : 1;
+    const char *wd = getenv("FIG_WIDE"), *sw = getenv("FIG_SLOTS_WIDE");
+    k.wide = !wd ? (unmapped ? FIG_WIDE_DEFAULT_UNMAPPED : 0) : !strcmp(wd, "grow") ? FIG_WIDE_GROW : !strcmp(wd, "idle") ? FIG_WIDE_IDLE : !strcmp(wd, "both") ? (FIG_WIDE_GROW | FIG_WIDE_IDLE) : 0;
+    if (!k.cont) k.wide = 0;
+    k.slots_wide = sw ? atoi(sw) : 256;
+    const char *wa = getenv("FIG_WIDE_MAX_ACTIVE");
+    k.wide_max_active = wa ? std::max(0, atoi(wa)) : 96;
     k.lanes_serial = ser && strcmp(ser, "serial") == 0;
     k.log = getenv("FIG_SCHED_LOG") != nullptr;
     k.minc = mc ? std::max(1, atoi(mc)) : 16;
@@ -197,7 +206,11 @@
 
 struct FigRound { std::vector<FigItem> items; std::vector<FigEntry> entries; int chunk = 0, n_active = 0; };
 
-static void fig_plan_round(const std::vector<int> &ids, const FigGapCtl *ctl, int capacity, int nsplit, int slots_cap, int minc, double ipw_base,
+static inline int fig_wide_for_lane(int wide_mode, int n_active_max, int wide_max_active) {
+    return n_active_max > wide_max_active ? (wide_mode & ~FIG_WIDE_GROW) : wide_mode;
+}
+
+static void fig_plan_round(const std::vector<int> &ids, const FigGapCtl *ctl, int capacity, int nsplit, int slots_cap, int wide_mode, int wide_cap, int wide_max_active, int minc, double ipw_base,
                            int &n_active_max, FigRound &R) {
     R.items.clear(); R.entries.clear();
     R.chunk = 0; R.n_active = 0;
@@ -206,6 +219,7 @@
     long long rem_total = 0;
     for (int g : ids) if (ctl[g].status == FIG_GAP_MORE) rem_total += std::max(0, ctl[g].range - ctl[g].j);
     n_active_max = std::max(n_active_max, R.n_active);
+    wide_mode = fig_wide_for_lane(wide_mode, n_active_max, wide_max_active);
     const double ipw = ipw_base * std::min(8.0, std::max(1.0, n_active_max / 96.0));
     const double share = rem_total > 0 ? (ipw * capacity / (double)std::max(1, nsplit)) / (double)rem_total : 1.0;
     const double target = ipw * capacity / (double)std::max(1, nsplit);
@@ -217,10 +231,22 @@
         int want = (int)std::ceil((range - j) * share);
         want = std::min(std::max(want, minc), slots_cap);
         int n = std::max(0, std::min(want, range - j));
-        R.chunk = std::max(R.chunk, n);
+        if (j > 0 && n > 0 && (wide_mode & FIG_WIDE_GROW) && wide_cap > slots_cap)
+            n = std::max(n, fig_wide_chunk(FigWide{FIG_WIDE_GROW, slots_cap, wide_cap}, 1, ctl[g].last, wide_cap, range - j, 1, 0));
         total += n;
         R.entries.push_back(FigEntry{g, n, 0, 0});
     }
+    if ((wide_mode & FIG_WIDE_IDLE) && wide_cap > slots_cap && (int)R.entries.size() == R.n_active) {
+        long long spare = (long long)(capacity / std::max(1, nsplit)) - total;
+        for (FigEntry &en : R.entries) {
+            const int j = ctl[en.gap].j, left = ctl[en.gap].range - j;
+            if (spare <= 0) break;
+            if (j == 0 || en.n == 0) continue;
+            const int n = fig_wide_chunk(FigWide{FIG_WIDE_IDLE, slots_cap, wide_cap}, en.n, en.n, wide_cap, left, 1, (int)std::min<long long>(en.n + spare, wide_cap));
+            if (n > en.n) { spare -= n - en.n; total += n - en.n; en.n = n; }
+        }
+    }
+    for (const FigEntry &en : R.entries) R.chunk = std::max(R.chunk, en.n);
     for (const FigEntry &en : R.entries)
         for (int k = en.n - 1; k >= 0; k--) R.items.push_back(FigItem{en.gap, ctl[en.gap].j + k, k, 0});
 }
@@ -241,4 +267,10 @@
     return (int)std::min<long long>(std::max<long long>(n, 1), FIG_CONT_CAP_MAX);
 }
 
+static size_t fig_lane_items(const std::vector<int> &ids, const std::vector<FigDevGap> &gaps) {
+    size_t n = 0;
+    for (int g : ids) n += (size_t)gaps[(size_t)g].nslots + 1;
+    return std::max<size_t>(n, 1);
+}
+
 #endif
diff --git a/figbird_amd/csrc/fig_engine.h b/figbird_amd/csrc/fig_engine.h
--- a/figbird_amd/csrc/fig_engine.h
+++ b/figbird_amd/csrc/fig_engine.h
@@ -245,7 +245,8 @@
 }
 
 struct FigKernArgs { int capG, capGl, ncolE, Wcap, nteams, q_begin, q_end, qsel, tiles, tile_step, tile_cols, tiled_max, sh_on;
-                     int cont = 0, minc = 16, cont_live = 100, cont_prio = 1; };
+                     int cont = 0, minc = 16, cont_live = 100, cont_prio = 1;
+                     int wide = 0, wide_base = 64, wide_cap = 64; };
 
 FIG_D long long fig_eng_carve(FigEng &E, const FigDevModel &M, const FigKernArgs &A, bool lds_tab) {
     E.capG = A.capG;
diff --git a/figbird_amd/csrc/fig_engine_sched.h b/figbird_amd/csrc/fig_engine_sched.h
--- a/figbird_amd/csrc/fig_engine_sched.h
+++ b/figbird_amd/csrc/fig_engine_sched.h
@@ -69,6 +69,7 @@
         L.fill_or_not = 0; L.same_count = 0; L.same_thresh = M.unmapped ? 50 : 4; L.stuckCount = 0;
         int range = gapMax - gapMin + 1;
         if (range > E.B->capC) range = E.B->capC;
+        if (range > g.rangeCap) range = g.rangeCap;
         L.range = range; L.side_flag = 0; L.less_read_flag = 0;
         L.prev_best = -1; L.curr_best = 0; L.prev_u = -1; L.curr_u = 0; L.sec_same = 0; L.sec_same2 = 0;
         L.done = 0; L.need_orig = 0; L.ev_iters = 0; L.ev_side_break = 0; L.ev_fill = 0;
@@ -448,10 +449,10 @@
 }
 
 FIG_D FigGapCtl &fig_ctl_of(const FigEng &E, int gi) { return *(E.B->gapctl + gi); }
-FIG_D void fig_ctl_publish(const FigEng &E, int gi) {
+FIG_D void fig_ctl_publish(const FigEng &E, int gi, int last) {
     if (E.tid != 0) return;
     FigGapCtl &c = fig_ctl_of(E, gi);
-    c.status = E.S->L.done ? FIG_GAP_LOOP_DONE : FIG_GAP_MORE; c.j = E.S->L.j; c.range = E.S->L.range;
+    c.status = E.S->L.done ? FIG_GAP_LOOP_DONE : FIG_GAP_MORE; c.j = E.S->L.j; c.range = E.S->L.range; c.last = last;
 }
 
 template <bool LDS>
@@ -470,7 +471,7 @@
         if (E.tid == 0) fig_ctl_of(E, gi).status = FIG_GAP_FINISHED;
     } else {
         fig_state_save(E, P);
-        fig_ctl_publish(E, gi);
+        fig_ctl_publish(E, gi, 0);
     }
     FIG_SYNC();
 }
@@ -495,7 +496,7 @@
     E.g = &E.B->gaps[en.gap];
     FigPersist P; fig_persist_of(*E.B, *E.g, P);
     fig_spec_replay(E, work, P, en.n, E.g->capGg);
-    fig_ctl_publish(E, en.gap);
+    fig_ctl_publish(E, en.gap, en.n);
 }
 
 template <bool LDS>
@@ -515,16 +516,37 @@
     return n;
 }
 
-FIG_D void fig_item_continue(FigEng &E, const FigScr &work, int gi, int n, int minc, FigCont &next) {
+enum { FIG_WIDE_GROW = 1, FIG_WIDE_IDLE = 2 };
+struct FigWide { int mode, base, W; };
+FIG_HD int fig_wide_chunk(FigWide w, int minc, int last, int slots, int left, int consumed_all, int spare) {
+    const int today = fig_cont_chunk(minc, last, slots < w.base ? slots : w.base, left);
+    if (!w.mode || !consumed_all) return today;
+    int cap = w.W < slots ? w.W : slots;
+    if (cap > left) cap = left;
+    int n = today;
+    if (w.mode & FIG_WIDE_GROW) { const int g = last > (1 << 29) ? (1 << 30) : 2 * last; const int c = g < cap ? g : cap; if (c > n) n = c; }
+    if (w.mode & FIG_WIDE_IDLE) { const int c = spare < cap ? spare : cap; if (c > n) n = c; }
+    return n;
+}
+
+FIG_HD int fig_wide_rank(FigWide w, int minc, int n, int slots, int left) {
+    int r = 0;
+    const int trips = left;
+    for (int i = 0; i < trips && left > 0 && n > 0; i++) { r++; left -= n; n = fig_wide_chunk(w, minc, n, slots, left, 1, 0); }
+    return r;
+}
+
+FIG_D void fig_item_continue(FigEng &E, const FigScr &work, int gi, int n, int minc, FigWide w, int spare, FigCont &next) {
     fig_item_replay(E, work, FigEntry{gi, n, 0, 0});
     FIG_SYNC();
     const FigLoop &L = E.S->L;
     next.gap = gi; next.next = 0; next.ready = 0; next.pad = 0;
     if (L.done) { next.kind = FIG_CONT_END; next.j0 = 0; next.n = 1; next.rank = 1; }
     else {
-        const int left = L.range - L.j;
-        next.kind = FIG_CONT_EVAL; next.j0 = L.j; next.n = fig_cont_chunk(minc, n, E.g->nslots, left);
-        next.rank = (left + next.n - 1) / (next.n > 0 ? next.n : 1);
+        const int left = L.range - L.j, slots = E.g->nslots;
+        next.kind = FIG_CONT_EVAL; next.j0 = L.j; next.n = fig_wide_chunk(w, minc, n, slots, left, 1, spare);
+        next.pad = fig_wide_chunk(FigWide{0, w.base, w.W}, minc, n, slots, left, 1, 0);
+        next.rank = fig_wide_rank(w, minc, next.n, slots, left);
     }
     FIG_SYNC();
 }
diff --git a/figbird_amd/csrc/fig_pack.h b/figbird_amd/csrc/fig_pack.h
--- a/figbird_amd/csrc/fig_pack.h
+++ b/figbird_amd/csrc/fig_pack.h
@@ -65,11 +65,22 @@
     int capR = 1, capP = 1, capC = 1, capG = 8, capW = 0, capE = 0;
     int64_t str_total = 0, n_gaps = 0, persist_total = 0, stream_total = 0;
     int nslots = 64;
+    int nslots_wide = 64;
     int64_t packed_bytes() const {
         return (int64_t)(packed.size() * 4 + flank.size() + gaps.size() * sizeof(FigDevGap) + qual.size() +
                          (u_pos.size() * 3 + p_pos.size() * 5) * 4 + (u_woff.size() + p_woff.size() + p_qoff.size()) * 8);
     }
 };
+
+static void fig_pack_persist(FigPacked &K, size_t state_bytes) {
+    long long off = 0;
+    for (FigDevGap &d : K.gaps) {
+        d.nslots = std::max(1, std::min(d.rangeCap, K.nslots_wide));
+        d.persistOff = off;
+        off += (fig_persist_layout(nullptr, d.capGg, d.nU, d.nP, d.rangeCap, d.nslots, state_bytes, nullptr) + 255) & ~255LL;
+    }
+    K.persist_total = off;
+}
 
 static int fig_pack(const fig_model *m, const fig_gap_batch *b, size_t state_bytes, FigPacked &K) {
     int64_t ng = b->n_gaps;
@@ -181,17 +192,9 @@
         int gm = std::max(d.G0, (int)(d.G0 * d.gpf2));
         if (m->unmapped_flag && d.G0 <= m->unm_limit) gm = std::max(gm, d.G0 < 30 ? 70 : 3 * d.G0);
         gmax[g] = std::min(gm, d.alloc_arg);
-    }
-    {
-        long long off = 0;
-        for (int64_t g = 0; g < ng; g++) {
-            FigDevGap &d = K.gaps[g];
-            d.capGg = (gmax[g] + 7) & ~7; d.rangeCap = gap_range(d.G0, d.gpf1, d.gpf2); d.nslots = K.nslots;
-            d.persistOff = off;
-            off += (fig_persist_layout(nullptr, d.capGg, d.nU, d.nP, d.rangeCap, d.nslots, state_bytes, nullptr) + 255) & ~255LL;
-        }
-        K.persist_total = off;
-    }
+        K.gaps[g].capGg = (gmax[g] + 7) & ~7; K.gaps[g].rangeCap = gap_range(d.G0, d.gpf1, d.gpf2);
+    }
+    fig_pack_persist(K, state_bytes);
     struct ClsDef { int capGl, nt; };
     const ClsDef defs[] = {{448, 256}, {1216, 512}, {1600, 512}, {1 << 30, 512}};
     K.order.clear(); K.classes.clear();
diff --git a/figbird_amd/csrc/fig_types.h b/figbird_amd/csrc/fig_types.h
--- a/figbird_amd/csrc/fig_types.h
+++ b/figbird_amd/csrc/fig_types.h
@@ -16,7 +16,7 @@
 enum { FIG_ORG_NONE = 0, FIG_ORG_FINAL = 1, FIG_ORG_ORIGINAL = 2, FIG_ORG_TIEBREAK = 4 };
 
 enum { FIG_GAP_FINISHED = 0, FIG_GAP_MORE = 1, FIG_GAP_LOOP_DONE = 2 };
-struct FigGapCtl { int32_t status, j, range, reach; };
+struct FigGapCtl { int32_t status, j, range; union { int32_t reach; int32_t last; }; };
 
 struct alignas(16) FigItem { int32_t gap, j, slot, chunk; };
 struct alignas(16) FigEntry { int32_t gap, n, j_planned, stamped; };
@@ -24,7 +24,7 @@
 enum { FIG_CONT_EVAL = 0, FIG_CONT_END = 1 };
 #define FIG_CONT_CAP_MAX 65535
 struct alignas(16) FigCont { int32_t gap, j0, n, kind; int32_t next, ready, rank, pad; };
-struct alignas(16) FigContHdr { int32_t tail, exited, pad[2]; };
+struct alignas(16) FigContHdr { int32_t tail, exited, open, pad; };
 static_assert(sizeof(FigCont) == 32 && sizeof(FigContHdr) == 16, "continuation records: buffers are sized by sizeof");
 
 enum FigCounter {
@@ -32,6 +32,7 @@
     FIG_CNT_FLOPS = 1, FIG_CNT_SPEC = 2,
     FIG_CNT_MLE_ALG = 3, FIG_CNT_MLE_EXEC = 4,
     FIG_CNT_CONT = 5,
+    FIG_CNT_NARROW = 6,
     FIG_CNT_PROF_LO = 8, FIG_CNT_WAIT = 30, FIG_CNT_WAVE = 31, FIG_CNT_PROF_HI = 32,
     FIG_CNT_N = 64
 };
```

Measured after the change: 26.00 (median of 6 runs). +5.5%, better.
